# yangzichuang/TextSummarization-On-Flink

Measured on AMD Instinct MI355X. Metric: train_tokens_per_sec, higher is better.
Workload: dtype bf16; 1 GPU; model=pointer-generator+coverage hidden=256 emb=128 enc=400 dec=100 vocab=50000, global_batch=256, per_gpu_batch=256, seq_len=400->100, parallelism=dp1, backend=none, grad_allreduce=none, graph=True, persistent_lstm=True, proj_attn=True, skip_pad_steps=True, decoder_row_groups=2

## Files before the change

csrc/bindings.cpp:

```cpp
#include <torch/library.h>
#include <ATen/ATen.h>
#include <c10/hip/HIPStream.h>
#include <algorithm>
#include <optional>

#include "launchers.h"

using at::Tensor;
using OT = std::optional<Tensor>;

namespace {

hipStream_t stream() { return c10::hip::getCurrentHIPStream().stream(); }

void chk(const Tensor& t, at::ScalarType dt, const char* name) {
  TORCH_CHECK(t.is_cuda(), name, " must be a GPU tensor");
  TORCH_CHECK(t.scalar_type() == dt, name, " has dtype ", t.scalar_type(), ", expected ", dt);
  TORCH_CHECK(t.is_contiguous(), name, " must be contiguous");
}
template <typename T>
T* P(const Tensor& t) { return reinterpret_cast<T*>(t.data_ptr()); }
template <typename T>
T* PO(const OT& t) { return t.has_value() && t->defined() ? reinterpret_cast<T*>(t->data_ptr()) : nullptr; }
void numel_eq(const Tensor& t, int64_t n, const char* name) {
  TORCH_CHECK(t.numel() == n, name, " has ", t.numel(), " elements, expected ", n);
}
void chko(const OT& t, at::ScalarType dt, int64_t n, const char* name) {
  if (t.has_value() && t->defined()) { chk(*t, dt, name); numel_eq(*t, n, name); }
}
const auto F32 = at::kFloat;
const auto BF = at::kBFloat16;
const auto I32 = at::kInt;

void lstm_enc_fwd_step(const Tensor& gx, const Tensor& bias, const Tensor& Wt, const Tensor& hs, const Tensor& cs,
                       const Tensor& acts, const Tensor& out, const Tensor& lens, int64_t s, int64_t T, int64_t B,
                       int64_t H) {
  chk(gx, F32, "gx"); chk(bias, F32, "bias"); numel_eq(bias, 2 * 4 * H, "bias"); chk(Wt, BF, "Wt"); chk(hs, BF, "hs"); chk(cs, F32, "cs"); chk(acts, F32, "acts");
  chk(out, BF, "out"); chk(lens, I32, "lens");
  TORCH_CHECK(H % 32 == 0 && s >= 0 && s < T, "bad lstm args");
  numel_eq(gx, 2 * T * B * 4 * H, "gx"); numel_eq(Wt, 2 * 4 * H * H, "Wt");
  numel_eq(hs, 2 * (T + 1) * B * H, "hs"); numel_eq(cs, 2 * (T + 1) * B * H, "cs");
  numel_eq(acts, 2 * T * B * 4 * H, "acts"); numel_eq(out, B * T * 2 * H, "out"); numel_eq(lens, B, "lens");
  launch_lstm_enc_fwd_step(P<float>(gx), P<float>(bias), P<bf16>(Wt), P<bf16>(hs), P<float>(cs), P<float>(acts), P<bf16>(out),
                           P<int>(lens), s, T, B, H, stream());
}

void lstm_enc_bwd_step(const Tensor& dz, const Tensor& Wn, const Tensor& dout, const Tensor& dh_fin,
                       const Tensor& dc_carry, const Tensor& acts, const Tensor& cs, const Tensor& lens, int64_t s,
                       int64_t T, int64_t B, int64_t H) {
  chk(dz, BF, "dz"); chk(Wn, BF, "Wn"); chk(dout, F32, "dout"); chk(dh_fin, F32, "dh_fin");
  chk(dc_carry, F32, "dc_carry"); chk(acts, F32, "acts"); chk(cs, F32, "cs"); chk(lens, I32, "lens");
  TORCH_CHECK(H % 32 == 0 && s >= 0 && s < T, "bad lstm args");
  numel_eq(dz, 2 * T * B * 4 * H, "dz"); numel_eq(Wn, 2 * 4 * H * H, "Wn"); numel_eq(dout, B * T * 2 * H, "dout");
  numel_eq(dh_fin, 2 * B * H, "dh_fin"); numel_eq(dc_carry, 2 * B * H, "dc_carry");
  numel_eq(acts, 2 * T * B * 4 * H, "acts"); numel_eq(cs, 2 * (T + 1) * B * H, "cs");
  launch_lstm_enc_bwd_step(P<bf16>(dz), P<bf16>(Wn), P<float>(dout), P<float>(dh_fin), P<float>(dc_carry),
                           P<float>(acts), P<float>(cs), P<int>(lens), s, T, B, H, stream());
}

int64_t lstm_persistent_grid_op(int64_t H, int64_t B) { return lstm_persistent_grid((int)H, (int)B); }
int64_t lstm_persistent_capacity_op(int64_t H) { return lstm_persistent_capacity((int)H); }
int64_t lstm_persistent_launches_op(int64_t H, int64_t B) { return lstm_persistent_launches((int)H, (int)B); }
int64_t lstm_persistent_xbuf_op(int64_t H, int64_t B, bool bwd) {
  return (int64_t)lstm_persistent_xbuf_elems((int)H, (int)B, bwd);
}

void lstm_fwd_persistent(const Tensor& gx, const Tensor& bias, const Tensor& Wt, const Tensor& hs, const Tensor& cs,
                         const Tensor& acts, const Tensor& out, const Tensor& lens, const Tensor& xbuf,
                         const Tensor& err, int64_t T, int64_t B, int64_t H) {
  chk(gx, F32, "gx"); chk(bias, F32, "bias"); numel_eq(bias, 2 * 4 * H, "bias"); chk(Wt, BF, "Wt"); chk(hs, BF, "hs"); chk(cs, F32, "cs"); chk(acts, F32, "acts");
  chk(out, BF, "out"); chk(lens, I32, "lens"); chk(xbuf, at::kLong, "xbuf"); chk(err, I32, "err");
  TORCH_CHECK(lstm_persistent_grid((int)H, (int)B) > 0, "persistent LSTM: unsupported H/B (H in {64,128,256,512}; "
              "a launch's grid must fit the resident capacity, one workgroup per CU)");
  TORCH_CHECK(T >= 1 && T < (1 << 30), "bad T");
  numel_eq(gx, 2 * T * B * 4 * H, "gx"); numel_eq(Wt, 2 * 4 * H * H, "Wt");
  numel_eq(hs, 2 * (T + 1) * B * H, "hs"); numel_eq(cs, 2 * (T + 1) * B * H, "cs");
  numel_eq(acts, 2 * T * B * 4 * H, "acts"); numel_eq(out, B * T * 2 * H, "out"); numel_eq(lens, B, "lens");
  TORCH_CHECK(xbuf.numel() >= (int64_t)lstm_persistent_xbuf_elems((int)H, (int)B, false), "xbuf too small");
  numel_eq(err, 1, "err");
  launch_lstm_fwd_persistent(P<float>(gx), P<float>(bias), P<bf16>(Wt), P<bf16>(hs), P<float>(cs), P<float>(acts), P<bf16>(out),
                             P<int>(lens), (unsigned long long*)xbuf.data_ptr(), (unsigned*)err.data_ptr(), T, B, H,
                             stream());
}

bool lstm_persistent_fx_ok_op(int64_t H, int64_t B, int64_t E) { return lstm_persistent_fx_ok((int)H, (int)B, (int)E); }
void lstm_fwd_persistent_fx(const Tensor& xsf, const Tensor& Wx0, const Tensor& Wx1, const Tensor& bias,
                            const Tensor& Wt, const Tensor& hs, const Tensor& cs, const Tensor& acts, const Tensor& out,
                            const Tensor& lens, const Tensor& xbuf, const Tensor& err, int64_t T, int64_t B, int64_t H) {
  chk(xsf, BF, "xsf"); chk(Wx0, BF, "Wx0"); chk(Wx1, BF, "Wx1");
  chk(bias, F32, "bias"); numel_eq(bias, 2 * 4 * H, "bias"); chk(Wt, BF, "Wt"); chk(hs, BF, "hs"); chk(cs, F32, "cs");
  chk(acts, F32, "acts"); chk(out, BF, "out"); chk(lens, I32, "lens"); chk(xbuf, at::kLong, "xbuf"); chk(err, I32, "err");
  TORCH_CHECK(lstm_persistent_fx_ok((int)H, (int)B, 128), "persistent LSTM with the input projection: unsupported H/B");
  TORCH_CHECK(T >= 1 && T < (1 << 30), "bad T");
  numel_eq(xsf, 2 * T * B * 128, "xsf"); numel_eq(Wx0, 4 * H * 128, "Wx0"); numel_eq(Wx1, 4 * H * 128, "Wx1");
  numel_eq(Wt, 2 * 4 * H * H, "Wt");
  numel_eq(hs, 2 * (T + 1) * B * H, "hs"); numel_eq(cs, 2 * (T + 1) * B * H, "cs");
  numel_eq(acts, 2 * T * B * 4 * H, "acts"); numel_eq(out, B * T * 2 * H, "out"); numel_eq(lens, B, "lens");
  TORCH_CHECK(xbuf.numel() >= (int64_t)lstm_persistent_xbuf_elems((int)H, (int)B, false), "xbuf too small");
  numel_eq(err, 1, "err");
  launch_lstm_fwd_persistent(nullptr, P<float>(bias), P<bf16>(Wt), P<bf16>(hs), P<float>(cs), P<float>(acts), P<bf16>(out),
                             P<int>(lens), (unsigned long long*)xbuf.data_ptr(), (unsigned*)err.data_ptr(), T, B, H,
                             stream(), P<bf16>(xsf), P<bf16>(Wx0), P<bf16>(Wx1));
}

void lstm_bwd_persistent(const Tensor& dz, const Tensor& Wn, const Tensor& dout, const Tensor& dh_fin,
                         const Tensor& dc_carry, const Tensor& acts, const Tensor& cs, const Tensor& lens,
                         const Tensor& xbuf, const Tensor& err, const OT& dbias, int64_t T, int64_t B, int64_t H,
                         bool dout_batch_frame) {
  const bool dout16 = dout.scalar_type() == BF;
  TORCH_CHECK(!dout16 || dout_batch_frame, "lstm_bwd_persistent: a bf16 dout is read in the batch frame only");
  chk(dz, BF, "dz"); chk(Wn, BF, "Wn"); chk(dout, dout16 ? BF : F32, "dout"); chk(dh_fin, F32, "dh_fin");
  chko(dbias, F32, 2 * 4 * H, "dbias");
  chk(dc_carry, F32, "dc_carry"); chk(acts, F32, "acts"); chk(cs, F32, "cs"); chk(lens, I32, "lens");
  chk(xbuf, at::kLong, "xbuf"); chk(err, I32, "err");
  TORCH_CHECK(lstm_persistent_grid((int)H, (int)B) > 0, "persistent LSTM: unsupported H/B");
  TORCH_CHECK(T >= 1 && T < (1 << 30), "bad T");
  numel_eq(dz, 2 * T * B * 4 * H, "dz"); numel_eq(Wn, 2 * 4 * H * H, "Wn"); numel_eq(dout, B * T * 2 * H, "dout");
  numel_eq(dh_fin, 2 * B * H, "dh_fin"); numel_eq(dc_carry, 2 * B * H, "dc_carry");
  numel_eq(acts, 2 * T * B * 4 * H, "acts"); numel_eq(cs, 2 * (T + 1) * B * H, "cs"); numel_eq(lens, B, "lens");
  TORCH_CHECK(xbuf.numel() >= (int64_t)lstm_persistent_xbuf_elems((int)H, (int)B, true), "xbuf too small");
  numel_eq(err, 1, "err");
  launch_lstm_bwd_persistent(P<bf16>(dz), P<bf16>(Wn), (const float*)dout.data_ptr(), P<float>(dh_fin),
                             P<float>(dc_carry), P<float>(acts), P<float>(cs), P<int>(lens),
                             (unsigned long long*)xbuf.data_ptr(), (unsigned*)err.data_ptr(), PO<float>(dbias), T, B, H,
                             dout_batch_frame, stream(), dout16);
}

void attn_score(const Tensor& F, const Tensor& s, const Tensor& v, const OT& wc, const OT& cov, const Tensor& lens,
                const Tensor& e, int64_t B, int64_t T, int64_t A, int64_t rep) {
  chk(F, BF, "F"); chk(s, F32, "s"); chk(v, F32, "v"); chk(lens, I32, "lens"); chk(e, F32, "e");
  TORCH_CHECK(A % 64 == 0 && A <= 1024 && T % 2 == 0, "attention size must be a multiple of 64 (<= 1024), T even");
  TORCH_CHECK((rep == 1 || rep == 2 || rep == 4) && B % rep == 0, "rep must be 1, 2 or 4 and divide B");
  numel_eq(F, B / rep * T * A, "F"); numel_eq(s, B * A, "s"); numel_eq(v, A, "v"); numel_eq(e, B * T, "e");
  numel_eq(lens, B / rep, "lens"); chko(wc, F32, A, "wc"); chko(cov, F32, B * T, "cov");
  launch_attn_score(P<bf16>(F), P<float>(s), P<float>(v), PO<float>(wc), PO<float>(cov), P<int>(lens), P<float>(e), B,
                    T, A, rep, stream());
}

void attn_softmax_ctx(const Tensor& e, const Tensor& E, const Tensor& lens, const OT& cov, const Tensor& a_out,
                      const OT& cov_out, const OT& covloss, const Tensor& ctx, const OT& ctx_bf, int64_t B, int64_t T,
                      int64_t A, int64_t rep) {
  chk(e, F32, "e"); chk(E, BF, "E"); chk(lens, I32, "lens"); chk(a_out, F32, "a_out"); chk(ctx, F32, "ctx");
  TORCH_CHECK((rep == 1 || rep == 2 || rep == 4) && B % rep == 0, "rep must be 1, 2 or 4 and divide B");
  TORCH_CHECK(A % 64 == 0 && T <= (rep == 1 ? 2048 : 1024), "bad attention shape");
  numel_eq(e, B * T, "e"); numel_eq(E, B / rep * T * A, "E"); numel_eq(a_out, B * T, "a_out");
  numel_eq(ctx, B * A, "ctx"); numel_eq(lens, B / rep, "lens");
  chko(cov, F32, B * T, "cov"); chko(cov_out, F32, B * T, "cov_out"); chko(covloss, F32, B, "covloss");
  chko(ctx_bf, BF, B * A, "ctx_bf");
  launch_attn_softmax_ctx(P<float>(e), P<bf16>(E), P<int>(lens), PO<float>(cov), P<float>(a_out), PO<float>(cov_out),
                          PO<float>(covloss), P<float>(ctx), PO<bf16>(ctx_bf), B, T, A, rep, stream());
}

bool attn_row_ok(int64_t A, int64_t T) { return attn_row_supported((int)A, (int)T); }
void attn_fwd_row(const Tensor& F, const Tensor& E, const Tensor& s, const Tensor& v, const OT& wc, const OT& cov,
                  const Tensor& lens, const Tensor& a_out, const OT& cov_out, const OT& covloss, const Tensor& ctx,
                  const OT& ctx_bf, int64_t B, int64_t T, int64_t A, int64_t rep) {
  chk(F, BF, "F"); chk(E, BF, "E"); chk(s, F32, "s"); chk(v, F32, "v"); chk(lens, I32, "lens");
  chk(a_out, F32, "a_out"); chk(ctx, F32, "ctx");
  TORCH_CHECK(attn_row_supported((int)A, (int)T), "row attention needs A in {512, 1024} and T <= 2048");
  TORCH_CHECK(rep >= 1 && B % rep == 0, "attn_fwd_row: rep must divide B");
  numel_eq(F, B / rep * T * A, "F"); numel_eq(E, B / rep * T * A, "E"); numel_eq(s, B * A, "s"); numel_eq(v, A, "v");
  numel_eq(lens, B / rep, "lens"); numel_eq(a_out, B * T, "a_out"); numel_eq(ctx, B * A, "ctx");
  chko(wc, F32, A, "wc"); chko(cov, F32, B * T, "cov"); chko(cov_out, F32, B * T, "cov_out");
  chko(covloss, F32, B, "covloss"); chko(ctx_bf, BF, B * A, "ctx_bf");
  launch_attn_fwd_row(P<bf16>(F), P<bf16>(E), P<float>(s), P<float>(v), PO<float>(wc),
                      PO<float>(cov), P<int>(lens), P<float>(a_out), PO<float>(cov_out), PO<float>(covloss), P<float>(ctx),
                      PO<bf16>(ctx_bf), B, T, A, (int)rep, stream());
}
void attn_fwd_row_probe(const Tensor& F, const Tensor& E, const Tensor& s, const Tensor& v, const Tensor& wc,
                        const Tensor& cov, const Tensor& lens, const Tensor& a_out, const Tensor& ctx, int64_t B, int64_t T,
                        int64_t rep, int64_t probe) {
  chk(F, BF, "F"); chk(E, BF, "E"); chk(s, F32, "s"); chk(v, F32, "v"); chk(wc, F32, "wc"); chk(cov, F32, "cov");
  chk(lens, I32, "lens"); chk(a_out, F32, "a_out"); chk(ctx, F32, "ctx");
  TORCH_CHECK(rep >= 1 && B % rep == 0 && T <= 2048, "attn_fwd_row_probe: rep | B, T <= 2048");
  numel_eq(F, B / rep * T * 512, "F"); numel_eq(E, B / rep * T * 512, "E"); numel_eq(s, B * 512, "s");
  numel_eq(v, 512, "v"); numel_eq(wc, 512, "wc"); numel_eq(cov, B * T, "cov"); numel_eq(lens, B / rep, "lens");
  numel_eq(a_out, B * T, "a_out"); numel_eq(ctx, B * 512, "ctx");
  launch_attn_fwd_row_probe(P<bf16>(F), P<bf16>(E), P<float>(s), P<float>(v), P<float>(wc), P<float>(cov), P<int>(lens),
                            P<float>(a_out), P<float>(ctx), (int)B, (int)T, (int)rep, (int)probe, stream());
}
void attn_bwd_row(const Tensor& E, const Tensor& F, const Tensor& s, const Tensor& v, const OT& wc, const OT& cov,
                  const Tensor& a, const Tensor& dctx, const Tensor& ctx, const OT& Ga, const OT& dcov_next,
                  const OT& gcl, const Tensor& lens, const Tensor& de_out, const Tensor& ds, const OT& dcov_out,
                  int64_t B, int64_t T, int64_t A) {
  chk(E, BF, "E"); chk(F, BF, "F"); chk(s, F32, "s"); chk(v, F32, "v"); chk(a, F32, "a"); chk(dctx, F32, "dctx");
  chk(ctx, F32, "ctx"); chk(lens, I32, "lens"); chk(de_out, F32, "de_out"); chk(ds, F32, "ds");
  TORCH_CHECK(attn_row_supported((int)A, (int)T), "row attention needs A in {512, 1024} and T <= 2048");
  numel_eq(E, B * T * A, "E"); numel_eq(F, B * T * A, "F"); numel_eq(s, B * A, "s"); numel_eq(v, A, "v");
  numel_eq(a, B * T, "a"); numel_eq(dctx, B * A, "dctx"); numel_eq(ctx, B * A, "ctx"); numel_eq(lens, B, "lens");
  numel_eq(de_out, B * T, "de_out"); numel_eq(ds, B * A, "ds");
  chko(wc, F32, A, "wc"); chko(cov, F32, B * T, "cov"); chko(Ga, F32, B * T, "Ga");
  chko(dcov_next, F32, B * T, "dcov_next"); chko(gcl, F32, B, "gcl"); chko(dcov_out, F32, B * T, "dcov_out");
  launch_attn_bwd_row(P<bf16>(E), P<bf16>(F), P<float>(s), P<float>(v), PO<float>(wc), PO<float>(cov), P<float>(a),
                      P<float>(dctx), P<float>(ctx), PO<float>(Ga), PO<float>(dcov_next), PO<float>(gcl),
                      P<int>(lens), P<float>(de_out), P<float>(ds), PO<float>(dcov_out), B, T, A, stream());
}

bool attn_rowp_ok(int64_t A, int64_t T, int64_t EG) { return attn_rowp_supported((int)A, (int)T, (int)EG); }
bool dec_persistent_ok_op(int64_t H, int64_t E, int64_t A, int64_t B, int64_t T) {
  return dec_persistent_shape_ok((int)H, (int)E, (int)A, (int)B, (int)T);
}
int64_t dec_persistent_grid_op(int64_t B) { return dec_persistent_grid((int)B); }
int64_t dec_persistent_capacity_op() { return dec_persistent_capacity(); }
int64_t dec_persistent_xbuf_op(int64_t B) { return (int64_t)dec_persistent_xbuf_elems((int)B); }
void dec_fwd_persistent(const Tensor& XG, const Tensor& KcT, const Tensor& WsT, const Tensor& bs, const Tensor& Cst,
                        const Tensor& Cb, const Tensor& Hb, const Tensor& ACT, const Tensor& S, const Tensor& F,
                        const Tensor& G, const Tensor& v, const OT& wc, const OT& COV, const Tensor& lens,
                        const Tensor& ATT, const Tensor& ATTb, const OT& covloss, const Tensor& GV, const Tensor& GVb,
                        const OT& dlen, const Tensor& xbuf, const Tensor& err, int64_t B, int64_t T, int64_t D,
                        int64_t H, int64_t E, int64_t A) {
  TORCH_CHECK(dec_persistent_shape_ok((int)H, (int)E, (int)A, (int)B, (int)T) && D >= 1,
              "dec_fwd_persistent: unsupported shape");
  const int64_t grid = dec_persistent_grid((int)B);
  TORCH_CHECK(grid > 0 && grid <= dec_persistent_capacity(),
              "dec_fwd_persistent: the grid would not be co-resident on this device");
  chk(XG, F32, "XG"); numel_eq(XG, D * B * 4 * H, "XG");
  chk(KcT, BF, "KcT"); numel_eq(KcT, 4 * H * (E + H), "KcT");
  chk(WsT, BF, "WsT"); numel_eq(WsT, A * 2 * H, "WsT");
  chk(bs, F32, "bs"); numel_eq(bs, A, "bs");
  chk(Cst, F32, "Cst"); numel_eq(Cst, (D + 1) * B * H, "Cst");
  chk(Cb, BF, "Cb"); numel_eq(Cb, (D + 1) * B * H, "Cb");
  chk(Hb, BF, "Hb"); numel_eq(Hb, (D + 1) * B * H, "Hb");
  chk(ACT, F32, "ACT"); numel_eq(ACT, D * B * 4 * H, "ACT");
  chk(S, F32, "S"); numel_eq(S, D * B * A, "S");
  chk(F, BF, "F"); numel_eq(F, B * T * A, "F");
  chk(G, BF, "G"); numel_eq(G, B * T * E, "G");
  chk(v, F32, "v"); numel_eq(v, A, "v");
  chko(wc, F32, A, "wc");
  chko(COV, F32, (D + 1) * B * T, "COV");
  chk(lens, I32, "lens"); numel_eq(lens, B, "lens");
  chk(ATT, F32, "ATT"); numel_eq(ATT, D * B * T, "ATT");
  chk(ATTb, BF, "ATTb"); numel_eq(ATTb, D * B * T, "ATTb");
  chko(covloss, F32, D * B, "covloss");
  TORCH_CHECK((PO<float>(COV) != nullptr) == (PO<float>(covloss) != nullptr), "COV and covloss go together");
  chk(GV, F32, "GV"); numel_eq(GV, D * B * E, "GV");
  chk(GVb, BF, "GVb"); numel_eq(GVb, D * B * E, "GVb");
  chko(dlen, I32, B, "dlen");
  chk(xbuf, at::kLong, "xbuf"); numel_eq(xbuf, (int64_t)dec_persistent_xbuf_elems((int)B), "xbuf");
  chk(err, I32, "err");
  launch_dec_fwd_persistent(P<float>(XG), P<bf16>(KcT), P<bf16>(WsT), P<float>(bs), P<float>(Cst), P<bf16>(Cb),
                            P<bf16>(Hb), P<float>(ACT), P<float>(S), P<bf16>(F), P<bf16>(G), P<float>(v),
                            PO<float>(wc), PO<float>(COV), P<int>(lens), P<float>(ATT), P<bf16>(ATTb),
                            PO<float>(covloss), P<float>(GV), P<bf16>(GVb), PO<int>(dlen),
                            (unsigned long long*)xbuf.data_ptr(), (unsigned*)err.data_ptr(), (int)B, (int)T, (int)D,
                            stream());
}

void attn_fwd_rowp(const Tensor& F, const Tensor& G, const Tensor& s, const Tensor& v, const OT& wc, const OT& cov,
                   const Tensor& lens, const Tensor& a_out, const OT& cov_out, const OT& covloss, const Tensor& gx,
                   const Tensor& gx_bf, int64_t B, int64_t T, int64_t A, const OT& dlen, int64_t step,
                   const OT& a_bf) {
  chk(F, BF, "F"); chk(G, BF, "G"); chk(s, F32, "s"); chk(v, F32, "v"); chk(lens, I32, "lens");
  chk(a_out, F32, "a_out"); chk(gx, F32, "gx"); chk(gx_bf, BF, "gx_bf"); chko(a_bf, BF, B * T, "a_bf");
  const int64_t EG = gx.numel() / std::max<int64_t>(B, 1);
  TORCH_CHECK(attn_rowp_supported((int)A, (int)T, (int)EG), "projected row attention needs A in {512, 1024}, "
              "T <= 2048 and a 128-wide projection");
  numel_eq(F, B * T * A, "F"); numel_eq(G, B * T * EG, "G"); numel_eq(s, B * A, "s"); numel_eq(v, A, "v");
  numel_eq(lens, B, "lens"); numel_eq(a_out, B * T, "a_out"); numel_eq(gx, B * EG, "gx"); numel_eq(gx_bf, B * EG, "gx_bf");
  chko(wc, F32, A, "wc"); chko(cov, F32, B * T, "cov"); chko(cov_out, F32, B * T, "cov_out");
  chko(covloss, F32, B, "covloss"); chko(dlen, I32, B, "dlen");
  launch_attn_fwd_rowp(P<bf16>(F), P<bf16>(G), P<float>(s), P<float>(v), PO<float>(wc), PO<float>(cov), P<int>(lens),
                       P<float>(a_out), PO<float>(cov_out), PO<float>(covloss), P<float>(gx), P<bf16>(gx_bf), B, T, A,
                       PO<int>(dlen), (int)step, stream(), PO<bf16>(a_bf));
}
void attn_bwd_rowp(const Tensor& G, const Tensor& F, const Tensor& s, const Tensor& v, const OT& wc, const OT& cov,
                   const Tensor& a, const OT& dx, const Tensor& gv, const OT& Ga, const OT& dcov_next, const OT& gcl,
                   const Tensor& lens, const Tensor& de_out, const Tensor& ds, const OT& dcov_out, int64_t B, int64_t T,
                   int64_t A, const OT& dlen, int64_t step) {
  chk(G, BF, "G"); chk(F, BF, "F"); chk(s, F32, "s"); chk(v, F32, "v"); chk(a, F32, "a"); chk(gv, F32, "gv");
  chk(lens, I32, "lens"); chk(de_out, F32, "de_out"); chk(ds, F32, "ds");
  const int64_t EG = gv.numel() / std::max<int64_t>(B, 1);
  TORCH_CHECK(attn_rowp_supported((int)A, (int)T, (int)EG), "projected row attention needs A in {512, 1024}, "
              "T <= 2048 and a 128-wide projection");
  numel_eq(G, B * T * EG, "G"); numel_eq(F, B * T * A, "F"); numel_eq(s, B * A, "s"); numel_eq(v, A, "v");
  numel_eq(a, B * T, "a"); numel_eq(gv, B * EG, "gv"); numel_eq(lens, B, "lens");
  numel_eq(de_out, B * T, "de_out"); numel_eq(ds, B * A, "ds");
  chko(dx, F32, B * EG, "dx"); chko(wc, F32, A, "wc"); chko(cov, F32, B * T, "cov"); chko(Ga, F32, B * T, "Ga");
  chko(dcov_next, F32, B * T, "dcov_next"); chko(gcl, F32, B, "gcl"); chko(dcov_out, F32, B * T, "dcov_out");
  chko(dlen, I32, B, "dlen");
  launch_attn_bwd_rowp(P<bf16>(G), P<bf16>(F), P<float>(s), P<float>(v), PO<float>(wc), PO<float>(cov), P<float>(a),
                       PO<float>(dx), P<float>(gv), PO<float>(Ga), PO<float>(dcov_next), PO<float>(gcl), P<int>(lens),
                       P<float>(de_out), P<float>(ds), PO<float>(dcov_out), B, T, A, PO<int>(dlen), (int)step, stream());
}

void attn_bwd_step(const Tensor& E, const Tensor& F, const Tensor& s, const Tensor& v, const OT& wc, const OT& cov,
                   const Tensor& a, const Tensor& dctx, const Tensor& ctx, const OT& Ga, const OT& dcov_next,
                   const OT& gcl, const Tensor& lens, const Tensor& de_out, const Tensor& ds, const OT& dcov_out,
                   int64_t B, int64_t T, int64_t A) {
  chk(E, BF, "E"); chk(F, BF, "F"); chk(s, F32, "s"); chk(v, F32, "v"); chk(a, F32, "a"); chk(dctx, F32, "dctx");
  chk(ctx, F32, "ctx"); chk(lens, I32, "lens"); chk(de_out, F32, "de_out"); chk(ds, F32, "ds");
  TORCH_CHECK(A % 64 == 0 && A <= 1024 && T >= 1, "bad A/T");
  numel_eq(E, B * T * A, "E"); numel_eq(F, B * T * A, "F"); numel_eq(s, B * A, "s"); numel_eq(v, A, "v");
  numel_eq(a, B * T, "a"); numel_eq(dctx, B * A, "dctx"); numel_eq(ctx, B * A, "ctx"); numel_eq(lens, B, "lens");
  numel_eq(de_out, B * T, "de_out"); numel_eq(ds, B * A, "ds");
  chko(wc, F32, A, "wc"); chko(cov, F32, B * T, "cov"); chko(Ga, F32, B * T, "Ga");
  chko(dcov_next, F32, B * T, "dcov_next"); chko(gcl, F32, B, "gcl"); chko(dcov_out, F32, B * T, "dcov_out");
  launch_attn_bwd_step(P<bf16>(E), P<bf16>(F), P<float>(s), P<float>(v), PO<float>(wc), PO<float>(cov), P<float>(a),
                       P<float>(dctx), P<float>(ctx), PO<float>(Ga), PO<float>(dcov_next), PO<float>(gcl),
                       P<int>(lens), P<float>(de_out), P<float>(ds), PO<float>(dcov_out), B, T, A, stream());
}

void attn_bwd_feat(const Tensor& F, const Tensor& S_all, const Tensor& v, const OT& wc, const OT& cov_all,
                   const Tensor& de_all, const Tensor& lens, const Tensor& dF, const Tensor& dv, const OT& dwc,
                   int64_t D, int64_t B, int64_t T, int64_t A, const OT& dlen) {
  chk(F, BF, "F"); chk(S_all, F32, "S_all"); chk(v, F32, "v"); chk(de_all, F32, "de_all"); chk(lens, I32, "lens");
  chk(dF, BF, "dF"); chk(dv, F32, "dv");
  TORCH_CHECK(A % 64 == 0, "bad A");
  numel_eq(F, B * T * A, "F"); numel_eq(S_all, D * B * A, "S_all"); numel_eq(de_all, D * B * T, "de_all");
  const int64_t nslot = dv.numel() / A;
  TORCH_CHECK(nslot >= 1 && nslot <= (1 << 20) && (nslot & (nslot - 1)) == 0 && dv.numel() == nslot * A,
              "dv: [nslot, A] with nslot a power of two");
  numel_eq(dF, B * T * A, "dF");
  chko(wc, F32, A, "wc"); chko(cov_all, F32, D * B * T, "cov_all"); chko(dwc, F32, nslot * A, "dwc");
  chko(dlen, I32, B, "dlen");
  launch_attn_bwd_feat(P<bf16>(F), P<float>(S_all), P<float>(v), PO<float>(wc), PO<float>(cov_all), P<float>(de_all),
                       P<int>(lens), P<bf16>(dF), P<float>(dv), PO<float>(dwc), D, B, T, A, (int)nslot, stream(),
                       PO<int>(dlen));
}

int64_t attn_chunks(int64_t T) { return attn_nchunk(T); }

void emb_grad_sorted(const Tensor& gemb, const Tensor& sid, const Tensor& perm, const Tensor& src0, const Tensor& src1) {
  chk(gemb, F32, "gemb"); chk(src0, F32, "src0"); chk(src1, F32, "src1");
  TORCH_CHECK(gemb.dim() == 2 && gemb.size(1) <= 512, "gemb must be [V][E], E <= 512");
  TORCH_CHECK(sid.scalar_type() == at::kInt && perm.scalar_type() == at::kInt && sid.is_contiguous() &&
              perm.is_contiguous() && sid.numel() == perm.numel(), "sid / perm int32, contiguous, one length");
  const int64_t E = gemb.size(1), V = gemb.size(0);
  TORCH_CHECK(src0.numel() % E == 0 && src1.numel() % E == 0, "src rows");
  const int64_t n0 = src0.numel() / E, n1 = src1.numel() / E;
  TORCH_CHECK(sid.numel() == n0 + n1, "sid must cover src0 and src1 rows");
  launch_emb_grad_sorted(P<float>(gemb), P<int>(sid), P<int>(perm), P<float>(src0), (int)n0, P<float>(src1),
                         (int)n1, (int)E, (int)V, stream());
}

int64_t emb_grad_det_chunks_op(int64_t n) { return emb_grad_det_chunks((int)n); }
void emb_grad_det(const Tensor& gemb, const Tensor& sid, const Tensor& perm, const Tensor& src0, const Tensor& src1,
                  const Tensor& pf, const Tensor& pl) {
  chk(gemb, F32, "gemb"); chk(src0, F32, "src0"); chk(src1, F32, "src1"); chk(pf, F32, "pf"); chk(pl, F32, "pl");
  TORCH_CHECK(gemb.dim() == 2 && gemb.size(1) <= 512, "gemb must be [V][E], E <= 512");
  TORCH_CHECK(sid.scalar_type() == at::kInt && perm.scalar_type() == at::kInt && sid.is_contiguous() &&
              perm.is_contiguous() && sid.numel() == perm.numel(), "sid / perm int32, contiguous, one length");
  const int64_t E = gemb.size(1), V = gemb.size(0);
  TORCH_CHECK(src0.numel() % E == 0 && src1.numel() % E == 0, "src rows");
  const int64_t n0 = src0.numel() / E, n1 = src1.numel() / E;
  TORCH_CHECK(sid.numel() == n0 + n1, "sid must cover src0 and src1 rows");
  const int64_t nc = emb_grad_det_chunks((int)(n0 + n1));
  numel_eq(pf, nc * E, "pf"); numel_eq(pl, nc * E, "pl");
  launch_emb_grad_det(P<float>(gemb), P<int>(sid), P<int>(perm), P<float>(src0), (int)n0, P<float>(src1), (int)n1,
                      (int)E, (int)V, P<float>(pf), P<float>(pl), stream());
}

void step_frame_hop(const Tensor& in, const Tensor& rev, const Tensor& out, int64_t B, int64_t T, int64_t H) {
  chk(in, F32, "in"); chk(out, F32, "out");
  TORCH_CHECK(H % 4 == 0 && B > 0 && T > 0, "step_frame_hop: H % 4 == 0");
  TORCH_CHECK(rev.scalar_type() == at::kLong && rev.is_contiguous() && rev.numel() == B * T, "rev [B,T] int64");
  numel_eq(in, 2 * T * B * 2 * H, "in"); numel_eq(out, 2 * T * B * H, "out");
  launch_step_frame_hop(P<float>(in), rev.data_ptr<int64_t>(), P<float>(out), (int)B, (int)T, (int)H, stream());
}

void to_step_frame(const Tensor& src, const OT& ids, const Tensor& rev, const Tensor& out, int64_t B, int64_t T,
                   int64_t W, int64_t doff) {
  TORCH_CHECK(src.is_cuda() && src.is_contiguous() && out.is_contiguous() && src.scalar_type() == out.scalar_type(),
              "src/out: contiguous GPU tensors of one dtype");
  TORCH_CHECK(src.scalar_type() == BF || src.scalar_type() == F32, "bf16 or fp32");
  TORCH_CHECK(rev.scalar_type() == at::kLong && rev.is_contiguous() && rev.numel() == B * T, "rev [B,T] int64");
  const int es = (int)src.element_size();
  TORCH_CHECK((W * es) % 16 == 0 && (doff * es) % 16 == 0, "rows must be 16-byte multiples");
  const int64_t S = src.size(-1);
  TORCH_CHECK(doff + W <= S && (S * es) % 16 == 0, "bad row width");
  if (ids.has_value()) {
    TORCH_CHECK(ids->scalar_type() == at::kLong && ids->is_contiguous() && ids->numel() == B * T, "ids [B,T] int64");
  } else {
    TORCH_CHECK(src.numel() == B * T * S, "src must be [B,T,S] without ids");
  }
  numel_eq(out, 2 * T * B * W, "out");
  launch_to_step_frame(src.data_ptr(), es, PO<int64_t>(ids), P<int64_t>(rev), out.data_ptr(), (int)B, (int)T, (int)W,
                       (int)S, (int)doff, src.numel() / S, stream());
}
void from_step_frame(const Tensor& in, const Tensor& rev, const Tensor& out, int64_t B, int64_t T, int64_t W) {
  chk(in, F32, "in"); chk(out, F32, "out");
  TORCH_CHECK(rev.scalar_type() == at::kLong && rev.is_contiguous() && rev.numel() == B * T, "rev [B,T] int64");
  TORCH_CHECK(W % 4 == 0, "W % 4");
  numel_eq(in, 2 * T * B * W, "in"); numel_eq(out, B * T * W, "out");
  launch_from_step_frame(P<float>(in), P<int64_t>(rev), P<float>(out), (int)B, (int)T, (int)W, stream());
}
void transpose_bta(const Tensor& in, const Tensor& out, int64_t B, int64_t T, int64_t A) {
  chk(in, BF, "in"); chk(out, BF, "out");
  TORCH_CHECK(A % 64 == 0, "A % 64");
  numel_eq(in, B * T * A, "in"); numel_eq(out, B * T * A, "out");
  launch_transpose_bta(P<bf16>(in), P<bf16>(out), (int)B, (int)T, (int)A, stream());
}
void tr01(const Tensor& in, const OT& out, const OT& outb, int64_t np_, int64_t nq, int64_t nr, bool acc) {
  chk(in, F32, "in");
  TORCH_CHECK(nr % 4 == 0 && np_ >= 1 && nq >= 1, "tr01: R % 4 == 0");
  TORCH_CHECK(!acc || (out.has_value() && !outb.has_value()), "tr01: acc adds into out (no bf16 twin)");
  numel_eq(in, np_ * nq * nr, "in");
  chko(out, F32, np_ * nq * nr, "out"); chko(outb, BF, np_ * nq * nr, "outb");
  TORCH_CHECK((uintptr_t)in.data_ptr() % 16 == 0, "tr01: in must be 16-byte aligned");
  TORCH_CHECK(!PO<float>(out) || (uintptr_t)PO<float>(out) % 16 == 0, "tr01: out must be 16-byte aligned");
  TORCH_CHECK(!PO<bf16>(outb) || (uintptr_t)PO<bf16>(outb) % 8 == 0, "tr01: outb must be 8-byte aligned");
  launch_tr01(P<float>(in), PO<float>(out), PO<bf16>(outb), (int)np_, (int)nq, (int)nr, acc, stream());
}
void cast_colsum(const Tensor& x, const Tensor& xb, const Tensor& colsum, int64_t N, int64_t C) {
  chk(x, F32, "x"); chk(xb, BF, "xb"); chk(colsum, F32, "colsum");
  TORCH_CHECK(C % 4 == 0 && C / 4 <= 256 && 256 % (C / 4) == 0, "cast_colsum: C % 4 == 0 and C / 4 divides 256");
  numel_eq(x, N * C, "x"); numel_eq(xb, N * C, "xb"); numel_eq(colsum, C, "colsum");
  auto part = at::empty({(int64_t)cast_colsum_blocks((int)N, (int)C), C}, x.options());
  launch_cast_colsum(P<float>(x), P<bf16>(xb), P<float>(part), P<float>(colsum), (int)N, (int)C, stream());
}
void colsum(const Tensor& x, const Tensor& out, int64_t N, int64_t C, bool acc) {
  TORCH_CHECK(x.is_cuda() && x.is_contiguous() && (x.scalar_type() == F32 || x.scalar_type() == BF),
              "colsum: x must be a contiguous CUDA fp32 / bf16 tensor");
  chk(out, F32, "out");
  numel_eq(x, N * C, "x"); numel_eq(out, C, "out");
  auto part = at::empty({(int64_t)colsum_det_chunks((int)N, (int)C), C}, out.options());
  launch_colsum_det(x.data_ptr(), x.scalar_type() == BF, P<float>(part), P<float>(out), (int)N, (int)C, acc, stream());
}

void rs_fwd(const Tensor& cs, const Tensor& hs, int64_t T, const Tensor& RCt, const Tensor& RHt, const Tensor& bc,
            const Tensor& bh, const Tensor& pre_c, const Tensor& pre_h, const Tensor& c0, const Tensor& c0b,
            const Tensor& h0b, const OT& cat_c, const OT& cat_h, int64_t B, int64_t H) {
  chk(cs, F32, "cs"); chk(hs, BF, "hs"); chk(RCt, BF, "RCt"); chk(RHt, BF, "RHt"); chk(bc, F32, "bc"); chk(bh, F32, "bh");
  chk(pre_c, F32, "pre_c"); chk(pre_h, F32, "pre_h"); chk(c0, F32, "c0"); chk(c0b, BF, "c0b"); chk(h0b, BF, "h0b");
  TORCH_CHECK(H % 32 == 0 && H <= 512, "reduce_states: H % 32 == 0, H <= 512");
  numel_eq(cs, 2 * (T + 1) * B * H, "cs"); numel_eq(hs, 2 * (T + 1) * B * H, "hs");
  numel_eq(RCt, 2 * H * H, "RCt"); numel_eq(RHt, 2 * H * H, "RHt"); numel_eq(bc, H, "bc"); numel_eq(bh, H, "bh");
  numel_eq(pre_c, B * H, "pre_c"); numel_eq(pre_h, B * H, "pre_h"); numel_eq(c0, B * H, "c0");
  numel_eq(c0b, B * H, "c0b"); numel_eq(h0b, B * H, "h0b");
  chko(cat_c, BF, 2 * B * H, "cat_c"); chko(cat_h, BF, 2 * B * H, "cat_h");
  const size_t off = (size_t)T * B * H, ds = (size_t)(T + 1) * B * H;
  launch_rs_fwd(P<float>(cs) + off, P<bf16>(hs) + off, ds, P<bf16>(RCt), P<bf16>(RHt), P<float>(bc), P<float>(bh),
                P<float>(pre_c), P<float>(pre_h), P<float>(c0), P<bf16>(c0b), P<bf16>(h0b), PO<bf16>(cat_c),
                PO<bf16>(cat_h), (int)B, (int)H, stream());
}

void rs_bwd(const Tensor& gc, const Tensor& gh, const Tensor& pre_c, const Tensor& pre_h, const Tensor& RC,
            const Tensor& RH, const Tensor& dpc, const Tensor& dph, const OT& gbc, const OT& gbh,
            const Tensor& dold_c, const Tensor& dold_h, int64_t B, int64_t H) {
  chk(gc, F32, "gc"); chk(gh, F32, "gh"); chk(pre_c, F32, "pre_c"); chk(pre_h, F32, "pre_h"); chk(RC, BF, "RC");
  chk(RH, BF, "RH"); chk(dpc, BF, "dpc"); chk(dph, BF, "dph"); chko(gbc, F32, H, "gbc"); chko(gbh, F32, H, "gbh");
  chk(dold_c, F32, "dold_c"); chk(dold_h, F32, "dold_h");
  TORCH_CHECK(H % 32 == 0 && H <= 512, "reduce_states: H % 32 == 0, H <= 512");
  for (const Tensor* t : {&gc, &gh, &pre_c, &pre_h, &dpc, &dph}) numel_eq(*t, B * H, "[B][H] operand");
  numel_eq(RC, 2 * H * H, "RC"); numel_eq(RH, 2 * H * H, "RH");
  numel_eq(dold_c, 2 * B * H, "dold_c"); numel_eq(dold_h, 2 * B * H, "dold_h");
  launch_rs_bwd(P<float>(gc), P<float>(gh), P<float>(pre_c), P<float>(pre_h), P<bf16>(RC), P<bf16>(RH), P<bf16>(dpc),
                P<bf16>(dph), PO<float>(gbc), PO<float>(gbh), P<float>(dold_c), P<float>(dold_h), (size_t)B * H, (int)B,
                (int)H, stream());
}

void emb_grad(const Tensor& gemb, const Tensor& ids0, const Tensor& src0, const Tensor& ids1, const Tensor& src1) {
  chk(gemb, F32, "gemb"); chk(src0, F32, "src0"); chk(src1, F32, "src1");
  TORCH_CHECK(ids0.scalar_type() == at::kLong && ids1.scalar_type() == at::kLong && ids0.is_contiguous() &&
              ids1.is_contiguous(), "ids must be contiguous int64");
  TORCH_CHECK(gemb.dim() == 2, "gemb must be [V][E]");
  const int64_t E = gemb.size(1), V = gemb.size(0);
  numel_eq(src0, ids0.numel() * E, "src0"); numel_eq(src1, ids1.numel() * E, "src1");
  launch_emb_grad(P<float>(gemb), P<int64_t>(ids0), P<float>(src0), (int)ids0.numel(), P<int64_t>(ids1), P<float>(src1),
                  (int)ids1.numel(), (int)E, (int)V, stream());
}


void dec_cell_fwd(const Tensor& XG, const OT& ctxp, const Tensor& hprev, const Tensor& cprev, const Tensor& WcT,
                  const Tensor& c_out, const Tensor& cb_out, const Tensor& hb_out, const Tensor& act, int64_t B,
                  int64_t H, int64_t A, const OT& dlen, int64_t step) {
  chk(XG, F32, "XG"); chk(hprev, BF, "hprev"); chk(cprev, F32, "cprev"); chk(WcT, BF, "WcT"); chk(c_out, F32, "c_out");
  chk(cb_out, BF, "cb_out"); chk(hb_out, BF, "hb_out"); chk(act, F32, "act");
  TORCH_CHECK(H % 32 == 0 && A % 32 == 0, "dims must be multiples of 32");
  numel_eq(XG, B * 4 * H, "XG"); chko(ctxp, BF, B * A, "ctxp"); numel_eq(hprev, B * H, "hprev");
  numel_eq(cprev, B * H, "cprev"); numel_eq(WcT, 4 * H * (A + H), "WcT"); numel_eq(c_out, B * H, "c_out");
  numel_eq(cb_out, B * H, "cb_out"); numel_eq(hb_out, B * H, "hb_out"); numel_eq(act, B * 4 * H, "act");
  chko(dlen, I32, B, "dlen");
  launch_dec_cell_fwd(P<float>(XG), PO<bf16>(ctxp), P<bf16>(hprev), P<float>(cprev), P<bf16>(WcT), P<float>(c_out),
                      P<bf16>(cb_out), P<bf16>(hb_out), P<float>(act), B, H, A, PO<int>(dlen), (int)step, stream());
}

void dec_sproj(const Tensor& cb, const Tensor& hb, const Tensor& WsT, const Tensor& bs, const Tensor& s_out, int64_t B,
               int64_t H, int64_t A, const OT& dlen, int64_t step) {
  chk(cb, BF, "cb"); chk(hb, BF, "hb"); chk(WsT, BF, "WsT"); chk(bs, F32, "bs"); chk(s_out, F32, "s_out");
  TORCH_CHECK(H % 32 == 0 && A % 16 == 0, "bad dims");
  numel_eq(cb, B * H, "cb"); numel_eq(hb, B * H, "hb"); numel_eq(WsT, A * 2 * H, "WsT"); numel_eq(bs, A, "bs");
  numel_eq(s_out, B * A, "s_out"); chko(dlen, I32, B, "dlen");
  launch_dec_sproj(P<bf16>(cb), P<bf16>(hb), P<bf16>(WsT), P<float>(bs), P<float>(s_out), B, H, A, PO<int>(dlen),
                   (int)step, stream());
}

void dec_bwd_cell(const Tensor& ds, const Tensor& Ws, const OT& dC_dir, const OT& dH_dir, const Tensor& dh_rec,
                  const Tensor& dc_carry, const Tensor& act, const Tensor& c_now, const Tensor& c_prev,
                  const Tensor& dz, int64_t B, int64_t H, int64_t A, const OT& dlen, int64_t step) {
  chk(ds, F32, "ds"); chk(Ws, BF, "Ws"); chk(dh_rec, F32, "dh_rec"); chk(dc_carry, F32, "dc_carry");
  chk(act, F32, "act"); chk(c_now, F32, "c_now"); chk(c_prev, F32, "c_prev"); chk(dz, BF, "dz");
  TORCH_CHECK(H % 16 == 0 && A % 32 == 0, "bad dims");
  numel_eq(ds, B * A, "ds"); numel_eq(Ws, 2 * H * A, "Ws"); chko(dC_dir, F32, B * H, "dC_dir");
  chko(dH_dir, F32, B * H, "dH_dir"); numel_eq(dh_rec, B * H, "dh_rec"); numel_eq(dc_carry, B * H, "dc_carry");
  numel_eq(act, B * 4 * H, "act"); numel_eq(c_now, B * H, "c_now"); numel_eq(c_prev, B * H, "c_prev");
  numel_eq(dz, B * 4 * H, "dz"); chko(dlen, I32, B, "dlen");
  launch_dec_bwd_cell(P<float>(ds), P<bf16>(Ws), PO<float>(dC_dir), PO<float>(dH_dir), P<float>(dh_rec),
                      P<float>(dc_carry), P<float>(act), P<float>(c_now), P<float>(c_prev), P<bf16>(dz), B, H, A,
                      PO<int>(dlen), (int)step, stream());
}

void dec_bwd_dz(const Tensor& dz, const Tensor& Wbig, const OT& dX_dir, const OT& dCTX_dir_prev, const Tensor& dx_out,
                const OT& dctx_prev_out, const Tensor& dh_rec, int64_t B, int64_t E, int64_t H, int64_t A,
                const OT& dlen, int64_t step) {
  chk(dz, BF, "dz"); chk(Wbig, BF, "Wbig"); chk(dx_out, F32, "dx_out"); chk(dh_rec, F32, "dh_rec");
  TORCH_CHECK(E % 16 == 0 && H % 32 == 0 && A % 16 == 0, "bad dims");
  numel_eq(dz, B * 4 * H, "dz"); numel_eq(Wbig, (E + H + A) * 4 * H, "Wbig");
  chko(dX_dir, F32, B * E, "dX_dir"); chko(dCTX_dir_prev, F32, B * A, "dCTX_dir_prev");
  numel_eq(dx_out, B * E, "dx_out"); chko(dctx_prev_out, F32, B * A, "dctx_prev_out");
  numel_eq(dh_rec, B * H, "dh_rec"); chko(dlen, I32, B, "dlen");
  launch_dec_bwd_dz(P<bf16>(dz), P<bf16>(Wbig), PO<float>(dX_dir), PO<float>(dCTX_dir_prev), P<float>(dx_out),
                    PO<float>(dctx_prev_out), P<float>(dh_rec), B, E, H, A, PO<int>(dlen), (int)step, stream());
}

void ptr_loss(const Tensor& logits, const OT& bias, const Tensor& target, const Tensor& rowg, const OT& pgen,
              const OT& attn, const Tensor& ext, const Tensor& lens, const Tensor& loss_row, const OT& dlogits,
              const OT& dpre, const OT& dA, int64_t N, int64_t B, int64_t T, int64_t V) {
  const bool lbf = logits.scalar_type() == at::kBFloat16;
  chk(logits, lbf ? BF : F32, "logits"); chk(target, I32, "target"); chk(rowg, F32, "rowg"); chk(ext, I32, "ext");
  chk(lens, I32, "lens"); chk(loss_row, F32, "loss_row");
  TORCH_CHECK(lbf != bias.has_value(), "bf16 logits carry their bias (pass None); fp32 logits need the bias");
  chko(bias, F32, V, "bias");
  numel_eq(logits, N * V, "logits"); numel_eq(target, N, "target"); numel_eq(rowg, N, "rowg");
  numel_eq(ext, B * T, "ext"); numel_eq(lens, B, "lens"); numel_eq(loss_row, N, "loss_row");
  TORCH_CHECK(N % B == 0, "N must be D*B");
  chko(pgen, F32, N, "pgen"); chko(attn, F32, N * T, "attn"); chko(dlogits, BF, N * V, "dlogits");
  chko(dpre, F32, N, "dpre"); chko(dA, F32, N * T, "dA");
  TORCH_CHECK(!PO<float>(pgen) || (PO<float>(attn) && (!PO<bf16>(dlogits) || (PO<float>(dpre) && PO<float>(dA)))),
              "pointer mode needs attn, and dpre/dA when computing grads");
  if (lbf) {
    TORCH_CHECK(V <= ptr_loss_bf16_max_vocab(), "bf16 ptr_loss: V <= 65536");
    launch_ptr_loss_bf16(P<bf16>(logits), P<int>(target), P<float>(rowg), PO<float>(pgen), PO<float>(attn),
                         P<int>(ext), P<int>(lens), P<float>(loss_row), PO<bf16>(dlogits), PO<float>(dpre),
                         PO<float>(dA), N, B, T, V, stream());
    return;
  }
  launch_ptr_loss(P<float>(logits), P<float>(*bias), P<int>(target), P<float>(rowg), PO<float>(pgen), PO<float>(attn),
                  P<int>(ext), P<int>(lens), P<float>(loss_row), PO<bf16>(dlogits), PO<float>(dpre), PO<float>(dA), N,
                  B, T, V, stream());
}

int64_t wgrad_tt_ws(int64_t M, int64_t N, int64_t K) {
  if (wgrad_tt_ok((int)M, (int)N, (int)K))
    return wgrad_tt_direct((int)M, (int)N, (int)K, false, false) ? 1
                                                                 : (int64_t)wgrad_tt_splits((int)M, (int)N, (int)K) * M * N;
  if (wgrad_tt_ok((int)N, (int)M, (int)K)) return (int64_t)wgrad_tt_splits((int)N, (int)M, (int)K) * M * N;
  return 0;
}
bool wgrad_tt(const Tensor& a, const Tensor& b, const Tensor& out, const Tensor& ws, bool acc) {
  TORCH_CHECK(a.dim() == 2 && b.dim() == 2 && out.dim() == 2, "wgrad_tt: 2-D views");
  TORCH_CHECK(a.is_cuda() && b.is_cuda() && out.is_cuda() && ws.is_cuda(), "wgrad_tt: GPU tensors");
  TORCH_CHECK(a.scalar_type() == BF && b.scalar_type() == BF && out.scalar_type() == F32 && ws.scalar_type() == F32,
              "wgrad_tt: bf16, bf16 -> fp32");
  TORCH_CHECK(a.stride(1) == 1 && b.stride(1) == 1 && out.stride(1) == 1 && ws.is_contiguous(), "wgrad_tt: unit column stride");
  const int64_t K = a.size(0), M = a.size(1), N = b.size(1), nv = out.size(1);
  TORCH_CHECK(b.size(0) == K && out.size(0) == M && nv <= N, "wgrad_tt: shapes");
  if (!(a.stride(0) % 8 == 0 && b.stride(0) % 8 == 0 && (uintptr_t)a.data_ptr() % 16 == 0 &&
        (uintptr_t)b.data_ptr() % 16 == 0))
    return false;
  const bool plain = wgrad_tt_ok((int)M, (int)N, (int)K), swapped = !plain && wgrad_tt_ok((int)N, (int)M, (int)K);
  if (!plain && !(swapped && nv == N)) return false;
  if (nv != N && (nv % 4 != 0)) return false;
  const bool direct = plain && wgrad_tt_direct((int)M, (int)N, (int)K, false, acc);
  const int64_t need = direct ? 0 : (int64_t)wgrad_tt_splits((int)(plain ? M : N), (int)(plain ? N : M), (int)K) * M * N;
  if (ws.numel() < need) {
    TORCH_CHECK(acc, "wgrad_tt: workspace too small");
    return false;
  }
  if (plain)
    launch_wgrad_tt(P<bf16>(a), (int)a.stride(0), P<bf16>(b), (int)b.stride(0), P<float>(ws), P<float>(out),
                    (int)out.stride(0), (int)M, (int)N, (int)K, false, acc, (int)nv, stream());
  else
    launch_wgrad_tt(P<bf16>(b), (int)b.stride(0), P<bf16>(a), (int)a.stride(0), P<float>(ws), P<float>(out),
                    (int)out.stride(0), (int)N, (int)M, (int)K, true, acc, (int)M, stream());
  return true;
}
bool ctx_bmm_ok_op(int64_t B, int64_t T, int64_t D, int64_t A) { return ctx_bmm_ok((int)B, (int)T, (int)D, (int)A); }
static void ctx_chk(const Tensor& t, at::ScalarType dt, int64_t n, const char* name) {
  chk(t, dt, name);
  numel_eq(t, n, name);
  TORCH_CHECK((uintptr_t)t.data_ptr() % 16 == 0, name, ": 16-byte aligned base");
}
void ctx_fwd(const Tensor& att, const Tensor& enc, const Tensor& ctx, const Tensor& ctxb, int64_t B, int64_t T, int64_t D,
             int64_t A) {
  TORCH_CHECK(ctx_bmm_ok((int)B, (int)T, (int)D, (int)A), "ctx_fwd: D <= 128, T % 8 == 0, A % 128 == 0");
  ctx_chk(att, BF, D * B * T, "att"); ctx_chk(enc, BF, B * T * A, "enc");
  ctx_chk(ctx, F32, D * B * A, "ctx"); ctx_chk(ctxb, BF, D * B * A, "ctxb");
  launch_ctx_fwd(P<bf16>(att), P<bf16>(enc), P<float>(ctx), P<bf16>(ctxb), (int)B, (int)T, (int)D, (int)A, stream());
}
void ctx_da(const Tensor& dctx, const Tensor& enc, const Tensor& da, int64_t B, int64_t T, int64_t D, int64_t A, bool acc) {
  TORCH_CHECK(ctx_bmm_ok((int)B, (int)T, (int)D, (int)A), "ctx_da: D <= 128, T % 8 == 0, A % 128 == 0");
  ctx_chk(dctx, BF, D * B * A, "dctx"); ctx_chk(enc, BF, B * T * A, "enc"); ctx_chk(da, F32, D * B * T, "da");
  launch_ctx_da(P<bf16>(dctx), P<bf16>(enc), P<float>(da), (int)B, (int)T, (int)D, (int)A, acc, stream());
}
void ctx_de(const Tensor& att, const Tensor& dctx, const Tensor& de, int64_t B, int64_t T, int64_t D, int64_t A) {
  TORCH_CHECK(ctx_bmm_ok((int)B, (int)T, (int)D, (int)A), "ctx_de: D <= 128, T % 8 == 0, A % 128 == 0");
  const bool b16 = de.scalar_type() == BF;
  ctx_chk(att, BF, D * B * T, "att"); ctx_chk(dctx, BF, D * B * A, "dctx"); ctx_chk(de, b16 ? BF : F32, B * T * A, "de");
  launch_ctx_de(P<bf16>(att), P<bf16>(dctx), b16 ? nullptr : P<float>(de), b16 ? P<bf16>(de) : nullptr, (int)B, (int)T,
                (int)D, (int)A, stream());
}
void wgrad_tn(const Tensor& a, const Tensor& b, const Tensor& out) {
  TORCH_CHECK(a.dim() == 2 && b.dim() == 2 && out.dim() == 2, "wgrad_tn: 2-D views");
  TORCH_CHECK(a.is_cuda() && b.is_cuda() && out.is_cuda(), "wgrad_tn: GPU tensors");
  TORCH_CHECK(a.scalar_type() == BF && b.scalar_type() == BF && out.scalar_type() == F32, "wgrad_tn: bf16, bf16 -> fp32");
  TORCH_CHECK(a.stride(1) == 1 && b.stride(1) == 1 && out.stride(1) == 1, "wgrad_tn: unit column stride");
  const int64_t K = a.size(0), M = a.size(1), N = b.size(1);
  TORCH_CHECK(b.size(0) == K && out.size(0) == M && out.size(1) == N, "wgrad_tn: shapes");
  TORCH_CHECK(M % 128 == 0 && N % 8 == 0 && K >= 1, "wgrad_tn: M a multiple of 128, N of 8");
  TORCH_CHECK(a.stride(0) % 8 == 0 && b.stride(0) % 8 == 0 && (uintptr_t)a.data_ptr() % 16 == 0 &&
              (uintptr_t)b.data_ptr() % 16 == 0, "wgrad_tn: 16-byte aligned rows");
  launch_wgrad_tn(P<bf16>(a), (int)a.stride(0), P<bf16>(b), (int)b.stride(0), P<float>(out), (int)out.stride(0),
                  (int)M, (int)N, (int)K, stream());
}

int64_t pack_max_jobs_op() { return pack_max_jobs(); }
int64_t pack_job_cols_op() { return pack_job_cols(); }
void pack_cast(const Tensor& jobs, int64_t total) {
  TORCH_CHECK(jobs.is_cuda() && jobs.scalar_type() == at::kLong && jobs.is_contiguous() && jobs.dim() == 2 &&
              jobs.size(1) == pack_job_cols(), "pack_cast: jobs [nj][", pack_job_cols(), "] int64 on the GPU");
  TORCH_CHECK(jobs.size(0) >= 1 && jobs.size(0) <= pack_max_jobs(), "pack_cast: 1..", pack_max_jobs(), " jobs");
  launch_pack_cast(P<long>(jobs), (int)jobs.size(0), (long)total, stream());
}

int64_t debug_enabled() { return tsamd_debug_enabled(); }
Tensor debug_status() {
  unsigned v[4];
  tsamd_debug_read(v);
  Tensor t = at::empty({4}, at::TensorOptions().dtype(at::kLong));
  int64_t* d = t.data_ptr<int64_t>();
  for (int i = 0; i < 4; ++i) d[i] = (int64_t)v[i];
  return t;
}
void debug_clear() { tsamd_debug_clear(); }

bool gemm_bt_ok(int64_t M, int64_t N, int64_t K) { return gemm_bt_supported((int)M, (int)N, (int)K, N % 256 == 0 ? 256 : 128); }
int64_t gemm_bt_splitk_ws(int64_t M, int64_t N, int64_t K) {
  if (!gemm_bt_ok(M, N, K)) return 0;
  const int S = gemm_bt_splits((int)M, (int)N, (int)K);
  return S > 1 ? (int64_t)S * M * N : 0;
}
bool gemm_bt_splitk(const Tensor& A, const Tensor& Bt, const Tensor& out, const Tensor& ws, bool acc) {
  TORCH_CHECK(A.is_cuda() && A.dim() == 2 && A.scalar_type() == BF && A.stride(1) == 1, "gemm_bt_splitk: A [rows, K] bf16");
  TORCH_CHECK(Bt.is_cuda() && Bt.dim() == 2 && Bt.scalar_type() == BF && Bt.stride(1) == 1, "gemm_bt_splitk: Bt [N, K] bf16");
  TORCH_CHECK(out.is_cuda() && out.dim() == 2 && out.stride(1) == 1 && out.scalar_type() == F32, "gemm_bt_splitk: out fp32");
  TORCH_CHECK(ws.is_cuda() && ws.is_contiguous() && ws.scalar_type() == F32, "gemm_bt_splitk: fp32 workspace");
  const int64_t M = out.size(0), N = out.size(1), K = Bt.size(1);
  TORCH_CHECK(Bt.size(0) == N && A.size(1) == K && A.size(0) >= M, "gemm_bt_splitk: shape mismatch A ", A.sizes(), " Bt ",
              Bt.sizes(), " out ", out.sizes());
  const int64_t need = gemm_bt_splitk_ws(M, N, K);
  if (need == 0 || ws.numel() < need) return false;
  if (!(A.stride(0) % 8 == 0 && Bt.stride(0) % 8 == 0 && reinterpret_cast<uintptr_t>(A.data_ptr()) % 16 == 0 &&
        reinterpret_cast<uintptr_t>(Bt.data_ptr()) % 16 == 0 && reinterpret_cast<uintptr_t>(out.data_ptr()) % 16 == 0 &&
        out.stride(0) % 4 == 0))
    return false;
  launch_gemm_bt_splitk(P<bf16>(A), A.stride(0), P<bf16>(Bt), Bt.stride(0), P<float>(ws), P<float>(out), out.stride(0),
                        (int)M, (int)N, (int)K, acc, stream());
  return true;
}
void gemm_bt(const Tensor& A, const Tensor& Bt, const Tensor& out, double beta, const OT& bias, const OT& ids,
             const OT& rev, int64_t B, int64_t T, int64_t dir, const OT& xsf) {
  TORCH_CHECK(A.is_cuda() && A.dim() == 2 && A.scalar_type() == BF && A.stride(1) == 1, "gemm_bt: A [rows, K] bf16");
  TORCH_CHECK(Bt.is_cuda() && Bt.dim() == 2 && Bt.scalar_type() == BF && Bt.stride(1) == 1, "gemm_bt: Bt [N, K] bf16");
  TORCH_CHECK(out.is_cuda() && out.dim() == 2 && out.stride(1) == 1 && (out.scalar_type() == F32 || out.scalar_type() == BF),
              "gemm_bt: out [M, N] fp32 / bf16");
  const int64_t M = out.size(0), N = out.size(1), K = Bt.size(1);
  TORCH_CHECK(Bt.size(0) == N && A.size(1) >= K, "gemm_bt: shape mismatch A ", A.sizes(), " Bt ", Bt.sizes(), " out ", out.sizes());
  TORCH_CHECK(gemm_bt_ok(M, N, K), "gemm_bt: N % 128 == 0 and K % 64 == 0 (got N ", N, " K ", K, ")");
  TORCH_CHECK(A.stride(0) % 8 == 0 && Bt.stride(0) % 8 == 0 && out.stride(0) % 8 == 0 &&
              reinterpret_cast<uintptr_t>(A.data_ptr()) % 16 == 0 && reinterpret_cast<uintptr_t>(Bt.data_ptr()) % 16 == 0 &&
              reinterpret_cast<uintptr_t>(out.data_ptr()) % 16 == 0, "gemm_bt: 16-byte aligned rows");
  const bool obf = out.scalar_type() == BF;
  TORCH_CHECK(beta == 0.0 || (beta == 1.0 && !obf), "gemm_bt: beta 0, or 1 with an fp32 out");
  chko(bias, F32, N, "bias");
  const bool frame = PO<int64_t>(rev) != nullptr;
  if (frame) {
    chk(*rev, at::kLong, "rev"); numel_eq(*rev, B * T, "rev");
    TORCH_CHECK(M == B * T && (dir == 0 || dir == 1), "gemm_bt: step frame needs M = T * B and dir 0 / 1");
    if (PO<int64_t>(ids)) { chk(*ids, at::kLong, "ids"); numel_eq(*ids, B * T, "ids"); }
    else TORCH_CHECK(A.size(0) == B * T, "gemm_bt: batch-frame A needs B * T rows");
    chko(xsf, BF, M * K, "xsf");
  } else {
    TORCH_CHECK(A.size(0) >= M && !PO<int64_t>(ids) && !PO<bf16>(xsf), "gemm_bt: plain A needs M rows (no xsf)");
  }
  launch_gemm_bt(P<bf16>(A), A.stride(0), P<bf16>(Bt), Bt.stride(0), out.data_ptr(), out.stride(0), obf, beta != 0.0,
                 PO<float>(bias), (int)M, (int)N, (int)K, frame ? 1 : 0, PO<int64_t>(ids), PO<int64_t>(rev), PO<bf16>(xsf), A.size(0),
                 (int)B, (int)T, (int)dir, stream());
}

void gemm_bt_merge(const Tensor& dz, const Tensor& Bt, const Tensor& out, const Tensor& rev, int64_t B, int64_t T,
                   int64_t mode) {
  TORCH_CHECK(dz.is_cuda() && dz.scalar_type() == BF && dz.is_contiguous() && dz.numel() % (2 * B * T) == 0,
              "gemm_bt_merge: dz [2][T][B][Kh] bf16, contiguous");
  const int64_t Kh = dz.numel() / (2 * B * T);
  TORCH_CHECK(Bt.is_cuda() && Bt.dim() == 2 && Bt.scalar_type() == BF && Bt.stride(1) == 1 && Bt.size(1) == 2 * Kh,
              "gemm_bt_merge: Bt [N, 2 Kh] bf16");
  chk(out, F32, "out");
  TORCH_CHECK(out.dim() == 2 && out.size(0) == B * T && out.size(1) == Bt.size(0) && out.stride(1) == 1,
              "gemm_bt_merge: out [T * B, N] fp32");
  chk(rev, at::kLong, "rev");
  numel_eq(rev, B * T, "rev");
  TORCH_CHECK(mode >= 0 && mode <= 7, "gemm_bt_merge: mode bits 0-2");
  const int64_t M = B * T, N = Bt.size(0), K = 2 * Kh;
  TORCH_CHECK(Kh % 64 == 0 && gemm_bt_ok(M, N, K), "gemm_bt_merge: Kh % 64 == 0 and N % 128 == 0");
  TORCH_CHECK(Bt.stride(0) % 8 == 0 && out.stride(0) % 4 == 0 && reinterpret_cast<uintptr_t>(dz.data_ptr()) % 16 == 0 &&
              reinterpret_cast<uintptr_t>(Bt.data_ptr()) % 16 == 0 && reinterpret_cast<uintptr_t>(out.data_ptr()) % 16 == 0,
              "gemm_bt_merge: 16-byte aligned rows");
  launch_gemm_bt(P<bf16>(dz), Kh, P<bf16>(Bt), Bt.stride(0), out.data_ptr(), out.stride(0), false, false, nullptr,
                 (int)M, (int)N, (int)K, 2, nullptr, P<int64_t>(rev), nullptr, 0, (int)B, (int)T, (int)mode, stream());
}

int64_t cu_hold_max_lds_op() { return cu_hold_max_lds(); }
void cu_hold(const Tensor& times, int64_t grid, double ms, int64_t lds_bytes) {
  chk(times, at::kLong, "times");
  numel_eq(times, 2 * grid, "times");
  TORCH_CHECK(grid >= 1 && grid <= 4096 && ms > 0 && ms <= 2000, "cu_hold: 1..4096 workgroups for at most 2 s");
  TORCH_CHECK(lds_bytes >= 0 && lds_bytes <= cu_hold_max_lds(), "cu_hold: lds_bytes above the CU's LDS");
  launch_cu_hold((int)grid, (unsigned long long)(ms * 1e5), P<long long>(times), (int)lds_bytes, stream());
}
void tanh_eval(const Tensor& x, const Tensor& t, const Tensor& s2, int64_t mode) {
  chk(x, F32, "x"); chk(t, F32, "t"); chk(s2, F32, "s2");
  numel_eq(t, x.numel(), "t"); numel_eq(s2, x.numel(), "s2");
  TORCH_CHECK(mode == 0 || mode == 1, "tanh_eval: mode 0 (exp + rcp) or 1 (rational)");
  launch_tanh_eval(P<float>(x), P<float>(t), P<float>(s2), (int)x.numel(), (int)mode, stream());
}
void tanh_tput(const Tensor& in, const Tensor& out, int64_t iters, int64_t mode) {
  chk(in, F32, "in"); chk(out, F32, "out");
  TORCH_CHECK(in.numel() >= 1024 && out.numel() % 256 == 0 && out.numel() > 0, "tanh_tput: in >= 1024, out % 256");
  TORCH_CHECK((mode == 0 || mode == 1) && iters >= 1, "tanh_tput: mode 0 / 1");
  launch_tanh_tput(P<float>(in), P<float>(out), (int)out.numel(), (int)iters, (int)mode, stream());
}

int64_t vocab_train_tiles_op(int64_t V, int64_t H) { return vocab_train_tiles((int)V, (int)H); }

void vocab_train_fwd(const Tensor& X, const Tensor& WT, const Tensor& bias, const Tensor& target, const Tensor& part,
                     const Tensor& zg, const Tensor& lse, const Tensor& pv, int64_t N, int64_t V, int64_t H,
                     int64_t ldx, const OT& vblk, const OT& vblk_n) {
  chk(X, BF, "X"); chk(WT, BF, "WT"); chk(bias, F32, "bias"); chk(target, I32, "target"); chk(part, F32, "part");
  chk(zg, F32, "zg"); chk(lse, F32, "lse"); chk(pv, F32, "pv");
  TORCH_CHECK(H == 128 || H == 256 || H == 512, "fused training vocab head: hidden size 128, 256 or 512");
  TORCH_CHECK(N >= 1 && V >= 1 && ldx >= H && ldx % 8 == 0, "bad N/V/ldx");
  numel_eq(X, N * ldx, "X"); numel_eq(WT, V * H, "WT"); numel_eq(bias, V, "bias"); numel_eq(target, N, "target");
  numel_eq(part, (int64_t)vocab_train_tiles((int)V, (int)H) * N * 2, "part"); numel_eq(zg, N, "zg"); numel_eq(lse, N, "lse");
  numel_eq(pv, N, "pv");
  const int64_t RB = (N + 31) / 32;
  TORCH_CHECK(vblk.has_value() == vblk_n.has_value(), "vblk and vblk_n go together");
  chko(vblk, I32, RB, "vblk"); chko(vblk_n, I32, 1, "vblk_n");
  launch_vocab_train_fwd(P<bf16>(X), (int)ldx, P<bf16>(WT), P<float>(bias), P<int>(target), P<float>(part), P<float>(zg),
                         P<float>(lse), P<float>(pv), N, V, H, PO<int>(vblk), PO<int>(vblk_n), stream());
}

void vocab_train_bwd(const Tensor& X, const Tensor& WT, const Tensor& bias, const Tensor& target, const Tensor& lse,
                     const Tensor& alpha, const Tensor& dl, const OT& dbias, int64_t N, int64_t V, int64_t H,
                     int64_t ldx, const OT& vblk, const OT& vblk_n, const OT& vlive, const OT& vstate) {
  chk(X, BF, "X"); chk(WT, BF, "WT"); chk(bias, F32, "bias"); chk(target, I32, "target"); chk(lse, F32, "lse");
  chk(alpha, F32, "alpha"); chk(dl, BF, "dl");
  TORCH_CHECK(H == 128 || H == 256 || H == 512, "fused training vocab head: hidden size 128, 256 or 512");
  TORCH_CHECK(N >= 1 && V >= 1 && ldx >= H && ldx % 8 == 0, "bad N/V/ldx");
  numel_eq(X, N * ldx, "X"); numel_eq(WT, V * H, "WT"); numel_eq(bias, V, "bias"); numel_eq(target, N, "target");
  numel_eq(lse, N, "lse"); numel_eq(alpha, N, "alpha"); chko(dbias, F32, V, "dbias");
  TORCH_CHECK(dl.numel() % N == 0, "dl: numel must be N * ldd");
  const int64_t ldd = dl.numel() / N;
  TORCH_CHECK(ldd >= V && (ldd == V || ldd % 8 == 0), "dl: row length ", ldd, " must be V or a multiple of 8");
  const int64_t RB = (N + 31) / 32;
  const bool has = vblk.has_value();
  TORCH_CHECK(vblk_n.has_value() == has && vlive.has_value() == vstate.has_value() && (has || !vlive.has_value()),
              "vblk and vblk_n go together, vlive and vstate go together (and need vblk)");
  chko(vblk, I32, RB, "vblk"); chko(vblk_n, I32, 1, "vblk_n"); chko(vlive, I32, RB, "vlive");
  chko(vstate, I32, RB, "vstate");
  launch_vocab_train_bwd(P<bf16>(X), (int)ldx, P<bf16>(WT), P<float>(bias), P<int>(target), P<float>(lse), P<float>(alpha),
                         P<bf16>(dl), (int)ldd, PO<float>(dbias), N, V, H, PO<int>(vblk), PO<int>(vblk_n), PO<int>(vlive),
                         PO<int>(vstate), stream());
}

void ptr_rowfin(const Tensor& pv, const Tensor& target, const Tensor& rowg, const OT& pgen, const OT& attn,
                const Tensor& ext, const Tensor& lens, const Tensor& loss_row, const OT& alpha, const OT& dpre,
                const OT& dA, int64_t N, int64_t B, int64_t T) {
  chk(pv, F32, "pv"); chk(target, I32, "target"); chk(rowg, F32, "rowg"); chk(ext, I32, "ext"); chk(lens, I32, "lens");
  chk(loss_row, F32, "loss_row");
  TORCH_CHECK(B >= 1 && N % B == 0, "N must be D*B");
  numel_eq(pv, N, "pv"); numel_eq(target, N, "target"); numel_eq(rowg, N, "rowg"); numel_eq(ext, B * T, "ext");
  numel_eq(lens, B, "lens"); numel_eq(loss_row, N, "loss_row");
  chko(pgen, F32, N, "pgen"); chko(attn, F32, N * T, "attn"); chko(alpha, F32, N, "alpha"); chko(dpre, F32, N, "dpre");
  chko(dA, F32, N * T, "dA");
  TORCH_CHECK(!PO<float>(pgen) || PO<float>(attn), "pointer mode needs attn");
  launch_ptr_rowfin(P<float>(pv), P<int>(target), P<float>(rowg), PO<float>(pgen), PO<float>(attn), P<int>(ext),
                    P<int>(lens), P<float>(loss_row), PO<float>(alpha), PO<float>(dpre), PO<float>(dA), N, B, T,
                    stream());
}

void clip_adagrad(const Tensor& w, const Tensor& acc, const Tensor& g, const Tensor& part, double lr, double max_norm,
                  double gscale, const Tensor& norm_out, const Tensor& flag, const OT& skip) {
  chk(w, F32, "w"); chk(acc, F32, "acc"); chk(g, F32, "g"); chk(part, F32, "part"); chk(norm_out, F32, "norm_out");
  chk(flag, I32, "flag"); chko(skip, I32, 1, "skip");
  TORCH_CHECK(w.numel() == acc.numel() && w.numel() == g.numel(), "flat buffers differ in size");
  numel_eq(part, opt_nparts(), "part");
  TORCH_CHECK(reinterpret_cast<uintptr_t>(w.data_ptr()) % 16 == 0 && reinterpret_cast<uintptr_t>(g.data_ptr()) % 16 == 0 &&
                  reinterpret_cast<uintptr_t>(acc.data_ptr()) % 16 == 0,
              "flat buffers must be 16-byte aligned");
  launch_clip_adagrad(P<float>(w), P<float>(acc), P<float>(g), w.numel(), P<float>(part), (float)lr, (float)max_norm,
                      (float)gscale, P<float>(norm_out), P<int>(flag), PO<int>(skip), stream());
}
int64_t opt_parts() { return opt_nparts(); }

void final_topk(const Tensor& logits, const Tensor& bias, const OT& pgen, const OT& attn, const Tensor& ext,
                const Tensor& lens, const Tensor& out_ids, const Tensor& out_lp, const Tensor& part_ms,
                const Tensor& part_v, const Tensor& part_i, int64_t R, int64_t V, int64_t T, int64_t K, int64_t beam) {
  chk(logits, F32, "logits"); chk(bias, F32, "bias"); chk(ext, I32, "ext"); chk(lens, I32, "lens");
  chk(out_ids, I32, "out_ids"); chk(out_lp, F32, "out_lp"); chk(part_ms, F32, "part_ms"); chk(part_v, F32, "part_v");
  chk(part_i, I32, "part_i");
  TORCH_CHECK(K >= 1 && K <= 16 && beam >= 1 && R % beam == 0 && T <= 2048, "bad topk args");
  numel_eq(logits, R * V, "logits"); numel_eq(bias, V, "bias"); numel_eq(ext, (R / beam) * T, "ext");
  numel_eq(lens, R / beam, "lens"); numel_eq(out_ids, R * K, "out_ids"); numel_eq(out_lp, R * K, "out_lp");
  TORCH_CHECK(topk_split(V) <= 64, "vocab too large for final_topk");
  numel_eq(part_ms, R * topk_split(V) * 2, "part_ms"); numel_eq(part_v, R * topk_split(V) * K, "part_v");
  numel_eq(part_i, R * topk_split(V) * K, "part_i");
  chko(pgen, F32, R, "pgen"); chko(attn, F32, R * T, "attn");
  TORCH_CHECK(!PO<float>(pgen) || PO<float>(attn), "pointer mode needs attn");
  launch_final_topk(P<float>(logits), P<float>(bias), PO<float>(pgen), PO<float>(attn), P<int>(ext), P<int>(lens),
                    P<int>(out_ids), P<float>(out_lp), P<float>(part_ms), P<float>(part_v), P<int>(part_i), R, V, T, K,
                    beam, stream());
}
int64_t topk_parts(int64_t V) { return topk_split(V); }

void vocab_topk(const Tensor& X, const Tensor& WT, const Tensor& bias, const OT& pgen, const OT& attn,
                const Tensor& ext, const Tensor& lens, const Tensor& out_ids, const Tensor& out_lp,
                const Tensor& logits, const Tensor& part_ms, int64_t R, int64_t V, int64_t H, int64_t T, int64_t K,
                int64_t beam) {
  chk(X, BF, "X"); chk(WT, BF, "WT"); chk(bias, F32, "bias"); chk(ext, I32, "ext"); chk(lens, I32, "lens");
  chk(out_ids, I32, "out_ids"); chk(out_lp, F32, "out_lp"); chk(logits, F32, "logits"); chk(part_ms, F32, "part_ms");
  const int64_t nt = vocab_topk_tiles((int)V, (int)H);
  TORCH_CHECK(K >= 1 && K <= 8 && beam >= 1 && R % beam == 0 && T <= 2048, "bad vocab_topk args (K <= 8)");
  TORCH_CHECK(H % 32 == 0 && (H <= 256 || H == 512) && nt <= 4096, "vocab_topk: H % 32 == 0, H <= 256 or 512, V <= 512k");
  numel_eq(X, R * H, "X"); numel_eq(WT, V * H, "WT"); numel_eq(bias, V, "bias");
  numel_eq(ext, (R / beam) * T, "ext"); numel_eq(lens, R / beam, "lens");
  numel_eq(out_ids, R * K, "out_ids"); numel_eq(out_lp, R * K, "out_lp");
  numel_eq(logits, R * V, "logits"); numel_eq(part_ms, R * nt * 2, "part_ms");
  chko(pgen, F32, R, "pgen"); chko(attn, F32, R * T, "attn");
  TORCH_CHECK(!PO<float>(pgen) || PO<float>(attn), "pointer mode needs attn");
  launch_vocab_topk(P<bf16>(X), P<bf16>(WT), P<float>(bias), PO<float>(pgen), PO<float>(attn), P<int>(ext),
                    P<int>(lens), P<int>(out_ids), P<float>(out_lp), P<float>(logits), P<float>(part_ms), R, V, H, T,
                    K, beam, PgIn{}, stream());
}
void vocab_topk_pg(const Tensor& X, const Tensor& WT, const Tensor& bias, const Tensor& ctx, const Tensor& c,
                   const Tensor& h, const Tensor& x, const Tensor& pg_w, const Tensor& pg_b, const Tensor& pg_out,
                   const Tensor& attn, const Tensor& ext, const Tensor& lens, const Tensor& out_ids,
                   const Tensor& out_lp, const Tensor& logits, const Tensor& part_ms, int64_t R, int64_t V, int64_t H,
                   int64_t T, int64_t K, int64_t beam, int64_t A, int64_t E) {
  chk(X, BF, "X"); chk(WT, BF, "WT"); chk(bias, F32, "bias"); chk(ext, I32, "ext"); chk(lens, I32, "lens");
  chk(out_ids, I32, "out_ids"); chk(out_lp, F32, "out_lp"); chk(logits, F32, "logits"); chk(part_ms, F32, "part_ms");
  chk(ctx, F32, "ctx"); chk(c, F32, "c"); chk(h, BF, "h"); chk(x, F32, "x"); chk(pg_w, F32, "pg_w");
  chk(pg_b, F32, "pg_b"); chk(pg_out, F32, "pg_out"); chk(attn, F32, "attn");
  const int64_t nt = vocab_topk_tiles((int)V, (int)H);
  TORCH_CHECK(K >= 1 && K <= 8 && beam >= 1 && R % beam == 0 && T <= 2048, "bad vocab_topk args (K <= 8)");
  TORCH_CHECK(H % 32 == 0 && (H <= 256 || H == 512) && nt <= 4096, "vocab_topk: H % 32 == 0, H <= 256 or 512, V <= 512k");
  numel_eq(X, R * H, "X"); numel_eq(WT, V * H, "WT"); numel_eq(bias, V, "bias");
  numel_eq(ext, (R / beam) * T, "ext"); numel_eq(lens, R / beam, "lens");
  numel_eq(out_ids, R * K, "out_ids"); numel_eq(out_lp, R * K, "out_lp");
  numel_eq(logits, R * V, "logits"); numel_eq(part_ms, R * nt * 2, "part_ms"); numel_eq(attn, R * T, "attn");
  numel_eq(ctx, R * A, "ctx"); numel_eq(c, R * H, "c"); numel_eq(h, R * H, "h"); numel_eq(x, R * E, "x");
  numel_eq(pg_w, A + 2 * H + E, "pg_w"); numel_eq(pg_b, 1, "pg_b"); numel_eq(pg_out, R, "pg_out");
  const PgIn pgi{P<float>(ctx), P<float>(c), P<bf16>(h), P<float>(x), P<float>(pg_w), P<float>(pg_b),
                 P<float>(pg_out), (int)A, (int)H, (int)E};
  launch_vocab_topk(P<bf16>(X), P<bf16>(WT), P<float>(bias), nullptr, P<float>(attn), P<int>(ext), P<int>(lens),
                    P<int>(out_ids), P<float>(out_lp), P<float>(logits), P<float>(part_ms), R, V, H, T, K, beam, pgi,
                    stream());
}
int64_t vocab_topk_parts(int64_t V, int64_t H) { return vocab_topk_tiles((int)V, (int)H); }
void lstm_bwd_stamps(const OT& buf) {
  set_lstm_bwd_stamps(buf.has_value() && buf->defined() ? (unsigned long long*)buf->data_ptr() : nullptr);
}
void vocab_select_stamps(const OT& buf) {
  set_vocab_select_stamps(buf.has_value() && buf->defined() ? (unsigned long long*)buf->data_ptr() : nullptr);
}
void vocab_span_probe(const Tensor& X, const Tensor& WT, const Tensor& bias, const Tensor& logits, const Tensor& part_ms,
                      int64_t R, int64_t V, int64_t probe) {
  chk(X, BF, "X"); chk(WT, BF, "WT"); chk(bias, F32, "bias"); chk(logits, F32, "logits"); chk(part_ms, F32, "part_ms");
  numel_eq(X, R * 256, "X"); numel_eq(WT, V * 256, "WT"); numel_eq(bias, V, "bias");
  TORCH_CHECK(logits.numel() >= std::max(R * V, R * 32 * 8 * (int64_t)vocab_topk_tiles((int)V, 256)), "logits too small");
  numel_eq(part_ms, R * vocab_topk_tiles((int)V, 256) * 2, "part_ms");
  launch_vocab_span_probe(P<bf16>(X), P<bf16>(WT), P<float>(bias), P<float>(logits), P<float>(part_ms), (int)R, (int)V,
                          (int)probe, stream());
}

NgSeq ng_seq(const OT& seq0, const OT& seq1, int64_t ngram, int64_t R, int64_t beam, int64_t max_dec) {
  if (ngram <= 1) return NgSeq{{nullptr, nullptr}, 0, 0};
  TORCH_CHECK(seq0.has_value() && seq0->defined() && seq1.has_value() && seq1->defined(),
              "n-gram blocking needs the seq0 / seq1 token-sequence buffers");
  chk(*seq0, I32, "seq0"); chk(*seq1, I32, "seq1");
  const int64_t pitch = R > 0 ? seq0->numel() / R : 0;
  TORCH_CHECK(pitch >= max_dec + 1 && pitch % 4 == 0 && beam * pitch <= NG_BAN_MAX && ngram <= (1 << 20),
              "n-gram blocking: seq is [R][P] with P >= max_dec + 1, P % 4 == 0 and beam * P <= ", NG_BAN_MAX);
  numel_eq(*seq0, R * pitch, "seq0"); numel_eq(*seq1, R * pitch, "seq1");
  TORCH_CHECK(seq0->data_ptr() != seq1->data_ptr(), "seq0 and seq1 must be two buffers");
  return NgSeq{{P<int>(*seq0), P<int>(*seq1)}, (int)pitch, (int)ngram};
}

void vocab_topk_beam_ng(const Tensor& X, const Tensor& WT, const Tensor& bias, const OT& ctx, const OT& c, const OT& h,
                     const OT& x, const OT& pg_w, const OT& pg_b, const OT& pg_out, const OT& attn, const Tensor& ext,
                     const Tensor& lens, const Tensor& out_ids, const Tensor& out_lp, const Tensor& logits,
                     const Tensor& part_ms, const Tensor& lp_sum, const Tensor& latest, const Tensor& gidx,
                     const Tensor& tok_hist, const Tensor& par_hist, const Tensor& done, const Tensor& res_count,
                     const Tensor& res_score, const Tensor& res_len, const Tensor& res_step, const Tensor& res_par,
                     const Tensor& step, const Tensor& art_ctr, const Tensor& gran, const Tensor& err,
                     const OT& att_hist, const OT& pg_hist, int64_t R,
                     int64_t V, int64_t H, int64_t T, int64_t K, int64_t beam, int64_t A, int64_t E, int64_t stop_id,
                     int64_t min_dec, int64_t max_dec, const OT& seq0, const OT& seq1, int64_t ngram) {
  chk(X, BF, "X"); chk(WT, BF, "WT"); chk(bias, F32, "bias"); chk(ext, I32, "ext"); chk(lens, I32, "lens");
  chk(out_ids, I32, "out_ids"); chk(out_lp, F32, "out_lp"); chk(logits, F32, "logits"); chk(part_ms, F32, "part_ms");
  const int64_t nt = vocab_topk_tiles((int)V, (int)H), Na = R / beam;
  TORCH_CHECK(K >= 1 && K <= 8 && beam >= 1 && R % beam == 0 && T <= 2048 && beam * K <= 64, "bad vocab_topk_beam args");
  TORCH_CHECK(H % 32 == 0 && (H <= 256 || H == 512) && nt <= 4096, "vocab_topk: H % 32 == 0, H <= 256 or 512, V <= 512k");
  numel_eq(X, R * H, "X"); numel_eq(WT, V * H, "WT"); numel_eq(bias, V, "bias");
  numel_eq(ext, Na * T, "ext"); numel_eq(lens, Na, "lens");
  numel_eq(out_ids, R * K, "out_ids"); numel_eq(out_lp, R * K, "out_lp");
  numel_eq(logits, R * V, "logits"); numel_eq(part_ms, R * nt * 2, "part_ms"); chko(attn, F32, R * T, "attn");
  const bool ptr = pg_w.has_value() && pg_w->defined();
  PgIn pgi{};
  if (ptr) {
    chko(ctx, F32, R * A, "ctx"); chko(c, F32, R * H, "c"); chko(h, BF, R * H, "h"); chko(x, F32, R * E, "x");
    chko(pg_w, F32, A + 2 * H + E, "pg_w"); chko(pg_b, F32, 1, "pg_b"); chko(pg_out, F32, R, "pg_out");
    TORCH_CHECK(PO<float>(ctx) && PO<float>(c) && PO<bf16>(h) && PO<float>(x) && PO<float>(pg_b) && PO<float>(attn),
                "pointer mode needs ctx, c, h, x, pg_b and attn");
    pgi = PgIn{PO<float>(ctx), PO<float>(c), PO<bf16>(h), PO<float>(x), PO<float>(pg_w), PO<float>(pg_b),
               PO<float>(pg_out), (int)A, (int)H, (int)E};
  }
  chk(lp_sum, F32, "lp_sum"); chk(latest, I32, "latest"); chk(gidx, I32, "gidx"); chk(tok_hist, I32, "tok_hist");
  chk(par_hist, I32, "par_hist"); chk(done, I32, "done"); chk(res_count, I32, "res_count");
  chk(res_score, F32, "res_score"); chk(res_len, I32, "res_len"); chk(res_step, I32, "res_step");
  chk(res_par, I32, "res_par"); chk(step, I32, "step"); chk(art_ctr, I32, "art_ctr");
  numel_eq(lp_sum, R, "lp_sum"); numel_eq(latest, R, "latest"); numel_eq(gidx, R, "gidx");
  numel_eq(tok_hist, max_dec * R, "tok_hist"); numel_eq(par_hist, max_dec * R, "par_hist"); numel_eq(done, Na, "done");
  numel_eq(res_count, Na, "res_count"); numel_eq(res_score, R, "res_score"); numel_eq(res_len, R, "res_len");
  numel_eq(res_step, R, "res_step"); numel_eq(res_par, R, "res_par"); numel_eq(step, 1, "step");
  numel_eq(art_ctr, Na, "art_ctr"); chk(gran, at::kLong, "gran"); numel_eq(gran, R * K, "gran");
  chk(err, I32, "err"); numel_eq(err, 1, "err");
  TORCH_CHECK(V + T < (1 << 17), "vocab_topk_beam: extended ids must fit 17 bits");
  chko(att_hist, F32, max_dec * R * T, "att_hist"); chko(pg_hist, F32, max_dec * R, "pg_hist");
  TORCH_CHECK(!PO<float>(att_hist) || PO<float>(attn), "att_hist needs attn");
  TORCH_CHECK(!PO<float>(pg_hist) || (ptr && PO<float>(att_hist)), "pg_hist needs the pointer inputs and att_hist");
  const BeamTail bt{P<float>(lp_sum), P<int>(latest), P<int>(gidx), P<int>(tok_hist), P<int>(par_hist), P<int>(done),
                    P<int>(res_count), P<float>(res_score), P<int>(res_len), P<int>(res_step), P<int>(res_par),
                    P<int>(step), (unsigned*)P<int>(art_ctr), (unsigned long long*)gran.data_ptr(), P<int>(err),
                    PO<float>(attn), PO<float>(att_hist), PO<float>(pg_out),
                    PO<float>(pg_hist), (int)T, (int)Na, (int)beam, (int)K, (int)stop_id, (int)min_dec, (int)max_dec};
  const NgSeq ng = ng_seq(seq0, seq1, ngram, R, beam, max_dec);
  launch_vocab_topk(P<bf16>(X), P<bf16>(WT), P<float>(bias), nullptr, ptr ? PO<float>(attn) : nullptr, P<int>(ext),
                    P<int>(lens), P<int>(out_ids), P<float>(out_lp), P<float>(logits), P<float>(part_ms), R, V, H, T, K,
                    beam, pgi, stream(), &bt, &ng);
}

void vocab_topk_beam(const Tensor& X, const Tensor& WT, const Tensor& bias, const OT& ctx, const OT& c, const OT& h,
                     const OT& x, const OT& pg_w, const OT& pg_b, const OT& pg_out, const OT& attn, const Tensor& ext,
                     const Tensor& lens, const Tensor& out_ids, const Tensor& out_lp, const Tensor& logits,
                     const Tensor& part_ms, const Tensor& lp_sum, const Tensor& latest, const Tensor& gidx,
                     const Tensor& tok_hist, const Tensor& par_hist, const Tensor& done, const Tensor& res_count,
                     const Tensor& res_score, const Tensor& res_len, const Tensor& res_step, const Tensor& res_par,
                     const Tensor& step, const Tensor& art_ctr, const Tensor& gran, const Tensor& err,
                     const OT& att_hist, const OT& pg_hist, int64_t R,
                     int64_t V, int64_t H, int64_t T, int64_t K, int64_t beam, int64_t A, int64_t E, int64_t stop_id,
                     int64_t min_dec, int64_t max_dec) {
  vocab_topk_beam_ng(X, WT, bias, ctx, c, h, x, pg_w, pg_b, pg_out, attn, ext, lens, out_ids, out_lp, logits, part_ms,
                     lp_sum, latest, gidx, tok_hist, par_hist, done, res_count, res_score, res_len, res_step, res_par,
                     step, art_ctr, gran, err, att_hist, pg_hist, R, V, H, T, K, beam, A, E, stop_id, min_dec, max_dec,
                     c10::nullopt, c10::nullopt, 0);
}

void dec_cell_fwd_beam(const Tensor& gidx, const Tensor& latest, const Tensor& XGtab, const Tensor& ctx_src,
                       const Tensor& h_src, const Tensor& c_src, const Tensor& WcT, const Tensor& c_out,
                       const Tensor& cb_out, const Tensor& hb_out, const Tensor& step, int64_t R, int64_t H, int64_t A,
                       int64_t V, int64_t unk) {
  chk(gidx, I32, "gidx"); chk(latest, I32, "latest"); chk(XGtab, F32, "XGtab"); chk(ctx_src, BF, "ctx_src");
  chk(h_src, BF, "h_src"); chk(c_src, F32, "c_src"); chk(WcT, BF, "WcT"); chk(c_out, F32, "c_out");
  chk(cb_out, BF, "cb_out"); chk(hb_out, BF, "hb_out"); chk(step, I32, "step");
  TORCH_CHECK(H % 16 == 0 && A % 32 == 0 && H % 32 == 0 && unk >= 0 && unk < V, "bad dims");
  numel_eq(gidx, R, "gidx"); numel_eq(latest, R, "latest"); numel_eq(XGtab, V * 4 * H, "XGtab");
  numel_eq(ctx_src, R * A, "ctx_src"); numel_eq(h_src, R * H, "h_src"); numel_eq(c_src, R * H, "c_src");
  numel_eq(WcT, 4 * H * (A + H), "WcT"); numel_eq(c_out, R * H, "c_out"); numel_eq(cb_out, R * H, "cb_out");
  numel_eq(hb_out, R * H, "hb_out"); numel_eq(step, 1, "step");
  launch_dec_cell_fwd_beam(P<int>(gidx), P<int>(latest), P<float>(XGtab), P<bf16>(ctx_src), P<bf16>(h_src),
                           P<float>(c_src), P<bf16>(WcT), P<float>(c_out), P<bf16>(cb_out), P<bf16>(hb_out),
                           P<int>(step), (int)R, (int)H, (int)A, (int)V, (int)unk, stream());
}

void beam_sproj_xmerge(const Tensor& cb, const Tensor& hb, const Tensor& WsT, const Tensor& bs, const Tensor& s_out,
                       const Tensor& ctx_src, const Tensor& WicT, const Tensor& Xtab, const Tensor& gidx,
                       const Tensor& latest, const Tensor& x_out, int64_t R, int64_t H, int64_t A, int64_t E,
                       int64_t V, int64_t unk) {
  chk(cb, BF, "cb"); chk(hb, BF, "hb"); chk(WsT, BF, "WsT"); chk(bs, F32, "bs"); chk(s_out, F32, "s_out");
  chk(ctx_src, BF, "ctx_src"); chk(WicT, BF, "WicT"); chk(Xtab, F32, "Xtab"); chk(gidx, I32, "gidx");
  chk(latest, I32, "latest"); chk(x_out, F32, "x_out");
  TORCH_CHECK(H % 32 == 0 && A % 32 == 0 && A % 16 == 0 && E % 16 == 0 && unk >= 0 && unk < V, "bad dims");
  numel_eq(cb, R * H, "cb"); numel_eq(hb, R * H, "hb"); numel_eq(WsT, A * 2 * H, "WsT"); numel_eq(bs, A, "bs");
  numel_eq(s_out, R * A, "s_out"); numel_eq(ctx_src, R * A, "ctx_src"); numel_eq(WicT, E * A, "WicT");
  numel_eq(Xtab, V * E, "Xtab"); numel_eq(gidx, R, "gidx"); numel_eq(latest, R, "latest"); numel_eq(x_out, R * E, "x_out");
  launch_beam_sproj_xmerge(P<bf16>(cb), P<bf16>(hb), P<bf16>(WsT), P<float>(bs), P<float>(s_out), P<bf16>(ctx_src),
                           P<bf16>(WicT), P<float>(Xtab), P<int>(gidx), P<int>(latest), P<float>(x_out), (int)R,
                           (int)H, (int)A, (int)E, (int)V, (int)unk, stream());
}

void attn_fwd_row_beam(const Tensor& F, const Tensor& E, const Tensor& s, const Tensor& v, const OT& wc,
                       const OT& cov_src, const OT& a_src, const OT& cov_keep, const Tensor& gidx, const Tensor& lens,
                       const Tensor& a_out, const Tensor& ctx, const OT& ctx_bf, int64_t B, int64_t T, int64_t A,
                       int64_t rep) {
  chk(F, BF, "F"); chk(E, BF, "E"); chk(s, F32, "s"); chk(v, F32, "v"); chk(lens, I32, "lens"); chk(gidx, I32, "gidx");
  chk(a_out, F32, "a_out"); chk(ctx, F32, "ctx");
  TORCH_CHECK(attn_row_supported((int)A, (int)T), "row attention needs A in {512, 1024} and T <= 2048");
  TORCH_CHECK(rep >= 1 && B % rep == 0, "attn_fwd_row_beam: rep must divide B");
  numel_eq(F, B / rep * T * A, "F"); numel_eq(E, B / rep * T * A, "E"); numel_eq(s, B * A, "s"); numel_eq(v, A, "v");
  numel_eq(lens, B / rep, "lens"); numel_eq(a_out, B * T, "a_out"); numel_eq(ctx, B * A, "ctx"); numel_eq(gidx, B, "gidx");
  chko(wc, F32, A, "wc"); chko(cov_src, F32, B * T, "cov_src"); chko(a_src, F32, B * T, "a_src");
  chko(cov_keep, F32, B * T, "cov_keep"); chko(ctx_bf, BF, B * A, "ctx_bf");
  const bool cov = PO<float>(cov_src) != nullptr;
  TORCH_CHECK(cov == (PO<float>(a_src) != nullptr) && cov == (PO<float>(cov_keep) != nullptr),
              "coverage gather: cov_src, a_src and cov_keep together");
  launch_attn_fwd_row(P<bf16>(F), P<bf16>(E), P<float>(s), P<float>(v), PO<float>(wc), PO<float>(cov_src), P<int>(lens),
                      P<float>(a_out), nullptr, nullptr, P<float>(ctx), PO<bf16>(ctx_bf), B, T, A, (int)rep, stream(),
                      cov ? P<int>(gidx) : nullptr, PO<float>(a_src), PO<float>(cov_keep));
}


void beam_step_ng(const Tensor& top_ids, const Tensor& top_lp, const Tensor& lp_sum, const Tensor& latest,
               const Tensor& gidx, const Tensor& tok_hist, const Tensor& par_hist, const Tensor& done,
               const Tensor& res_count, const Tensor& res_score, const Tensor& res_len, const Tensor& res_step,
               const Tensor& res_par, const Tensor& step, const OT& ctr, const OT& att, const OT& att_hist,
               const OT& pg, const OT& pg_hist, int64_t T, int64_t Na, int64_t beam, int64_t K, int64_t stop_id,
               int64_t min_dec, int64_t max_dec, const OT& seq0, const OT& seq1, int64_t ngram) {
  chk(top_ids, I32, "top_ids"); chk(top_lp, F32, "top_lp"); chk(lp_sum, F32, "lp_sum"); chk(latest, I32, "latest");
  chk(gidx, I32, "gidx"); chk(tok_hist, I32, "tok_hist"); chk(par_hist, I32, "par_hist"); chk(done, I32, "done");
  chk(res_count, I32, "res_count"); chk(res_score, F32, "res_score"); chk(res_len, I32, "res_len");
  chk(res_step, I32, "res_step"); chk(res_par, I32, "res_par"); chk(step, I32, "step"); chko(ctr, I32, 1, "ctr");
  const int64_t R = Na * beam;
  TORCH_CHECK(beam >= 1 && beam <= 16 && K >= 1 && K <= 16 && beam * K <= 64, "bad beam args");
  numel_eq(top_ids, R * K, "top_ids"); numel_eq(top_lp, R * K, "top_lp"); numel_eq(lp_sum, R, "lp_sum");
  numel_eq(latest, R, "latest"); numel_eq(gidx, R, "gidx"); numel_eq(tok_hist, max_dec * R, "tok_hist");
  numel_eq(par_hist, max_dec * R, "par_hist"); numel_eq(done, Na, "done"); numel_eq(res_count, Na, "res_count");
  numel_eq(res_score, R, "res_score"); numel_eq(res_len, R, "res_len"); numel_eq(res_step, R, "res_step");
  numel_eq(res_par, R, "res_par"); numel_eq(step, 1, "step");
  TORCH_CHECK(att.has_value() == att_hist.has_value() && pg.has_value() == pg_hist.has_value() &&
              (!pg.has_value() || att.has_value()), "att/att_hist and pg/pg_hist come in pairs (pg needs att)");
  chko(att, F32, R * T, "att"); chko(att_hist, F32, max_dec * R * T, "att_hist");
  chko(pg, F32, R, "pg"); chko(pg_hist, F32, max_dec * R, "pg_hist");
  const NgSeq ng = ng_seq(seq0, seq1, ngram, R, beam, max_dec);
  launch_beam_step(P<int>(top_ids), P<float>(top_lp), P<float>(lp_sum), P<int>(latest), P<int>(gidx), P<int>(tok_hist),
                   P<int>(par_hist), P<int>(done), P<int>(res_count), P<float>(res_score), P<int>(res_len),
                   P<int>(res_step), P<int>(res_par), P<int>(step), (unsigned*)PO<int>(ctr), PO<float>(att),
                   PO<float>(att_hist), PO<float>(pg), PO<float>(pg_hist), (int)T, Na, beam, K, stop_id, min_dec,
                   max_dec, stream(), &ng);
}

void beam_step(const Tensor& top_ids, const Tensor& top_lp, const Tensor& lp_sum, const Tensor& latest,
               const Tensor& gidx, const Tensor& tok_hist, const Tensor& par_hist, const Tensor& done,
               const Tensor& res_count, const Tensor& res_score, const Tensor& res_len, const Tensor& res_step,
               const Tensor& res_par, const Tensor& step, const OT& ctr, const OT& att, const OT& att_hist,
               const OT& pg, const OT& pg_hist, int64_t T, int64_t Na, int64_t beam, int64_t K, int64_t stop_id,
               int64_t min_dec, int64_t max_dec) {
  beam_step_ng(top_ids, top_lp, lp_sum, latest, gidx, tok_hist, par_hist, done, res_count, res_score, res_len, res_step,
               res_par, step, ctr, att, att_hist, pg, pg_hist, T, Na, beam, K, stop_id, min_dec, max_dec, c10::nullopt,
               c10::nullopt, 0);
}

void beam_gather(const Tensor& gidx, const Tensor& latest, const Tensor& c_src, const Tensor& h_src,
                 const Tensor& ctx_src, const Tensor& a_src, const OT& cov_src, const Tensor& XGtab, const Tensor& Xtab,
                 const Tensor& c_out, const Tensor& h_out, const Tensor& ctx_out, const Tensor& ctxb_out,
                 const OT& cov_out, const Tensor& XG_out, const Tensor& x_out, int64_t R, int64_t H, int64_t A,
                 int64_t T, int64_t E, int64_t V, int64_t unk, const OT& step) {
  chko(step, I32, 1, "step");
  chk(gidx, I32, "gidx"); chk(latest, I32, "latest"); chk(c_src, F32, "c_src"); chk(h_src, BF, "h_src");
  chk(ctx_src, F32, "ctx_src"); chk(a_src, F32, "a_src"); chk(XGtab, F32, "XGtab"); chk(Xtab, F32, "Xtab");
  chk(c_out, F32, "c_out"); chk(h_out, BF, "h_out"); chk(ctx_out, F32, "ctx_out"); chk(ctxb_out, BF, "ctxb_out");
  chk(XG_out, F32, "XG_out"); chk(x_out, F32, "x_out");
  numel_eq(gidx, R, "gidx"); numel_eq(latest, R, "latest"); numel_eq(c_src, R * H, "c_src"); numel_eq(h_src, R * H, "h_src");
  numel_eq(ctx_src, R * A, "ctx_src"); numel_eq(a_src, R * T, "a_src"); numel_eq(XGtab, V * 4 * H, "XGtab");
  numel_eq(Xtab, V * E, "Xtab"); numel_eq(c_out, R * H, "c_out"); numel_eq(h_out, R * H, "h_out");
  numel_eq(ctx_out, R * A, "ctx_out"); numel_eq(ctxb_out, R * A, "ctxb_out"); numel_eq(XG_out, R * 4 * H, "XG_out");
  numel_eq(x_out, R * E, "x_out"); chko(cov_src, F32, R * T, "cov_src"); chko(cov_out, F32, R * T, "cov_out");
  TORCH_CHECK(unk >= 0 && unk < V, "bad unk id");
  TORCH_CHECK(!PO<float>(cov_out) || PO<float>(cov_src), "coverage gather needs cov_src");
  launch_beam_gather(P<int>(gidx), P<int>(latest), P<float>(c_src), P<bf16>(h_src), P<float>(ctx_src), P<float>(a_src),
                     PO<float>(cov_src), P<float>(XGtab), P<float>(Xtab), P<float>(c_out), P<bf16>(h_out),
                     P<float>(ctx_out), P<bf16>(ctxb_out), PO<float>(cov_out), P<float>(XG_out), P<float>(x_out), R, H,
                     A, T, E, V, unk, PO<int>(step), stream());
}

void linear2(const Tensor& a1, int64_t K1, const OT& a2, int64_t K2, const Tensor& Wt, const OT& bias, const OT& add,
             const OT& out, const OT& outb, int64_t B, int64_t N) {
  chk(a1, BF, "a1"); chk(Wt, BF, "Wt");
  TORCH_CHECK(K1 % 32 == 0 && K2 % 32 == 0 && N % 16 == 0 && K1 > 0, "linear2: K multiples of 32, N of 16");
  TORCH_CHECK((K2 == 0) == !(a2.has_value() && a2->defined()), "linear2: a2 given iff K2 > 0");
  numel_eq(a1, B * K1, "a1"); chko(a2, BF, B * K2, "a2"); numel_eq(Wt, N * (K1 + K2), "Wt");
  chko(bias, F32, N, "bias"); chko(add, F32, B * N, "add"); chko(out, F32, B * N, "out"); chko(outb, BF, B * N, "outb");
  TORCH_CHECK(PO<float>(out) || PO<bf16>(outb), "linear2 needs an output");
  launch_linear2(P<bf16>(a1), K1, PO<bf16>(a2), K2, P<bf16>(Wt), PO<float>(bias), PO<float>(add), PO<float>(out),
                 PO<bf16>(outb), B, N, stream());
}

static void linear2_check(const Tensor& a1, int64_t K1, const OT& a2, int64_t K2, const Tensor& Wt, const OT& bias,
                          const OT& add, const OT& out, const OT& outb, int64_t B, int64_t N) {
  chk(a1, BF, "a1"); chk(Wt, BF, "Wt");
  TORCH_CHECK(K1 % 32 == 0 && K2 % 32 == 0 && N % 16 == 0 && K1 > 0, "linear2: K multiples of 32, N of 16");
  TORCH_CHECK((K2 == 0) == !(a2.has_value() && a2->defined()), "linear2: a2 given iff K2 > 0");
  numel_eq(a1, B * K1, "a1"); chko(a2, BF, B * K2, "a2"); numel_eq(Wt, N * (K1 + K2), "Wt");
  chko(bias, F32, N, "bias"); chko(add, F32, B * N, "add"); chko(out, F32, B * N, "out"); chko(outb, BF, B * N, "outb");
  TORCH_CHECK(PO<float>(out) || PO<bf16>(outb), "linear2 needs an output");
}
void linear2_pair(const Tensor& a1, int64_t K1, const OT& a2, int64_t K2, const Tensor& Wt, const OT& bias,
                  const OT& add, const OT& out, const OT& outb, int64_t N, const Tensor& c1, int64_t L1, const OT& c2,
                  int64_t L2, const Tensor& Vt, const OT& vbias, const OT& vadd, const OT& vout, const OT& voutb,
                  int64_t M, int64_t B) {
  linear2_check(a1, K1, a2, K2, Wt, bias, add, out, outb, B, N);
  linear2_check(c1, L1, c2, L2, Vt, vbias, vadd, vout, voutb, B, M);
  launch_linear2_pair(P<bf16>(a1), K1, PO<bf16>(a2), K2, P<bf16>(Wt), PO<float>(bias), PO<float>(add), PO<float>(out),
                      PO<bf16>(outb), N, P<bf16>(c1), L1, PO<bf16>(c2), L2, P<bf16>(Vt), PO<float>(vbias),
                      PO<float>(vadd), PO<float>(vout), PO<bf16>(voutb), M, B, stream());
}

void pgen(const Tensor& ctx, const Tensor& c, const Tensor& h, const Tensor& x, const Tensor& w, const Tensor& b,
          const Tensor& pg, int64_t R, int64_t A, int64_t H, int64_t E) {
  chk(ctx, F32, "ctx"); chk(c, F32, "c"); chk(h, BF, "h"); chk(x, F32, "x"); chk(w, F32, "w"); chk(b, F32, "b");
  chk(pg, F32, "pg");
  numel_eq(ctx, R * A, "ctx"); numel_eq(c, R * H, "c"); numel_eq(h, R * H, "h"); numel_eq(x, R * E, "x");
  numel_eq(w, A + 2 * H + E, "w"); numel_eq(b, 1, "b"); numel_eq(pg, R, "pg");
  launch_pgen(P<float>(ctx), P<float>(c), P<bf16>(h), P<float>(x), P<float>(w), P<float>(b), P<float>(pg), R, A, H, E,
              stream());
}

void pgen_bwd(const Tensor& ctx, const Tensor& c, const Tensor& h, const Tensor& x, const Tensor& dpre,
              const Tensor& gw, int64_t N, int64_t A, int64_t H, int64_t E, bool det) {
  chk(ctx, F32, "ctx"); chk(c, F32, "c"); chk(h, BF, "h"); chk(x, F32, "x"); chk(dpre, F32, "dpre");
  chk(gw, F32, "gw");
  numel_eq(ctx, N * A, "ctx"); numel_eq(c, N * H, "c"); numel_eq(h, N * H, "h"); numel_eq(x, N * E, "x");
  numel_eq(dpre, N, "dpre"); numel_eq(gw, A + 2 * H + E, "gw");
  (void)det;
  const int64_t Kt = A + 2 * H + E, S = pgen_bwd_splits((int)N, (int)A, (int)H, (int)E);
  auto part = at::empty({S, Kt}, gw.options());
  auto cpart = at::empty({(int64_t)colsum_det_chunks((int)S, (int)Kt), Kt}, gw.options());
  launch_pgen_bwd(P<float>(ctx), P<float>(c), P<bf16>(h), P<float>(x), P<float>(dpre), P<float>(gw), P<float>(part),
                  P<float>(cpart), N, A, H, E, stream());
}

void pgen_dirs(const Tensor& dpre, const Tensor& w, const Tensor& dctx, const Tensor& dc, const Tensor& dh,
               const Tensor& dx, const OT& gb, int64_t N, int64_t A, int64_t H, int64_t E) {
  chk(dpre, F32, "dpre"); chk(w, F32, "w"); chk(dctx, F32, "dctx"); chk(dc, F32, "dc"); chk(dh, F32, "dh");
  chk(dx, F32, "dx"); chko(gb, F32, 1, "gb");
  numel_eq(dpre, N, "dpre"); numel_eq(w, A + 2 * H + E, "w"); numel_eq(dctx, N * A, "dctx"); numel_eq(dc, N * H, "dc");
  numel_eq(dh, N * H, "dh"); numel_eq(dx, N * E, "dx");
  launch_pgen_dirs(P<float>(dpre), P<float>(w), P<float>(dctx), P<float>(dc), P<float>(dh), P<float>(dx), PO<float>(gb),
                   (int)N, (int)A, (int)H, (int)E, stream());
}

}

TORCH_LIBRARY(tsamd, m) {
  m.def("lstm_enc_fwd_step", &lstm_enc_fwd_step);
  m.def("lstm_enc_bwd_step", &lstm_enc_bwd_step);
  m.def("lstm_persistent_grid", &lstm_persistent_grid_op);
  m.def("lstm_persistent_capacity", &lstm_persistent_capacity_op);
  m.def("lstm_persistent_launches", &lstm_persistent_launches_op);
  m.def("rs_fwd", &rs_fwd);
  m.def("vocab_topk_pg", &vocab_topk_pg);
  m.def("rs_bwd", &rs_bwd);
  m.def("lstm_persistent_xbuf", &lstm_persistent_xbuf_op);
  m.def("lstm_fwd_persistent", &lstm_fwd_persistent);
  m.def("lstm_fwd_persistent_fx", &lstm_fwd_persistent_fx);
  m.def("lstm_persistent_fx_ok", &lstm_persistent_fx_ok_op);
  m.def("lstm_bwd_persistent", &lstm_bwd_persistent);
  m.def("attn_score", &attn_score);
  m.def("attn_softmax_ctx", &attn_softmax_ctx);
  m.def("attn_bwd_step", &attn_bwd_step);
  m.def("attn_row_ok", &attn_row_ok);
  m.def("attn_fwd_row", &attn_fwd_row);
  m.def("attn_bwd_row", &attn_bwd_row);
  m.def("attn_rowp_ok", &attn_rowp_ok);
  m.def("attn_fwd_rowp", &attn_fwd_rowp);
  m.def("dec_persistent_ok", &dec_persistent_ok_op);
  m.def("dec_persistent_grid", &dec_persistent_grid_op);
  m.def("dec_persistent_capacity", &dec_persistent_capacity_op);
  m.def("dec_persistent_xbuf", &dec_persistent_xbuf_op);
  m.def("dec_fwd_persistent", &dec_fwd_persistent);
  m.def("attn_bwd_rowp", &attn_bwd_rowp);
  m.def("attn_bwd_feat", &attn_bwd_feat);
  m.def("attn_chunks", &attn_chunks);
  m.def("dec_cell_fwd", &dec_cell_fwd);
  m.def("dec_sproj", &dec_sproj);
  m.def("dec_bwd_cell", &dec_bwd_cell);
  m.def("dec_bwd_dz", &dec_bwd_dz);
  m.def("ptr_loss", &ptr_loss);
  m.def("wgrad_tn", &wgrad_tn);
  m.def("wgrad_tt", &wgrad_tt);
  m.def("ctx_bmm_ok", &ctx_bmm_ok_op);
  m.def("ctx_fwd", &ctx_fwd);
  m.def("ctx_da", &ctx_da);
  m.def("ctx_de", &ctx_de);
  m.def("wgrad_tt_ws", &wgrad_tt_ws);
  m.def("pgen_dirs", &pgen_dirs);
  m.def("pack_cast", &pack_cast);
  m.def("pack_max_jobs", &pack_max_jobs_op);
  m.def("pack_job_cols", &pack_job_cols_op);
  m.def("debug_enabled", &debug_enabled);
  m.def("debug_status", &debug_status);
  m.def("debug_clear", &debug_clear);
  m.def("gemm_bt_ok", &gemm_bt_ok);
  m.def("gemm_bt", &gemm_bt);
  m.def("gemm_bt_splitk_ws", &gemm_bt_splitk_ws);
  m.def("gemm_bt_splitk", &gemm_bt_splitk);
  m.def("gemm_bt_merge", &gemm_bt_merge);
  m.def("cu_hold_max_lds", &cu_hold_max_lds_op);
  m.def("cu_hold", &cu_hold);
  m.def("tanh_eval", &tanh_eval);
  m.def("tanh_tput", &tanh_tput);
  m.def("vocab_train_tiles", &vocab_train_tiles_op);
  m.def("vocab_train_fwd", &vocab_train_fwd);
  m.def("vocab_train_bwd", &vocab_train_bwd);
  m.def("emb_grad", &emb_grad);
  m.def("emb_grad_sorted", &emb_grad_sorted);
  m.def("emb_grad_det", &emb_grad_det);
  m.def("emb_grad_det_chunks", &emb_grad_det_chunks_op);
  m.def("to_step_frame", &to_step_frame);
  m.def("from_step_frame", &from_step_frame);
  m.def("transpose_bta", &transpose_bta);
  m.def("tr01", &tr01);
  m.def("linear2_pair", &linear2_pair);
  m.def("cast_colsum", &cast_colsum);
  m.def("colsum", &colsum);
  m.def("step_frame_hop", &step_frame_hop);
  m.def("ptr_rowfin", &ptr_rowfin);
  m.def("clip_adagrad", &clip_adagrad);
  m.def("opt_parts", &opt_parts);
  m.def("final_topk", &final_topk);
  m.def("topk_parts", &topk_parts);
  m.def("beam_step", &beam_step);
  m.def("beam_step_ng", &beam_step_ng);
  m.def("beam_gather", &beam_gather);
  m.def("linear2", &linear2);
  m.def("pgen", &pgen);
  m.def("vocab_topk", &vocab_topk);
  m.def("vocab_topk_parts", &vocab_topk_parts);
  m.def("vocab_span_probe", &vocab_span_probe);
  m.def("attn_fwd_row_probe", &attn_fwd_row_probe);
  m.def("vocab_select_stamps", &vocab_select_stamps);
  m.def("lstm_bwd_stamps", &lstm_bwd_stamps);
  m.def("vocab_topk_beam", &vocab_topk_beam);
  m.def("vocab_topk_beam_ng", &vocab_topk_beam_ng);
  m.def("dec_cell_fwd_beam", &dec_cell_fwd_beam);
  m.def("beam_sproj_xmerge", &beam_sproj_xmerge);
  m.def("attn_fwd_row_beam", &attn_fwd_row_beam);
  m.def("pgen_bwd", &pgen_bwd);
}
```

csrc/kernels/attn_rowp_fwd.h:

```cpp
#pragma once
#include "attn_common.h"

namespace attn_rowp {

typedef uint32_t u32x4 __attribute__((ext_vector_type(4)));
constexpr int kRowMaxT = 2048;
constexpr int kEG = 128;

template <int NK>
struct Rows {
  u32x4 x[NK][4];
};

template <int NK>
__device__ __forceinline__ void load_rows(Rows<NK>& r, const bf16* base, int p0, int len, int lane) {
  constexpr int A = 512 * NK;
#pragma unroll
  for (int q = 0; q < 4; ++q) {
    const int p = min(p0 + q, len - 1);
#pragma unroll
    for (int kb = 0; kb < NK; ++kb)
      r.x[kb][q] = __builtin_bit_cast(u32x4, ld8(base + (size_t)p * A + kb * 512 + lane * 8));
  }
}

template <int NK, int NW, typename OnG>
__device__ __forceinline__ void attn_fwd_rowp_body(
    const bf16* __restrict__ F, const bf16* __restrict__ G, const float* srow, const float* __restrict__ v,
    const float* __restrict__ wc, const float* cov, const int* __restrict__ lens, float* __restrict__ a_out,
    float* cov_out, float* __restrict__ covloss, float* __restrict__ gx, bf16* __restrict__ gx_bf, int T,
    const int* __restrict__ dlen, int step, bf16* __restrict__ a_bf, int b, float* es, float (*part)[4][kEG],
    float* wm, float* wl, float* red, OnG on_g) {
  const Dot2Sel dsel = dot2_sel();
  constexpr int A = 512 * NK, NT = NW * 64;
  const int tid = threadIdx.x, wid = tid >> 6, lane = tid & 63;
  const int len = (int)DCHECK_IDX(lens[b], 1, T + 1, CHK_ATTN_LEN);
  const size_t rb = (size_t)b * T;
  if (dlen && step >= dlen[b]) {
    for (int i = tid; i < T; i += NT) {
      a_out[rb + i] = 0.f;
      if (a_bf) a_bf[rb + i] = f2bf(0.f);
      if (cov_out) cov_out[rb + i] = cov ? cov[rb + i] : 0.f;
    }
    for (int k = tid; k < kEG; k += NT) {
      gx[(size_t)b * kEG + k] = 0.f;
      gx_bf[(size_t)b * kEG + k] = f2bf(0.f);
      on_g(k, 0.f);
    }
    if (covloss && tid == 0) covloss[b] = 0.f;
    return;
  }
  const bf16* Fb = F + (size_t)b * T * A;
  const bf16* Gb = G + (size_t)b * T * kEG + (lane & 15) * 8;
  const int ngrp = (len + 3) >> 2;
  const int qm = lane >> 4;
  const int b5 = (lane >> 5) & 1, b4 = (lane >> 4) & 1;
  Rows<NK> fA, fB;
  u32x4 gA, gB;
  float cA = 0.f, cB = 0.f;
  auto load = [&](int grp, Rows<NK>& f, u32x4& gq, float& c) {
    load_rows<NK>(f, Fb, 4 * grp, len, lane);
    const int p = min(4 * grp + qm, len - 1);
    gq = __builtin_bit_cast(u32x4, ld8(Gb + (size_t)p * kEG));
    c = cov ? cov[rb + p] : 0.f;
  };
  if (wid < ngrp) load(wid, fA, gA, cA);
  f32x2 s2[NK][4], w2[NK][4], v2[NK][4], acc[4];
  float vsum = 0.f;
#pragma unroll
  for (int kb = 0; kb < NK; ++kb) {
    const int k0 = kb * 512 + lane * 8;
#pragma unroll
    for (int jp = 0; jp < 4; ++jp) {
      const float2 sv = *reinterpret_cast<const float2*>(srow + k0 + 2 * jp);
      const float2 vv = *reinterpret_cast<const float2*>(v + k0 + 2 * jp);
      const float2 wv = wc ? *reinterpret_cast<const float2*>(wc + k0 + 2 * jp) : make_float2(0.f, 0.f);
      s2[kb][jp] = f32x2{sv.x, sv.y} * K2LOG2E;
      w2[kb][jp] = f32x2{wv.x, wv.y} * K2LOG2E;
      v2[kb][jp] = f32x2{vv.x, vv.y};
      vsum += vv.x + vv.y;
    }
  }
#pragma unroll
  for (int jp = 0; jp < 4; ++jp) acc[jp] = f32x2{0.f, 0.f};
  float m_w = -INFINITY, l_l = 0.f;
  auto compute = [&](int grp, const Rows<NK>& f, const u32x4& gq, float c_l) {
    float pd[4];
#pragma unroll
    for (int q = 0; q < 4; ++q) {
      const float c = rdlane(c_l, 16 * q);
      f32x2 d2 = f32x2{0.f, 0.f};
#pragma unroll
      for (int kb = 0; kb < NK; ++kb)
#pragma unroll
        for (int jp = 0; jp < 4; ++jp) {
          const f32x2 y = fadd_bf2(f.x[kb][q][jp], fma2(w2[kb][jp], splat2(c), s2[kb][jp]), dsel);
          d2 = fma2(v2[kb][jp], rsig2(y), d2);
        }
      pd[q] = vsum - 2.0f * (d2.x + d2.y);
    }
    float eq = bfly4(pd, b5, b4);
    const int p = 4 * grp + qm;
    if (p >= len) eq = -INFINITY;
    if ((lane & 15) == 0 && p < len) es[p] = eq;
    const float e0 = rdlane(eq, 0), e1 = rdlane(eq, 16), e2 = rdlane(eq, 32), e3 = rdlane(eq, 48);
    const float mn = fmaxf(m_w, fmaxf(fmaxf(e0, e1), fmaxf(e2, e3)));
    const float sc = m_w == -INFINITY ? 0.f : fexp(m_w - mn);
    const float pq = fexp(eq - mn);
    l_l = fmaf(l_l, sc, pq);
#pragma unroll
    for (int jp = 0; jp < 4; ++jp) acc[jp] = fma2(bf2pair(gq[jp]), splat2(pq), acc[jp] * sc);
    m_w = mn;
  };
  for (int g = wid; g < ngrp;) {
    const int g1 = g + NW;
    if (g1 < ngrp) load(g1, fB, gB, cB);
    compute(g, fA, gA, cA);
    if (g1 >= ngrp) break;
    const int g2 = g1 + NW;
    if (g2 < ngrp) load(g2, fA, gA, cA);
    compute(g1, fB, gB, cB);
    g = g2;
  }
  const float lw = (rdlane(l_l, 0) + rdlane(l_l, 16)) + (rdlane(l_l, 32) + rdlane(l_l, 48));
  if (lane == 0) {
    wm[wid] = m_w;
    wl[wid] = lw;
  }
#pragma unroll
  for (int jp = 0; jp < 4; ++jp)
    *reinterpret_cast<float2*>(&part[wid][qm][(lane & 15) * 8 + 2 * jp]) = make_float2(acc[jp].x, acc[jp].y);
  __syncthreads();
  float m = -INFINITY;
#pragma unroll
  for (int w = 0; w < NW; ++w) m = fmaxf(m, wm[w]);
  float L = 0.f, wsc[NW];
#pragma unroll
  for (int w = 0; w < NW; ++w) {
    wsc[w] = wm[w] == -INFINITY ? 0.f : fexp(wm[w] - m);
    L += wl[w] * wsc[w];
  }
  const float invL = 1.0f / L;
  for (int k = tid; k < kEG; k += NT) {
    float c = 0.f;
#pragma unroll
    for (int w = 0; w < NW; ++w) c += ((part[w][0][k] + part[w][1][k]) + (part[w][2][k] + part[w][3][k])) * wsc[w];
    c *= invL;
    gx[(size_t)b * kEG + k] = c;
    gx_bf[(size_t)b * kEG + k] = f2bf(c);
    on_g(k, c);
  }
  float cl = 0.f;
  for (int i = tid; i < T; i += NT) {
    const float a = i < len ? fexp(es[i] - m) * invL : 0.f;
    a_out[rb + i] = a;
    if (a_bf) a_bf[rb + i] = f2bf(a);
    if (cov_out) {
      const float c = cov ? cov[rb + i] : 0.f;
      cov_out[rb + i] = c + a;
      cl += fminf(a, c);
    }
  }
  if (covloss) {
    cl = block_sum<NT>(cl, red);
    if (tid == 0) covloss[b] = cl;
  }
}

}
```

csrc/kernels/decoder_persistent.hip:

```cpp
#include "attn_rowp_fwd.h"
#include "handoff.h"
#include "launchers.h"
#include <mutex>

using namespace attn_rowp;
using namespace handoff;

namespace {

constexpr int kH = 256, kE = 128, kA = 512, kNC = 16, kNW = 16, kNT = kNW * 64;
constexpr int kKc = kE + kH;
constexpr int kWcS = kKc + 8, kWsS = 2 * kH + 8;
constexpr int kChS = 2 * kH + 8, kGtS = kE + 8;
constexpr int kGg = 16 * (kE / 2), kGch = 16 * kH, kGs = 16 * kA;
constexpr int kTeamGranules = 2 * (kGg + kGch + kGs);
constexpr int oWc = 0;
constexpr int oWs = oWc + 64 * kWcS * 2;
constexpr int oCh = oWs + 32 * kWsS * 2;
constexpr int oGt = oCh + 16 * kChS * 2;
constexpr int oEs = oGt + 16 * kGtS * 2;
constexpr int oPart = oEs + kRowMaxT * 4;
constexpr int oSrow = oPart + kNW * 4 * kEG * 4;
constexpr int oMisc = oSrow + kA * 4;
constexpr int kLds = oMisc + 3 * kNW * 4;
static_assert(oWs % 16 == 0 && oCh % 16 == 0 && oGt % 16 == 0 && oEs % 16 == 0 && oPart % 16 == 0 && oSrow % 16 == 0 &&
              oMisc % 16 == 0, "LDS carve alignment");
static_assert(kLds <= 160 * 1024, "LDS of one CU");
static_assert(4 * 4 * 256 * 4 <= kNW * 4 * kEG * 4, "K-split partials fit the attention partial buffer");

}

struct DecPersistentArgs {
  const float* XG;
  const bf16* KcT;
  const bf16* WsT;
  const float* bs;
  float* Cst;
  bf16* Cb;
  bf16* Hb;
  float* ACT;
  float* S;
  const bf16* F;
  const bf16* G;
  const float* v;
  const float* wc;
  float* COV;
  const int* lens;
  float* ATT;
  bf16* ATTb;
  float* covloss;
  float* GV;
  bf16* GVb;
  const int* dlen;
  gu64* xbuf;
  gu32* err;
  int B, T, D;
};

__global__ __launch_bounds__(kNT) void dec_fwd_persistent_kernel(DecPersistentArgs p) {
  extern __shared__ __attribute__((aligned(16))) char smem[];
  bf16* Wc = reinterpret_cast<bf16*>(smem + oWc);
  bf16* Ws = reinterpret_cast<bf16*>(smem + oWs);
  bf16* ch = reinterpret_cast<bf16*>(smem + oCh);
  bf16* gt = reinterpret_cast<bf16*>(smem + oGt);
  float* es = reinterpret_cast<float*>(smem + oEs);
  float(*part)[4][kEG] = reinterpret_cast<float(*)[4][kEG]>(smem + oPart);
  float* red = reinterpret_cast<float*>(smem + oPart);
  float* srow = reinterpret_cast<float*>(smem + oSrow);
  float* wm = reinterpret_cast<float*>(smem + oMisc);
  float* wl = wm + kNW;
  float* redw = wl + kNW;

  const int B = p.B, T = p.T, D = p.D;
  int team, j;
  if (!team_of(kNC, B / 16, team, j)) return;
  const int tid = threadIdx.x, wid = tid >> 6, lane = tid & 63;
  const int r0 = team * 16, b = r0 + j;
  const int l15 = lane & 15, kof = 8 * (lane >> 4);
  gu64* gbuf = p.xbuf + (size_t)team * kTeamGranules;
  gu64* chbuf = gbuf + 2 * kGg;
  gu64* sbuf = chbuf + 2 * kGch;

  int tile_last = D, row_last = D;
  if (p.dlen) {
    tile_last = 0;
    for (int i = 0; i < 16; ++i) tile_last = max(tile_last, p.dlen[r0 + i]);
    tile_last = min(tile_last, D);
    row_last = p.dlen[b];
  }

  for (int i = tid; i < 64 * (kKc / 8); i += kNT) {
    const int row = i / (kKc / 8), c8 = i % (kKc / 8);
    const int grow = (row >> 4) * kH + 16 * j + (row & 15);
    *reinterpret_cast<bf16x8*>(Wc + row * kWcS + c8 * 8) = ld8(p.KcT + (size_t)grow * kKc + c8 * 8);
  }
  for (int i = tid; i < 32 * (2 * kH / 8); i += kNT) {
    const int row = i / (2 * kH / 8), c8 = i % (2 * kH / 8);
    *reinterpret_cast<bf16x8*>(Ws + row * kWsS + c8 * 8) = ld8(p.WsT + (size_t)(32 * j + row) * (2 * kH) + c8 * 8);
  }
  if (tid < 16 * (kH / 8)) {
    const int row = tid / (kH / 8), c8 = tid % (kH / 8);
    *reinterpret_cast<bf16x8*>(ch + row * kChS + kH + c8 * 8) = ld8(p.Hb + (size_t)(r0 + row) * kH + c8 * 8);
  }
  const int crow = (lane >> 4) * 4 + (wid & 3), cu = 16 * j + l15;
  const size_t cri = (size_t)(r0 + crow) * kH + cu;
  float cstate = wid < 4 ? p.Cst[cri] : 0.f;
  const size_t BH = (size_t)B * kH, BT = (size_t)B * T;
  bool dead = false;

  for (int t = 0; t < tile_last; ++t) {
    const unsigned tag = (unsigned)t + 1u;
    const int par = t & 1;
    const bf16 *Fp = p.F, *Gp = p.G;
    const float *vp = p.v, *wcp = p.wc;
    asm volatile("" : "+s"(Fp), "+s"(Gp), "+s"(vp), "+s"(wcp));
    float xg[4] = {0.f, 0.f, 0.f, 0.f};
    if (wid < 4) {
      const float* xr = p.XG + ((size_t)t * B + r0 + crow) * (4 * kH);
#pragma unroll
      for (int g = 0; g < 4; ++g) xg[g] = xr[g * kH + cu];
    }
    if (t > 0) {
      unsigned gv[1] = {0u};
      sweep<1>(gbuf + (par ^ 1) * kGg, wid * 64, tag - 1u, gv, dead, p.err, 3u, lane);
      *reinterpret_cast<unsigned*>(gt + wid * kGtS + 2 * lane) = gv[0];
    }
    __syncthreads();
    {
      const int gate = wid & 3, ks = wid >> 2;
      const int ib = t > 0 ? 0 : kE / 32, nst = kKc / 32 - ib;
      const int i0 = ib + ks * nst / 4, i1 = ib + (ks + 1) * nst / 4;
      const bf16* wrow = Wc + (gate * 16 + l15) * kWcS + kof;
      const bf16* grow = gt + l15 * kGtS + kof;
      const bf16* hrow = ch + l15 * kChS + kH - kE + kof;
      f32x4 acc = f32x4{0, 0, 0, 0};
      for (int i = i0; i < i1; ++i) {
        const int k = 32 * i;
        const bf16x8 a = k < kE ? ld8(grow + k) : ld8(hrow + k);
        acc = mfma16(a, ld8(wrow + k), acc);
      }
#pragma unroll
      for (int r = 0; r < 4; ++r) red[((ks * 4 + gate) * 4 + r) * 64 + lane] = acc[r];
    }
    __syncthreads();
    if (wid < 4) {
      float z[4];
#pragma unroll
      for (int g = 0; g < 4; ++g) {
        float s = 0.f;
#pragma unroll
        for (int src = 0; src < 4; ++src) s += red[((src * 4 + g) * 4 + wid) * 64 + lane];
        z[g] = s;
      }
      const float ig = fsigmoid(z[0] + xg[0]), jg = ftanh(z[1] + xg[1]);
      const float fg = fsigmoid(z[2] + xg[2] + 1.0f), og = fsigmoid(z[3] + xg[3]);
      const float c = fg * cstate + ig * jg;
      const float h = og * ftanh(c);
      cstate = c;
      store_granule(chbuf + par * kGch + crow * kH + cu, tag, pack_bf2(c, h));
      const size_t o = (size_t)(t + 1) * BH + cri;
      p.Cst[o] = c;
      p.Cb[o] = f2bf(c);
      p.Hb[o] = f2bf(h);
      float* a4 = p.ACT + ((size_t)t * B + r0 + crow) * (4 * kH);
      a4[cu] = ig; a4[kH + cu] = jg; a4[2 * kH + cu] = fg; a4[3 * kH + cu] = og;
    }
    {
      unsigned cv[4] = {0u, 0u, 0u, 0u};
      sweep<4>(chbuf + par * kGch, wid * kH, tag, cv, dead, p.err, 3u, lane);
      unsigned short* crw = reinterpret_cast<unsigned short*>(ch + wid * kChS);
#pragma unroll
      for (int q = 0; q < 4; ++q) {
        crw[q * 64 + lane] = (unsigned short)(cv[q] & 0xffffu);
        crw[kH + q * 64 + lane] = (unsigned short)(cv[q] >> 16);
      }
    }
    __syncthreads();
    if (wid < 8) {
      const int nt = wid & 1, ks = wid >> 1;
      const bf16* arow = ch + l15 * kChS + kof;
      const bf16* wrow = Ws + (nt * 16 + l15) * kWsS + kof;
      f32x4 acc = f32x4{0, 0, 0, 0};
#pragma unroll
      for (int i = 4 * ks; i < 4 * ks + 4; ++i) acc = mfma16(ld8(arow + 32 * i), ld8(wrow + 32 * i), acc);
#pragma unroll
      for (int r = 0; r < 4; ++r) red[((ks * 2 + nt) * 4 + r) * 64 + lane] = acc[r];
    }
    __syncthreads();
    if (wid < 8) {
      const int w = wid & 3, nt = wid >> 2;
      float o = 0.f;
#pragma unroll
      for (int src = 0; src < 4; ++src) o += red[((src * 2 + nt) * 4 + w) * 64 + lane];
      const int row = (lane >> 4) * 4 + w, n = 32 * j + nt * 16 + l15;
      const float sv = o + p.bs[n] + 0.f;
      store_granule(sbuf + par * kGs + row * kA + n, tag, __float_as_uint(sv));
      p.S[((size_t)t * B + r0 + row) * kA + n] = sv;
    }
    if (t < row_last && wid < 8) {
      unsigned sv[1] = {0u};
      sweep<1>(sbuf + par * kGs + j * kA, wid * 64, tag, sv, dead, p.err, 3u, lane);
      srow[wid * 64 + lane] = __uint_as_float(sv[0]);
    }
    __syncthreads();
    gu64* gdst = gbuf + par * kGg + j * (kE / 2);
    attn_fwd_rowp_body<1, kNW>(
        Fp, Gp, srow, vp, wcp, (p.COV && t > 0) ? p.COV + (size_t)t * BT : nullptr, p.lens,
        p.ATT + (size_t)t * BT, p.COV ? p.COV + (size_t)(t + 1) * BT : nullptr,
        p.covloss ? p.covloss + (size_t)t * B : nullptr, p.GV + (size_t)t * B * kE, p.GVb + (size_t)t * B * kE, T,
        p.dlen, t, p.ATTb + (size_t)t * BT, b, es, part, wm, wl, redw, [&](int k, float g) {
          const float gn = __shfl_xor(g, 1, 64);
          if (!(k & 1)) store_granule(gdst + (k >> 1), tag, pack_bf2(g, gn));
        });
  }
  for (int t = tile_last; t < D; ++t) {
    if (wid < 4) {
      const size_t o = (size_t)(t + 1) * BH + cri;
      p.Cst[o] = 0.f;
      p.Cb[o] = f2bf(0.f);
      p.Hb[o] = f2bf(0.f);
      float* a4 = p.ACT + ((size_t)t * B + r0 + crow) * (4 * kH);
      a4[cu] = 0.f; a4[kH + cu] = 0.f; a4[2 * kH + cu] = 0.f; a4[3 * kH + cu] = 0.f;
    }
    __syncthreads();
    attn_fwd_rowp_body<1, kNW>(
        p.F, p.G, srow, p.v, p.wc, (p.COV && t > 0) ? p.COV + (size_t)t * BT : nullptr, p.lens,
        p.ATT + (size_t)t * BT, p.COV ? p.COV + (size_t)(t + 1) * BT : nullptr,
        p.covloss ? p.covloss + (size_t)t * B : nullptr, p.GV + (size_t)t * B * kE, p.GVb + (size_t)t * B * kE, T,
        p.dlen, t, p.ATTb + (size_t)t * BT, b, es, part, wm, wl, redw, [](int, float) {});
  }
}

bool dec_persistent_shape_ok(int H, int E, int A, int B, int T) {
  return H == kH && E == kE && A == kA && B >= 16 && B % 16 == 0 && T >= 1 && T <= kRowMaxT;
}

int dec_persistent_grid(int B) { return B >= 16 && B % 16 == 0 ? 8 * kNC * ((B / 16 + 7) / 8) : 0; }

size_t dec_persistent_xbuf_elems(int B) { return (size_t)(B / 16) * kTeamGranules; }

int dec_persistent_capacity() {
  static std::mutex mu;
  static int cache[64] = {};
  int dev = 0;
  if (hipGetDevice(&dev) != hipSuccess || dev < 0 || dev >= 64) return 0;
  std::lock_guard<std::mutex> lock(mu);
  if (cache[dev]) return cache[dev] - 1;
  int cus = 0, occ = 0;
  if (hipDeviceGetAttribute(&cus, hipDeviceAttributeMultiprocessorCount, dev) != hipSuccess) cus = 0;
  bool ok = hipFuncSetAttribute(reinterpret_cast<const void*>(dec_fwd_persistent_kernel),
                                hipFuncAttributeMaxDynamicSharedMemorySize, kLds) == hipSuccess;
  ok = ok && hipOccupancyMaxActiveBlocksPerMultiprocessor(&occ, dec_fwd_persistent_kernel, kNT, kLds) == hipSuccess;
  const int cap = (ok && occ >= 1) ? cus : 0;
  cache[dev] = cap + 1;
  return cap;
}

void launch_dec_fwd_persistent(const float* XG, const bf16* KcT, const bf16* WsT, const float* bs, float* Cst, bf16* Cb,
                               bf16* Hb, float* ACT, float* S, const bf16* F, const bf16* G, const float* v,
                               const float* wc, float* COV, const int* lens, float* ATT, bf16* ATTb, float* covloss,
                               float* GV, bf16* GVb, const int* dlen, unsigned long long* xbuf, unsigned* err, int B,
                               int T, int D, hipStream_t st) {
  const int grid = dec_persistent_grid(B);
  if (grid <= 0 || grid > dec_persistent_capacity()) return;
  DecPersistentArgs p{XG, KcT, WsT, bs, Cst, Cb, Hb, ACT, S, F, G, v, wc, COV, lens, ATT, ATTb, covloss, GV, GVb, dlen,
                      (gu64*)xbuf, (gu32*)err, B, T, D};
  hipLaunchKernelGGL(dec_fwd_persistent_kernel, dim3(grid), dim3(kNT), kLds, st, p);
}
```

csrc/kernels/handoff.h:

```cpp
#pragma once
#include "common.h"

#define RLX_AGENT __ATOMIC_RELAXED, __HIP_MEMORY_SCOPE_AGENT

namespace handoff {

typedef __attribute__((address_space(1))) unsigned long long gu64;
typedef __attribute__((address_space(1))) unsigned int gu32;
constexpr unsigned kSpinLimit = 1u << 21;

__device__ __forceinline__ unsigned pack_bf2(float lo, float hi) {
  const unsigned a = __builtin_bit_cast(unsigned short, f2bf(lo));
  const unsigned b = __builtin_bit_cast(unsigned short, f2bf(hi));
  return a | (b << 16);
}

__device__ __forceinline__ void store_granule(gu64* g, unsigned tag, unsigned v) {
  __hip_atomic_store(g, ((unsigned long long)tag << 32) | v, RLX_AGENT);
}

template <int NPL>
__device__ __forceinline__ void sweep(const gu64* g, int first, unsigned tag, unsigned (&v)[NPL], bool& dead,
                                      gu32* err, unsigned code, int lane) {
  static_assert(NPL <= 32, "ready mask is 32 bits");
  constexpr unsigned all = NPL == 32 ? 0xffffffffu : ((1u << NPL) - 1);
  unsigned ready = 0;
  unsigned long long x[NPL];
  for (unsigned spins = 0;;) {
#pragma unroll
    for (int j = 0; j < NPL; ++j)
      if (!((ready >> j) & 1)) x[j] = __hip_atomic_load(g + first + j * 64 + lane, RLX_AGENT);
#pragma unroll
    for (int j = 0; j < NPL; ++j)
      if (!((ready >> j) & 1) && (unsigned)(x[j] >> 32) == tag) {
        v[j] = (unsigned)x[j];
        ready |= 1u << j;
      }
    if (__all(ready == all) || dead) return;
    if (++spins > kSpinLimit / 4) {
      if (lane == 0) __hip_atomic_store(err, code, RLX_AGENT);
      dead = true;
      return;
    }
    __builtin_amdgcn_s_sleep(24);
  }
}

__device__ __forceinline__ bool team_of(int NC, int nteams, int& team, int& c) {
  const int xcd = blockIdx.x & 7, q = blockIdx.x >> 3;
  team = (q / NC) * 8 + xcd;
  c = q % NC;
  return team < nteams;
}

}
```

csrc/kernels/launchers.h:

```cpp
#pragma once
#include <hip/hip_runtime.h>
typedef __bf16 bf16;

void launch_lstm_enc_fwd_step(const float* gx, const float* bias, const bf16* Wt, bf16* hs, float* cs, float* acts, bf16* out,
                              const int* lens, int s, int T, int B, int H, hipStream_t st);
void launch_lstm_enc_bwd_step(bf16* dz, const bf16* Wn, const float* dout, const float* dh_fin, float* dc_carry,
                              const float* acts, const float* cs, const int* lens, int s, int T, int B, int H,
                              hipStream_t st);

void launch_attn_score(const bf16* F, const float* s, const float* v, const float* wc, const float* cov,
                       const int* lens, float* e, int B, int T, int A, int rep, hipStream_t st);
void launch_attn_softmax_ctx(const float* e, const bf16* E, const int* lens, const float* cov, float* a_out,
                             float* cov_out, float* covloss, float* ctx, bf16* ctx_bf, int B, int T, int A, int rep,
                             hipStream_t st);
int attn_nchunk(int T);
void launch_attn_bwd_step(const bf16* E, const bf16* F, const float* s, const float* v, const float* wc,
                          const float* cov, const float* a, const float* dctx, const float* ctx, const float* Ga,
                          const float* dcov_next, const float* gcl, const int* lens, float* de_out, float* ds,
                          float* dcov_out, int B, int T, int A, hipStream_t st);
void launch_attn_bwd_feat(const bf16* F, const float* S_all, const float* v, const float* wc, const float* cov_all,
                          const float* de_all, const int* lens, bf16* dF, float* dv, float* dwc, int D, int B, int T,
                          int A, int nslot, hipStream_t st, const int* dlen = nullptr);

bool attn_row_supported(int A, int T);
void launch_attn_fwd_row_probe(const bf16* F, const bf16* E, const float* s, const float* v, const float* wc,
                               const float* cov, const int* lens, float* a_out, float* ctx, int B, int T, int rep,
                               int probe, hipStream_t st);
void launch_attn_fwd_row(const bf16* F, const bf16* E, const float* s, const float* v, const float* wc,
                         const float* cov, const int* lens, float* a_out, float* cov_out, float* covloss, float* ctx,
                         bf16* ctx_bf, int B, int T, int A, int rep, hipStream_t st, const int* cg = nullptr,
                         const float* asrc = nullptr, float* cov_keep = nullptr);
void launch_attn_bwd_row(const bf16* E, const bf16* F, const float* s, const float* v, const float* wc,
                         const float* cov, const float* a, const float* dctx, const float* ctx, const float* Ga,
                         const float* dcov_next, const float* gcl, const int* lens, float* de_out, float* ds,
                         float* dcov_out, int B, int T, int A, hipStream_t st);

bool attn_rowp_supported(int A, int T, int EG);
void launch_attn_fwd_rowp(const bf16* F, const bf16* G, const float* s, const float* v, const float* wc,
                          const float* cov, const int* lens, float* a_out, float* cov_out, float* covloss, float* gx,
                          bf16* gx_bf, int B, int T, int A, const int* dlen, int step, hipStream_t st,
                          bf16* a_bf = nullptr);
void launch_attn_bwd_rowp(const bf16* G, const bf16* F, const float* s, const float* v, const float* wc,
                          const float* cov, const float* a, const float* dx, const float* gv, const float* Ga,
                          const float* dcov_next, const float* gcl, const int* lens, float* de_out, float* ds,
                          float* dcov_out, int B, int T, int A, const int* dlen, int step, hipStream_t st);

void launch_dec_cell_fwd(const float* XG, const bf16* ctxp, const bf16* hprev, const float* cprev, const bf16* WcT,
                         float* c_out, bf16* cb_out, bf16* hb_out, float* act, int B, int H, int A, const int* dlen,
                         int step, hipStream_t st);
void launch_dec_cell_fwd_beam(const int* gidx, const int* latest, const float* XGtab, const bf16* ctxp,
                              const bf16* hprev, const float* cprev, const bf16* WcT, float* c_out, bf16* cb_out,
                              bf16* hb_out, int* step, int B, int H, int A, int V, int unk, hipStream_t st);
void launch_beam_sproj_xmerge(const bf16* cb, const bf16* hb, const bf16* WsT, const float* bs, float* s_out,
                              const bf16* ctx_src, const bf16* WicT, const float* Xtab, const int* gidx,
                              const int* latest, float* x_out, int B, int H, int A, int E, int V, int unk,
                              hipStream_t st);
void launch_dec_sproj(const bf16* cb, const bf16* hb, const bf16* WsT, const float* bs, float* s_out, int B, int H,
                      int A, const int* dlen, int step, hipStream_t st);
bool dec_persistent_shape_ok(int H, int E, int A, int B, int T);
int dec_persistent_grid(int B);
int dec_persistent_capacity();
size_t dec_persistent_xbuf_elems(int B);
void launch_dec_fwd_persistent(const float* XG, const bf16* KcT, const bf16* WsT, const float* bs, float* Cst, bf16* Cb,
                               bf16* Hb, float* ACT, float* S, const bf16* F, const bf16* G, const float* v,
                               const float* wc, float* COV, const int* lens, float* ATT, bf16* ATTb, float* covloss,
                               float* GV, bf16* GVb, const int* dlen, unsigned long long* xbuf, unsigned* err, int B,
                               int T, int D, hipStream_t st);
void launch_dec_bwd_cell(const float* ds, const bf16* Ws, const float* dC_dir, const float* dH_dir,
                         const float* dh_rec, float* dc_carry, const float* act, const float* c_now,
                         const float* c_prev, bf16* dz, int B, int H, int A, const int* dlen, int step,
                         hipStream_t st);
void launch_dec_bwd_dz(const bf16* dz, const bf16* Wbig, const float* dX_dir, const float* dCTX_dir_prev,
                       float* dx_out, float* dctx_prev_out, float* dh_rec, int B, int E, int H, int A,
                       const int* dlen, int step, hipStream_t st);

void launch_ptr_loss_bf16(const bf16* logits, const int* target, const float* rowg, const float* pgen,
                          const float* attn, const int* ext, const int* lens, float* loss_row, bf16* dlogits,
                          float* dpre, float* dA, int N, int B, int T, int V, hipStream_t st);
int ptr_loss_bf16_max_vocab();
void launch_ptr_loss(const float* logits, const float* bias, const int* target, const float* rowg, const float* pgen, const float* attn,
                     const int* ext, const int* lens, float* loss_row, bf16* dlogits, float* dpre, float* dA, int N,
                     int B, int T, int V, hipStream_t st);

void launch_clip_adagrad(float* w, float* acc, const float* g, long n, float* part, float lr, float max_norm,
                         float gscale, float* norm_out, int* flag, const int* skip, hipStream_t st);
int opt_nparts();

void launch_final_topk(const float* logits, const float* bias, const float* pgen, const float* attn, const int* ext,
                       const int* lens, int* out_ids, float* out_lp, float* part_ms, float* part_v, int* part_i, int R,
                       int V, int T, int K, int beam, hipStream_t st);
#define NG_BAN_MAX 4096
struct NgSeq {
  int* seq[2];
  int P;
  int n;
};
int topk_split(int V);
void launch_beam_step(const int* top_ids, const float* top_lp, float* lp_sum, int* latest, int* gidx, int* tok_hist,
                      int* par_hist, int* done, int* res_count, float* res_score, int* res_len, int* res_step,
                      int* res_par, int* step, unsigned* ctr, const float* att, float* att_hist, const float* pg,
                      float* pg_hist, int T, int Na, int beam, int K, int stop_id, int min_dec, int max_dec,
                      hipStream_t st, const NgSeq* ng = nullptr);
void launch_beam_gather(const int* gidx, const int* latest, const float* c_src, const bf16* h_src,
                        const float* ctx_src, const float* a_src, const float* cov_src, const float* XGtab,
                        const float* Xtab, float* c_out, bf16* h_out, float* ctx_out, bf16* ctxb_out, float* cov_out,
                        float* XG_out, float* x_out, int R, int H, int A, int T, int E, int V, int unk,
                        int* step, hipStream_t st);
void launch_linear2(const bf16* a1, int K1, const bf16* a2, int K2, const bf16* Wt, const float* bias,
                    const float* add, float* out, bf16* outb, int B, int N, hipStream_t st);
void launch_linear2_pair(const bf16* a1, int K1, const bf16* a2, int K2, const bf16* Wt, const float* bias,
                         const float* add, float* out, bf16* outb, int N, const bf16* c1, int L1, const bf16* c2,
                         int L2, const bf16* Vt, const float* vbias, const float* vadd, float* vout, bf16* voutb,
                         int M, int B, hipStream_t st);
void launch_pgen(const float* ctx, const float* c, const bf16* h, const float* x, const float* w, const float* b,
                 float* pg, int R, int A, int H, int E, hipStream_t st);
int pgen_bwd_splits(int N, int A, int H, int E);
void launch_pgen_bwd(const float* ctx, const float* c, const bf16* h, const float* x, const float* dpre, float* gw,
                     float* part, float* cpart, int N, int A, int H, int E, hipStream_t st);
int lstm_persistent_grid(int H, int B);
int lstm_persistent_capacity(int H);
int lstm_persistent_launches(int H, int B);
size_t lstm_persistent_xbuf_elems(int H, int B, bool bwd);
void launch_lstm_fwd_persistent(const float* gx, const float* bias, const bf16* Wt, bf16* hs, float* cs, float* acts,
                                bf16* out, const int* lens, unsigned long long* xbuf, unsigned* err, int T, int B,
                                int H, hipStream_t st, const bf16* xsf = nullptr, const bf16* Wx0 = nullptr,
                                const bf16* Wx1 = nullptr);
bool lstm_persistent_fx_ok(int H, int B, int E);
void launch_lstm_bwd_persistent(bf16* dz, const bf16* Wn, const float* dout, const float* dh_fin, float* dc_carry,
                                const float* acts, const float* cs, const int* lens, unsigned long long* xbuf,
                                unsigned* err, float* dbias, int T, int B, int H, bool dout_bf, hipStream_t st,
                                bool dout_bf16 = false);
int vocab_topk_tiles(int V, int H);
void set_vocab_select_stamps(unsigned long long* buf);
void launch_vocab_span_probe(const bf16* X, const bf16* WT, const float* bias, float* logits, float* part_ms, int R, int V,
                             int probe, hipStream_t st);


struct BeamTail {
  float* lp_sum; int* latest; int* gidx; int* tok_hist; int* par_hist; int* done; int* res_count;
  float* res_score; int* res_len; int* res_step; int* res_par; int* step;
  unsigned* art_ctr;
  unsigned long long* gran;
  int* err;
  const float* att; float* att_hist; const float* pg; float* pg_hist;
  int T, Na, beam, K, stop_id, min_dec, max_dec;
};
struct PgIn {
  const float* ctx; const float* c; const bf16* h; const float* x; const float* w; const float* b; float* out;
  int A, H, E;
};
void launch_vocab_topk(const bf16* X, const bf16* WT, const float* bias, const float* pgen, const float* attn,
                       const int* ext, const int* lens, int* out_ids, float* out_lp, float* logits, float* part_ms,
                       int R, int V, int H, int T, int K, int beam, PgIn pgi, hipStream_t st,
                       const BeamTail* bt = nullptr, const NgSeq* ng = nullptr);
int vocab_train_tiles(int V, int H);
void launch_vocab_train_fwd(const bf16* X, int ldx, const bf16* WT, const float* bias, const int* target, float* part,
                            float* zg, float* lse, float* pv, int N, int V, int H, const int* vblk, const int* vblk_n,
                            hipStream_t st);
void launch_vocab_train_bwd(const bf16* X, int ldx, const bf16* WT, const float* bias, const int* target,
                            const float* lse, const float* alpha, bf16* dl, int ldd, float* dbias, int N, int V, int H,
                            const int* vblk, const int* vblk_n, const int* vlive, int* vstate, hipStream_t st);
void launch_ptr_rowfin(const float* pv, const int* target, const float* rowg, const float* pgen, const float* attn,
                       const int* ext, const int* lens, float* loss_row, float* alpha, float* dpre, float* dA, int N,
                       int B, int T, hipStream_t st);

void launch_rs_fwd(const float* c_fw, const bf16* h_fw, size_t dstride, const bf16* RCt, const bf16* RHt,
                   const float* bc, const float* bh, float* pre_c, float* pre_h, float* c0, bf16* c0b, bf16* h0b,
                   bf16* cat_c, bf16* cat_h, int B, int H, hipStream_t st);
void launch_rs_bwd(const float* gc, const float* gh, const float* pre_c, const float* pre_h, const bf16* RC,
                   const bf16* RH, bf16* dpc, bf16* dph, float* gbc, float* gbh, float* dold_c, float* dold_h,
                   size_t dstride, int B, int H, hipStream_t st);

void launch_emb_grad(float* gemb, const int64_t* ids0, const float* src0, int n0, const int64_t* ids1,
                     const float* src1, int n1, int E, int V, hipStream_t st);

void launch_to_step_frame(const void* src, int es, const int64_t* ids, const int64_t* rev, void* out, int B, int T,
                          int W, int S, int doff, long nsrc, hipStream_t st);
void launch_from_step_frame(const float* in, const int64_t* rev, float* out, int B, int T, int W, hipStream_t st);
void launch_step_frame_hop(const float* in, const int64_t* rev, float* out, int B, int T, int H, hipStream_t st);
void launch_transpose_bta(const bf16* in, bf16* out, int B, int T, int A, hipStream_t st);
void launch_tr01(const float* in, float* out, bf16* outb, int P, int Q, int R, bool acc, hipStream_t st);
int cast_colsum_blocks(int N, int C);
void launch_cast_colsum(const float* x, bf16* xb, float* part, float* colsum, int N, int C, hipStream_t st);
int colsum_det_chunks(int N, int C);
void launch_colsum_det(const void* x, bool bf, float* part, float* out, int N, int C, bool acc, hipStream_t st);
void launch_emb_grad_sorted(float* gemb, const int* sid, const int* perm, const float* src0, int n0,
                            const float* src1, int n1, int E, int V, hipStream_t st);
int emb_grad_det_chunks(int n);
void launch_emb_grad_det(float* gemb, const int* sid, const int* perm, const float* src0, int n0, const float* src1,
                         int n1, int E, int V, float* pf, float* pl, hipStream_t st);

int tsamd_debug_enabled();
void tsamd_debug_read(unsigned* out4);
void tsamd_debug_clear();

int wgrad_tn_splits(int M, int N, int K);
int wgrad_tt_splits(int M, int N, int K);
bool wgrad_tt_ok(int M, int N, int K);
void launch_wgrad_tt(const bf16* a, int lda, const bf16* b, int ldb, float* slab, float* out, int ldo, int M, int N,
                     int K, bool trans, bool acc, int nv, hipStream_t st);
bool wgrad_tt_direct(int M, int N, int K, bool trans, bool acc);
void launch_wgrad_tn(const bf16* a, int lda, const bf16* b, int ldb, float* out, int ldo, int M, int N, int K,
                     hipStream_t st);

int pack_max_jobs();
int pack_job_cols();
void launch_pack_cast(const long* jobs, int nj, long total, hipStream_t st);

void launch_pgen_dirs(const float* dpre, const float* w, float* dctx, float* dc, float* dh, float* dx, float* gb,
                      int N, int A, int H, int E, hipStream_t st);

int cu_hold_max_lds();
void launch_cu_hold(int grid, unsigned long long ticks, long long* times, int lds_bytes, hipStream_t st);
void launch_tanh_eval(const float* x, float* t, float* s2, int n, int mode, hipStream_t st);
void launch_tanh_tput(const float* in, float* out, int threads, int iters, int mode, hipStream_t st);

bool gemm_bt_supported(int M, int N, int K, int BN);
int gemm_bt_splits(int M, int N, int K);
void launch_gemm_bt_splitk(const bf16* A, long lda, const bf16* Bt, long ldb, float* slab, float* out, long ldo, int M,
                           int N, int K, bool acc, hipStream_t st);
void launch_slab_sum(const float* slab, float* out, int ldo, int M, int N, int S, bool acc, hipStream_t st);
void launch_gemm_bt(const bf16* A, long lda, const bf16* Bt, long ldb, void* C, long ldc, bool out_bf16, bool beta,
                    const float* bias, int M, int N, int K, int amode, const int64_t* ids, const int64_t* rev,
                    bf16* xsf, long nsrc, int B, int T, int dir, hipStream_t st);

bool ctx_bmm_ok(int B, int T, int D, int A);
void launch_ctx_fwd(const bf16* att, const bf16* enc, float* ctx, bf16* ctxb, int B, int T, int D, int A, hipStream_t st);
void launch_ctx_da(const bf16* dctx, const bf16* enc, float* da, int B, int T, int D, int A, bool acc, hipStream_t st);
void launch_ctx_de(const bf16* att, const bf16* dctx, float* de, bf16* deb, int B, int T, int D, int A, hipStream_t st);

void set_lstm_bwd_stamps(unsigned long long* buf);
```

textsummarization_on_flink_amd/_build.py:

```python
from __future__ import annotations

import concurrent.futures as cf
import os
import subprocess
import sys
import sysconfig

PKG_DIR = os.path.dirname(os.path.abspath(__file__))
REPO = os.path.dirname(PKG_DIR)
CSRC = os.path.join(REPO, "csrc")
BUILD = os.path.join(REPO, "build", "obj")
ARCH = os.environ.get("PYTORCH_ROCM_ARCH", "gfx950")
HIPCC = os.environ.get("HIPCC", "/opt/rocm/bin/hipcc")
CXX = os.environ.get("CXX", "g++")


def _torch_flags():
    import torch
    import torch.utils.cpp_extension as ce

    inc = ce.include_paths(device_type="cuda")
    libs = ce.library_paths(device_type="cuda")
    abi = int(torch._C._GLIBCXX_USE_CXX11_ABI)
    cflags = [f"-I{p}" for p in inc] + [
        f"-I{sysconfig.get_paths()['include']}",
        f"-D_GLIBCXX_USE_CXX11_ABI={abi}",
        "-DTORCH_EXTENSION_NAME=_C",
    ]
    ldflags = [f"-L{p}" for p in libs] + [f"-Wl,-rpath,{p}" for p in libs] + [
        "-lc10", "-ltorch", "-ltorch_cpu", "-lc10_hip", "-ltorch_hip", "-lamdhip64",
    ]
    return cflags, ldflags


def _newer(src_list, dst):
    if not os.path.exists(dst):
        return True
    t = os.path.getmtime(dst)
    return any(os.path.getmtime(s) > t for s in src_list)


def _run(cmd, verbose):
    if verbose:
        print(" ".join(cmd), flush=True)
    r = subprocess.run(cmd, capture_output=True, text=True)
    if r.returncode != 0:
        raise RuntimeError(f"build failed: {' '.join(cmd)}\n{r.stdout}\n{r.stderr}")
    if verbose and r.stderr.strip():
        print(r.stderr, flush=True)


def _headers(d):
    out = []
    for root, _, files in os.walk(d):
        out += [os.path.join(root, f) for f in files if f.endswith((".h", ".hpp", ".cuh"))]
    return out


def build_kernels(verbose=False, jobs=8, debug=False):
    bdir = BUILD + ("_debug" if debug else "")
    os.makedirs(bdir, exist_ok=True)
    kdir = os.path.join(CSRC, "kernels")
    hips = sorted(os.path.join(kdir, f) for f in os.listdir(kdir) if f.endswith(".hip"))
    hdrs = _headers(kdir)
    common = ["-O3", "-std=c++17", "-fPIC", f"--offload-arch={ARCH}", "-ffp-contract=fast",
              "-Wno-unused-result", "-munsafe-fp-atomics", f"-I{kdir}"]
    if debug:
        common += ["-DTSAMD_DEBUG", "-fgpu-rdc"]
    objs, jobsl = [], []
    for src in hips:
        obj = os.path.join(bdir, os.path.basename(src) + ".o")
        objs.append(obj)
        if _newer([src] + hdrs, obj):
            jobsl.append([HIPCC, *common, "-c", src, "-o", obj])
    tflags, tld = _torch_flags()
    for host in ("bindings.cpp", "blt_gemm.cpp"):
        bsrc = os.path.join(CSRC, host)
        bobj = os.path.join(bdir, host.replace(".cpp", ".o"))
        objs.append(bobj)
        if _newer([bsrc] + hdrs, bobj):
            jobsl.append([HIPCC, "-O2", "-std=c++17", "-fPIC", f"-I{kdir}", *tflags, "-c", bsrc, "-o", bobj])
    with cf.ThreadPoolExecutor(max_workers=jobs) as ex:
        list(ex.map(lambda c: _run(c, verbose), jobsl))
    so = os.path.join(PKG_DIR, "_C_debug.so" if debug else "_C.so")
    if jobsl or not os.path.exists(so):
        link = [HIPCC, "-shared", "-fPIC", f"--offload-arch={ARCH}"] + (["-fgpu-rdc"] if debug else [])
        _run([*link, *objs, "-o", so, *tld, "-lhipblaslt"], verbose)
    return so


def build_runtime(verbose=False):
    os.makedirs(BUILD, exist_ok=True)
    rdir = os.path.join(CSRC, "runtime")
    srcs = sorted(os.path.join(rdir, f) for f in os.listdir(rdir) if f.endswith(".cpp"))
    so = os.path.join(PKG_DIR, "_rt.so")
    if not srcs:
        return None
    if _newer(srcs + _headers(rdir), so):
        _run([CXX, "-O2", "-std=c++17", "-fPIC", "-shared", "-pthread", f"-I{rdir}", *srcs,
              "-o", so, "-lrt"], verbose)
    return so


def build(verbose=False, debug=True):
    rt = build_runtime(verbose)
    c = build_kernels(verbose)
    if debug:
        build_kernels(verbose, debug=True)
    return rt, c


if __name__ == "__main__":
    print(build(verbose="-v" in sys.argv, debug="--no-debug" not in sys.argv))
```

Baseline: 7.510 million tokens/s.

## Restructure persistent decoder step into phases with LDS-resident attention vectors and coverage

The persistent decoder kernel is split into scoped phases that re-read kernel arguments from the kernarg segment and re-derive thread ids, which keeps long-lived registers down across the time loop. The attention vector v, the scaled coverage weight and the running coverage row now stay resident in LDS instead of being re-read from global memory each step. The rowp attention body is made generic over a source/hooks policy so the decoder can defer its LSTM state stores into the attention phase and reuse the dead-row path. Optional wall-clock stamping is added behind a compile flag. The change costs extra LDS and adds complexity in how coverage state flows between steps.

```diff
diff --git a/csrc/bindings.cpp b/csrc/bindings.cpp
--- a/csrc/bindings.cpp
+++ b/csrc/bindings.cpp
@@ -203,6 +203,15 @@
 int64_t dec_persistent_grid_op(int64_t B) { return dec_persistent_grid((int)B); }
 int64_t dec_persistent_capacity_op() { return dec_persistent_capacity(); }
 int64_t dec_persistent_xbuf_op(int64_t B) { return (int64_t)dec_persistent_xbuf_elems((int)B); }
+int64_t dec_persistent_stamps_op(const OT& buf, int64_t B, int64_t D) {
+  if (buf.has_value()) {
+    chk(*buf, I32, "stamps");
+    TORCH_CHECK(buf->numel() >= dec_persistent_grid((int)B) * D * 8, "stamps too small");
+  }
+  const int n = dec_persistent_stamps_into(buf.has_value() ? (unsigned*)buf->data_ptr() : nullptr);
+  TORCH_CHECK(n > 0, "dec_persistent_stamps: this library was built without -DTSAMD_DEC_STAMPS");
+  return n;
+}
 void dec_fwd_persistent(const Tensor& XG, const Tensor& KcT, const Tensor& WsT, const Tensor& bs, const Tensor& Cst,
                         const Tensor& Cb, const Tensor& Hb, const Tensor& ACT, const Tensor& S, const Tensor& F,
                         const Tensor& G, const Tensor& v, const OT& wc, const OT& COV, const Tensor& lens,
@@ -1177,6 +1186,7 @@
   m.def("dec_persistent_grid", &dec_persistent_grid_op);
   m.def("dec_persistent_capacity", &dec_persistent_capacity_op);
   m.def("dec_persistent_xbuf", &dec_persistent_xbuf_op);
+  m.def("dec_persistent_stamps", &dec_persistent_stamps_op);
   m.def("dec_fwd_persistent", &dec_fwd_persistent);
   m.def("attn_bwd_rowp", &attn_bwd_rowp);
   m.def("attn_bwd_feat", &attn_bwd_feat);
diff --git a/csrc/kernels/attn_rowp_fwd.h b/csrc/kernels/attn_rowp_fwd.h
--- a/csrc/kernels/attn_rowp_fwd.h
+++ b/csrc/kernels/attn_rowp_fwd.h
@@ -24,30 +24,63 @@
   }
 }
 
-template <int NK, int NW, typename OnG>
-__device__ __forceinline__ void attn_fwd_rowp_body(
-    const bf16* __restrict__ F, const bf16* __restrict__ G, const float* srow, const float* __restrict__ v,
-    const float* __restrict__ wc, const float* cov, const int* __restrict__ lens, float* __restrict__ a_out,
-    float* cov_out, float* __restrict__ covloss, float* __restrict__ gx, bf16* __restrict__ gx_bf, int T,
-    const int* __restrict__ dlen, int step, bf16* __restrict__ a_bf, int b, float* es, float (*part)[4][kEG],
-    float* wm, float* wl, float* red, OnG on_g) {
+struct GlobalSrc {
+  const float* __restrict__ v;
+  const float* __restrict__ wc;
+  const float* cov;
+  __device__ __forceinline__ float2 v2(int k) const { return *reinterpret_cast<const float2*>(v + k); }
+  __device__ __forceinline__ f32x2 w2(int k) const {
+    const float2 wv = wc ? *reinterpret_cast<const float2*>(wc + k) : make_float2(0.f, 0.f);
+    return f32x2{wv.x, wv.y} * K2LOG2E;
+  }
+  __device__ __forceinline__ float cov_at(size_t rb, int p) const { return cov ? cov[rb + p] : 0.f; }
+  __device__ __forceinline__ void cov_set(int, float) const {}
+};
+
+template <typename OnG>
+struct OnGHooks {
+  OnG on_g;
+  __device__ __forceinline__ int tid() const { return threadIdx.x; }
+  __device__ __forceinline__ void early() const {}
+  __device__ __forceinline__ void mark(int) const {}
+};
+
+template <int NW, typename Src, typename Hooks>
+__device__ __forceinline__ void attn_fwd_rowp_dead(const Src src, float* __restrict__ a_out, float* cov_out,
+                                                   float* __restrict__ covloss, float* __restrict__ gx,
+                                                   bf16* __restrict__ gx_bf, int T, bf16* __restrict__ a_bf, int b,
+                                                   Hooks hk) {
+  constexpr int NT = NW * 64;
+  const int tid = hk.tid();
+  const size_t rb = (size_t)b * T;
+  for (int k = tid; k < kEG; k += NT) {
+    gx[(size_t)b * kEG + k] = 0.f;
+    gx_bf[(size_t)b * kEG + k] = f2bf(0.f);
+    hk.on_g(k, 0.f);
+  }
+  hk.mark(1);
+  for (int i = tid; i < T; i += NT) {
+    a_out[rb + i] = 0.f;
+    if (a_bf) a_bf[rb + i] = f2bf(0.f);
+    if (cov_out) cov_out[rb + i] = src.cov_at(rb, i);
+  }
+  if (covloss && tid == 0) covloss[b] = 0.f;
+}
+
+template <int NK, int NW, typename Src, typename Hooks>
+__device__ __forceinline__ void attn_fwd_rowp_core(
+    const bf16* __restrict__ F, const bf16* __restrict__ G, const float* srow, const Src src,
+    const int* __restrict__ lens, float* __restrict__ a_out, float* cov_out, float* __restrict__ covloss,
+    float* __restrict__ gx, bf16* __restrict__ gx_bf, int T, const int* __restrict__ dlen, int step,
+    bf16* __restrict__ a_bf, int b, float* es, float (*part)[4][kEG], float* wm, float* wl, float* red, Hooks hk) {
   const Dot2Sel dsel = dot2_sel();
   constexpr int A = 512 * NK, NT = NW * 64;
-  const int tid = threadIdx.x, wid = tid >> 6, lane = tid & 63;
+  const int tid = hk.tid(), wid = tid >> 6, lane = tid & 63;
   const int len = (int)DCHECK_IDX(lens[b], 1, T + 1, CHK_ATTN_LEN);
   const size_t rb = (size_t)b * T;
   if (dlen && step >= dlen[b]) {
-    for (int i = tid; i < T; i += NT) {
-      a_out[rb + i] = 0.f;
-      if (a_bf) a_bf[rb + i] = f2bf(0.f);
-      if (cov_out) cov_out[rb + i] = cov ? cov[rb + i] : 0.f;
-    }
-    for (int k = tid; k < kEG; k += NT) {
-      gx[(size_t)b * kEG + k] = 0.f;
-      gx_bf[(size_t)b * kEG + k] = f2bf(0.f);
-      on_g(k, 0.f);
-    }
-    if (covloss && tid == 0) covloss[b] = 0.f;
+    hk.early();
+    attn_fwd_rowp_dead<NW>(src, a_out, cov_out, covloss, gx, gx_bf, T, a_bf, b, hk);
     return;
   }
   const bf16* Fb = F + (size_t)b * T * A;
@@ -62,9 +95,10 @@
     load_rows<NK>(f, Fb, 4 * grp, len, lane);
     const int p = min(4 * grp + qm, len - 1);
     gq = __builtin_bit_cast(u32x4, ld8(Gb + (size_t)p * kEG));
-    c = cov ? cov[rb + p] : 0.f;
+    c = src.cov_at(rb, p);
   };
   if (wid < ngrp) load(wid, fA, gA, cA);
+  hk.early();
   f32x2 s2[NK][4], w2[NK][4], v2[NK][4], acc[4];
   float vsum = 0.f;
 #pragma unroll
@@ -73,10 +107,9 @@
 #pragma unroll
     for (int jp = 0; jp < 4; ++jp) {
       const float2 sv = *reinterpret_cast<const float2*>(srow + k0 + 2 * jp);
-      const float2 vv = *reinterpret_cast<const float2*>(v + k0 + 2 * jp);
-      const float2 wv = wc ? *reinterpret_cast<const float2*>(wc + k0 + 2 * jp) : make_float2(0.f, 0.f);
+      const float2 vv = src.v2(k0 + 2 * jp);
       s2[kb][jp] = f32x2{sv.x, sv.y} * K2LOG2E;
-      w2[kb][jp] = f32x2{wv.x, wv.y} * K2LOG2E;
+      w2[kb][jp] = src.w2(k0 + 2 * jp);
       v2[kb][jp] = f32x2{vv.x, vv.y};
       vsum += vv.x + vv.y;
     }
@@ -122,6 +155,7 @@
     compute(g1, fB, gB, cB);
     g = g2;
   }
+  hk.mark(0);
   const float lw = (rdlane(l_l, 0) + rdlane(l_l, 16)) + (rdlane(l_l, 32) + rdlane(l_l, 48));
   if (lane == 0) {
     wm[wid] = m_w;
@@ -138,26 +172,29 @@
 #pragma unroll
   for (int w = 0; w < NW; ++w) {
     wsc[w] = wm[w] == -INFINITY ? 0.f : fexp(wm[w] - m);
-    L += wl[w] * wsc[w];
+    L = __builtin_fmaf(wl[w], wsc[w], L);
   }
   const float invL = 1.0f / L;
   for (int k = tid; k < kEG; k += NT) {
     float c = 0.f;
 #pragma unroll
-    for (int w = 0; w < NW; ++w) c += ((part[w][0][k] + part[w][1][k]) + (part[w][2][k] + part[w][3][k])) * wsc[w];
+    for (int w = 0; w < NW; ++w)
+      c = __builtin_fmaf((part[w][0][k] + part[w][1][k]) + (part[w][2][k] + part[w][3][k]), wsc[w], c);
     c *= invL;
     gx[(size_t)b * kEG + k] = c;
     gx_bf[(size_t)b * kEG + k] = f2bf(c);
-    on_g(k, c);
-  }
+    hk.on_g(k, c);
+  }
+  hk.mark(1);
   float cl = 0.f;
   for (int i = tid; i < T; i += NT) {
     const float a = i < len ? fexp(es[i] - m) * invL : 0.f;
     a_out[rb + i] = a;
     if (a_bf) a_bf[rb + i] = f2bf(a);
     if (cov_out) {
-      const float c = cov ? cov[rb + i] : 0.f;
+      const float c = src.cov_at(rb, i);
       cov_out[rb + i] = c + a;
+      src.cov_set(i, c + a);
       cl += fminf(a, c);
     }
   }
@@ -167,4 +204,15 @@
   }
 }
 
-}
+template <int NK, int NW, typename OnG>
+__device__ __forceinline__ void attn_fwd_rowp_body(
+    const bf16* __restrict__ F, const bf16* __restrict__ G, const float* srow, const float* __restrict__ v,
+    const float* __restrict__ wc, const float* cov, const int* __restrict__ lens, float* __restrict__ a_out,
+    float* cov_out, float* __restrict__ covloss, float* __restrict__ gx, bf16* __restrict__ gx_bf, int T,
+    const int* __restrict__ dlen, int step, bf16* __restrict__ a_bf, int b, float* es, float (*part)[4][kEG],
+    float* wm, float* wl, float* red, OnG on_g) {
+  attn_fwd_rowp_core<NK, NW>(F, G, srow, GlobalSrc{v, wc, cov}, lens, a_out, cov_out,
+                             covloss, gx, gx_bf, T, dlen, step, a_bf, b, es, part, wm, wl, red, OnGHooks<OnG>{on_g});
+}
+
+}
diff --git a/csrc/kernels/decoder_persistent.hip b/csrc/kernels/decoder_persistent.hip
--- a/csrc/kernels/decoder_persistent.hip
+++ b/csrc/kernels/decoder_persistent.hip
@@ -14,6 +14,8 @@
 constexpr int kChS = 2 * kH + 8, kGtS = kE + 8;
 constexpr int kGg = 16 * (kE / 2), kGch = 16 * kH, kGs = 16 * kA;
 constexpr int kTeamGranules = 2 * (kGg + kGch + kGs);
+constexpr int kSleep = 24;
+constexpr int kStamps = 8;
 constexpr int oWc = 0;
 constexpr int oWs = oWc + 64 * kWcS * 2;
 constexpr int oCh = oWs + 32 * kWsS * 2;
@@ -22,9 +24,12 @@
 constexpr int oPart = oEs + kRowMaxT * 4;
 constexpr int oSrow = oPart + kNW * 4 * kEG * 4;
 constexpr int oMisc = oSrow + kA * 4;
-constexpr int kLds = oMisc + 3 * kNW * 4;
+constexpr int oV = oMisc + 3 * kNW * 4;
+constexpr int oWk = oV + kA * 4;
+constexpr int oCov = oWk + kA * 4;
+constexpr int kLds = oCov + kRowMaxT * 4;
 static_assert(oWs % 16 == 0 && oCh % 16 == 0 && oGt % 16 == 0 && oEs % 16 == 0 && oPart % 16 == 0 && oSrow % 16 == 0 &&
-              oMisc % 16 == 0, "LDS carve alignment");
+              oMisc % 16 == 0 && oV % 16 == 0 && oWk % 16 == 0 && oCov % 16 == 0, "LDS carve alignment");
 static_assert(kLds <= 160 * 1024, "LDS of one CU");
 static_assert(4 * 4 * 256 * 4 <= kNW * 4 * kEG * 4, "K-split partials fit the attention partial buffer");
 
@@ -54,8 +59,59 @@
   const int* dlen;
   gu64* xbuf;
   gu32* err;
+  unsigned* stamps;
   int B, T, D;
 };
+
+namespace {
+
+typedef const DecPersistentArgs __attribute__((address_space(4))) KArgs;
+__device__ __forceinline__ KArgs* phase_args() {
+  KArgs* a = (KArgs*)__builtin_amdgcn_kernarg_segment_ptr();
+  asm volatile("" : "+s"(a));
+  return a;
+}
+__device__ __forceinline__ int phase_tid() {
+  int t = threadIdx.x;
+  asm volatile("" : "+v"(t));
+  return t;
+}
+
+struct ResidentSrc {
+  const float* vl;
+  const float* wk;
+  float* covl;
+  bool has_cov;
+  __device__ __forceinline__ float2 v2(int k) const { return *reinterpret_cast<const float2*>(vl + k); }
+  __device__ __forceinline__ f32x2 w2(int k) const {
+    const float2 w = *reinterpret_cast<const float2*>(wk + k);
+    return f32x2{w.x, w.y};
+  }
+  __device__ __forceinline__ float cov_at(size_t, int p) const { return has_cov ? covl[p] : 0.f; }
+  __device__ __forceinline__ void cov_set(int i, float c) const { covl[i] = c; }
+};
+
+template <typename OnG, typename Early, typename Mark>
+struct StepHooks {
+  OnG on_g;
+  Early early_;
+  Mark mark_;
+  __device__ __forceinline__ int tid() const { return phase_tid(); }
+  __device__ __forceinline__ void early() const { early_(); }
+  __device__ __forceinline__ void mark(int i) const { mark_(i); }
+};
+template <typename OnG, typename Early, typename Mark>
+__device__ __forceinline__ StepHooks<OnG, Early, Mark> step_hooks(OnG g, Early e, Mark m) {
+  return StepHooks<OnG, Early, Mark>{g, e, m};
+}
+
+#ifdef TSAMD_DEC_STAMPS
+#define DEC_STAMP(i) (st[i] = (unsigned)wall_clock64())
+#else
+#define DEC_STAMP(i) ((void)0)
+#endif
+
+}
 
 __global__ __launch_bounds__(kNT) void dec_fwd_persistent_kernel(DecPersistentArgs p) {
   extern __shared__ __attribute__((aligned(16))) char smem[];
@@ -70,164 +126,233 @@
   float* wm = reinterpret_cast<float*>(smem + oMisc);
   float* wl = wm + kNW;
   float* redw = wl + kNW;
+  float* vl = reinterpret_cast<float*>(smem + oV);
+  float* wk = reinterpret_cast<float*>(smem + oWk);
+  float* covl = reinterpret_cast<float*>(smem + oCov);
 
   const int B = p.B, T = p.T, D = p.D;
   int team, j;
   if (!team_of(kNC, B / 16, team, j)) return;
-  const int tid = threadIdx.x, wid = tid >> 6, lane = tid & 63;
   const int r0 = team * 16, b = r0 + j;
-  const int l15 = lane & 15, kof = 8 * (lane >> 4);
-  gu64* gbuf = p.xbuf + (size_t)team * kTeamGranules;
-  gu64* chbuf = gbuf + 2 * kGg;
-  gu64* sbuf = chbuf + 2 * kGch;
-
+  const bool has_cov = p.COV != nullptr;
   int tile_last = D, row_last = D;
-  if (p.dlen) {
-    tile_last = 0;
-    for (int i = 0; i < 16; ++i) tile_last = max(tile_last, p.dlen[r0 + i]);
-    tile_last = min(tile_last, D);
-    row_last = p.dlen[b];
+  float cstate = 0.f;
+  {
+    const int tid = threadIdx.x, wid = tid >> 6, lane = tid & 63;
+    if (p.dlen) {
+      tile_last = 0;
+      for (int i = 0; i < 16; ++i) tile_last = max(tile_last, p.dlen[r0 + i]);
+      tile_last = min(tile_last, D);
+      row_last = p.dlen[b];
+    }
+    for (int i = tid; i < 64 * (kKc / 8); i += kNT) {
+      const int row = i / (kKc / 8), c8 = i % (kKc / 8);
+      const int grow = (row >> 4) * kH + 16 * j + (row & 15);
+      *reinterpret_cast<bf16x8*>(Wc + row * kWcS + c8 * 8) = ld8(p.KcT + (size_t)grow * kKc + c8 * 8);
+    }
+    for (int i = tid; i < 32 * (2 * kH / 8); i += kNT) {
+      const int row = i / (2 * kH / 8), c8 = i % (2 * kH / 8);
+      *reinterpret_cast<bf16x8*>(Ws + row * kWsS + c8 * 8) = ld8(p.WsT + (size_t)(32 * j + row) * (2 * kH) + c8 * 8);
+    }
+    if (tid < 16 * (kH / 8)) {
+      const int row = tid / (kH / 8), c8 = tid % (kH / 8);
+      *reinterpret_cast<bf16x8*>(ch + row * kChS + kH + c8 * 8) = ld8(p.Hb + (size_t)(r0 + row) * kH + c8 * 8);
+    }
+    if (tid < kA) {
+      vl[tid] = p.v[tid];
+      wk[tid] = (p.wc ? p.wc[tid] : 0.f) * K2LOG2E;
+    }
+    for (int i = tid; i < kRowMaxT; i += kNT) covl[i] = 0.f;
+    const int crow = (lane >> 4) * 4 + (wid & 3), cu = 16 * j + (lane & 15);
+    if (wid < 4) cstate = p.Cst[(size_t)(r0 + crow) * kH + cu];
   }
-
-  for (int i = tid; i < 64 * (kKc / 8); i += kNT) {
-    const int row = i / (kKc / 8), c8 = i % (kKc / 8);
-    const int grow = (row >> 4) * kH + 16 * j + (row & 15);
-    *reinterpret_cast<bf16x8*>(Wc + row * kWcS + c8 * 8) = ld8(p.KcT + (size_t)grow * kKc + c8 * 8);
-  }
-  for (int i = tid; i < 32 * (2 * kH / 8); i += kNT) {
-    const int row = i / (2 * kH / 8), c8 = i % (2 * kH / 8);
-    *reinterpret_cast<bf16x8*>(Ws + row * kWsS + c8 * 8) = ld8(p.WsT + (size_t)(32 * j + row) * (2 * kH) + c8 * 8);
-  }
-  if (tid < 16 * (kH / 8)) {
-    const int row = tid / (kH / 8), c8 = tid % (kH / 8);
-    *reinterpret_cast<bf16x8*>(ch + row * kChS + kH + c8 * 8) = ld8(p.Hb + (size_t)(r0 + row) * kH + c8 * 8);
-  }
-  const int crow = (lane >> 4) * 4 + (wid & 3), cu = 16 * j + l15;
-  const size_t cri = (size_t)(r0 + crow) * kH + cu;
-  float cstate = wid < 4 ? p.Cst[cri] : 0.f;
-  const size_t BH = (size_t)B * kH, BT = (size_t)B * T;
   bool dead = false;
+  const ResidentSrc src{vl, wk, covl, has_cov};
 
   for (int t = 0; t < tile_last; ++t) {
     const unsigned tag = (unsigned)t + 1u;
     const int par = t & 1;
-    const bf16 *Fp = p.F, *Gp = p.G;
-    const float *vp = p.v, *wcp = p.wc;
-    asm volatile("" : "+s"(Fp), "+s"(Gp), "+s"(vp), "+s"(wcp));
-    float xg[4] = {0.f, 0.f, 0.f, 0.f};
-    if (wid < 4) {
-      const float* xr = p.XG + ((size_t)t * B + r0 + crow) * (4 * kH);
-#pragma unroll
-      for (int g = 0; g < 4; ++g) xg[g] = xr[g * kH + cu];
-    }
-    if (t > 0) {
-      unsigned gv[1] = {0u};
-      sweep<1>(gbuf + (par ^ 1) * kGg, wid * 64, tag - 1u, gv, dead, p.err, 3u, lane);
-      *reinterpret_cast<unsigned*>(gt + wid * kGtS + 2 * lane) = gv[0];
-    }
-    __syncthreads();
+#ifdef TSAMD_DEC_STAMPS
+    unsigned st[kStamps] = {0u, 0u, 0u, 0u, 0u, 0u, 0u, 0u};
+#endif
+    float dc = 0.f, dh = 0.f, dgate[4] = {0.f, 0.f, 0.f, 0.f}, ds = 0.f;
     {
-      const int gate = wid & 3, ks = wid >> 2;
-      const int ib = t > 0 ? 0 : kE / 32, nst = kKc / 32 - ib;
-      const int i0 = ib + ks * nst / 4, i1 = ib + (ks + 1) * nst / 4;
-      const bf16* wrow = Wc + (gate * 16 + l15) * kWcS + kof;
-      const bf16* grow = gt + l15 * kGtS + kof;
-      const bf16* hrow = ch + l15 * kChS + kH - kE + kof;
-      f32x4 acc = f32x4{0, 0, 0, 0};
-      for (int i = i0; i < i1; ++i) {
-        const int k = 32 * i;
-        const bf16x8 a = k < kE ? ld8(grow + k) : ld8(hrow + k);
-        acc = mfma16(a, ld8(wrow + k), acc);
-      }
-#pragma unroll
-      for (int r = 0; r < 4; ++r) red[((ks * 4 + gate) * 4 + r) * 64 + lane] = acc[r];
-    }
-    __syncthreads();
-    if (wid < 4) {
-      float z[4];
-#pragma unroll
-      for (int g = 0; g < 4; ++g) {
-        float s = 0.f;
-#pragma unroll
-        for (int src = 0; src < 4; ++src) s += red[((src * 4 + g) * 4 + wid) * 64 + lane];
-        z[g] = s;
-      }
-      const float ig = fsigmoid(z[0] + xg[0]), jg = ftanh(z[1] + xg[1]);
-      const float fg = fsigmoid(z[2] + xg[2] + 1.0f), og = fsigmoid(z[3] + xg[3]);
-      const float c = fg * cstate + ig * jg;
-      const float h = og * ftanh(c);
-      cstate = c;
-      store_granule(chbuf + par * kGch + crow * kH + cu, tag, pack_bf2(c, h));
-      const size_t o = (size_t)(t + 1) * BH + cri;
-      p.Cst[o] = c;
-      p.Cb[o] = f2bf(c);
-      p.Hb[o] = f2bf(h);
-      float* a4 = p.ACT + ((size_t)t * B + r0 + crow) * (4 * kH);
-      a4[cu] = ig; a4[kH + cu] = jg; a4[2 * kH + cu] = fg; a4[3 * kH + cu] = og;
-    }
-    {
+      KArgs* a = phase_args();
+      const int tid = phase_tid(), wid = tid >> 6, lane = tid & 63;
+      const int l15 = lane & 15, kof = 8 * (lane >> 4);
+      const int crow = (lane >> 4) * 4 + (wid & 3), cu = 16 * j + l15;
+      gu64* gbuf = a->xbuf + (size_t)team * kTeamGranules;
+      if (t > 0) {
+        unsigned gv[1] = {0u};
+        sweep<1, kSleep>(gbuf + (par ^ 1) * kGg, wid * 64, tag - 1u, gv, dead, a->err, 3u, lane);
+        *reinterpret_cast<unsigned*>(gt + wid * kGtS + 2 * lane) = gv[0];
+      }
+      DEC_STAMP(0);
+      float xg[4] = {0.f, 0.f, 0.f, 0.f};
+      if (wid < 4) {
+        const float* xr = a->XG + ((size_t)t * B + r0 + crow) * (4 * kH);
+#pragma unroll
+        for (int g = 0; g < 4; ++g) xg[g] = xr[g * kH + cu];
+      }
+      __syncthreads();
+      {
+        const int gate = wid & 3, ks = wid >> 2;
+        const int ib = t > 0 ? 0 : kE / 32, nst = kKc / 32 - ib;
+        const int i0 = ib + ks * nst / 4, i1 = ib + (ks + 1) * nst / 4;
+        const bf16* wrow = Wc + (gate * 16 + l15) * kWcS + kof;
+        const bf16* grow = gt + l15 * kGtS + kof;
+        const bf16* hrow = ch + l15 * kChS + kH - kE + kof;
+        f32x4 acc = f32x4{0, 0, 0, 0};
+        for (int i = i0; i < i1; ++i) {
+          const int k = 32 * i;
+          const bf16x8 av = k < kE ? ld8(grow + k) : ld8(hrow + k);
+          acc = mfma16(av, ld8(wrow + k), acc);
+        }
+#pragma unroll
+        for (int r = 0; r < 4; ++r) red[((ks * 4 + gate) * 4 + r) * 64 + lane] = acc[r];
+      }
+      __syncthreads();
+      gu64* chbuf = gbuf + 2 * kGg;
+      if (wid < 4) {
+        float z[4];
+#pragma unroll
+        for (int g = 0; g < 4; ++g) {
+          float s = 0.f;
+#pragma unroll
+          for (int sl = 0; sl < 4; ++sl) s += red[((sl * 4 + g) * 4 + wid) * 64 + lane];
+          z[g] = s;
+        }
+        const float ig = fsigmoid(z[0] + xg[0]), jg = ftanh(z[1] + xg[1]);
+        const float fg = fsigmoid(z[2] + xg[2] + 1.0f), og = fsigmoid(z[3] + xg[3]);
+        const float c = fg * cstate + ig * jg;
+        const float h = og * ftanh(c);
+        cstate = c;
+        store_granule(chbuf + par * kGch + crow * kH + cu, tag, pack_bf2(c, h));
+        dc = c; dh = h;
+        dgate[0] = ig; dgate[1] = jg; dgate[2] = fg; dgate[3] = og;
+      }
+      DEC_STAMP(1);
       unsigned cv[4] = {0u, 0u, 0u, 0u};
-      sweep<4>(chbuf + par * kGch, wid * kH, tag, cv, dead, p.err, 3u, lane);
+      sweep<4, kSleep>(chbuf + par * kGch, wid * kH, tag, cv, dead, a->err, 3u, lane);
       unsigned short* crw = reinterpret_cast<unsigned short*>(ch + wid * kChS);
 #pragma unroll
       for (int q = 0; q < 4; ++q) {
         crw[q * 64 + lane] = (unsigned short)(cv[q] & 0xffffu);
         crw[kH + q * 64 + lane] = (unsigned short)(cv[q] >> 16);
       }
+      DEC_STAMP(2);
     }
     __syncthreads();
-    if (wid < 8) {
-      const int nt = wid & 1, ks = wid >> 1;
-      const bf16* arow = ch + l15 * kChS + kof;
-      const bf16* wrow = Ws + (nt * 16 + l15) * kWsS + kof;
-      f32x4 acc = f32x4{0, 0, 0, 0};
-#pragma unroll
-      for (int i = 4 * ks; i < 4 * ks + 4; ++i) acc = mfma16(ld8(arow + 32 * i), ld8(wrow + 32 * i), acc);
-#pragma unroll
-      for (int r = 0; r < 4; ++r) red[((ks * 2 + nt) * 4 + r) * 64 + lane] = acc[r];
-    }
-    __syncthreads();
-    if (wid < 8) {
-      const int w = wid & 3, nt = wid >> 2;
-      float o = 0.f;
-#pragma unroll
-      for (int src = 0; src < 4; ++src) o += red[((src * 2 + nt) * 4 + w) * 64 + lane];
-      const int row = (lane >> 4) * 4 + w, n = 32 * j + nt * 16 + l15;
-      const float sv = o + p.bs[n] + 0.f;
-      store_granule(sbuf + par * kGs + row * kA + n, tag, __float_as_uint(sv));
-      p.S[((size_t)t * B + r0 + row) * kA + n] = sv;
-    }
-    if (t < row_last && wid < 8) {
-      unsigned sv[1] = {0u};
-      sweep<1>(sbuf + par * kGs + j * kA, wid * 64, tag, sv, dead, p.err, 3u, lane);
-      srow[wid * 64 + lane] = __uint_as_float(sv[0]);
-    }
-    __syncthreads();
-    gu64* gdst = gbuf + par * kGg + j * (kE / 2);
-    attn_fwd_rowp_body<1, kNW>(
-        Fp, Gp, srow, vp, wcp, (p.COV && t > 0) ? p.COV + (size_t)t * BT : nullptr, p.lens,
-        p.ATT + (size_t)t * BT, p.COV ? p.COV + (size_t)(t + 1) * BT : nullptr,
-        p.covloss ? p.covloss + (size_t)t * B : nullptr, p.GV + (size_t)t * B * kE, p.GVb + (size_t)t * B * kE, T,
-        p.dlen, t, p.ATTb + (size_t)t * BT, b, es, part, wm, wl, redw, [&](int k, float g) {
-          const float gn = __shfl_xor(g, 1, 64);
-          if (!(k & 1)) store_granule(gdst + (k >> 1), tag, pack_bf2(g, gn));
-        });
+    {
+      KArgs* a = phase_args();
+      const int tid = phase_tid(), wid = tid >> 6, lane = tid & 63;
+      const int l15 = lane & 15, kof = 8 * (lane >> 4);
+      const int w = wid & 3, nt2 = (wid >> 2) & 1;
+      const int row = (lane >> 4) * 4 + w, n = 32 * j + nt2 * 16 + l15;
+      const float bsn = a->bs[n];
+      if (wid < 8) {
+        const int nt = wid & 1, ks = wid >> 1;
+        const bf16* arow = ch + l15 * kChS + kof;
+        const bf16* wrow = Ws + (nt * 16 + l15) * kWsS + kof;
+        f32x4 acc = f32x4{0, 0, 0, 0};
+#pragma unroll
+        for (int i = 4 * ks; i < 4 * ks + 4; ++i) acc = mfma16(ld8(arow + 32 * i), ld8(wrow + 32 * i), acc);
+#pragma unroll
+        for (int r = 0; r < 4; ++r) red[((ks * 2 + nt) * 4 + r) * 64 + lane] = acc[r];
+      }
+      __syncthreads();
+      gu64* sbuf = a->xbuf + (size_t)team * kTeamGranules + 2 * kGg + 2 * kGch;
+      if (wid < 8) {
+        float o = 0.f;
+#pragma unroll
+        for (int sl = 0; sl < 4; ++sl) o += red[((sl * 2 + nt2) * 4 + w) * 64 + lane];
+        const float sv = o + bsn + 0.f;
+        store_granule(sbuf + par * kGs + row * kA + n, tag, __float_as_uint(sv));
+        ds = sv;
+      }
+      DEC_STAMP(3);
+    }
+    {
+      KArgs* a = phase_args();
+      const bf16 *Fp = a->F, *Gp = a->G;
+      const int* lens = a->lens;
+      const int* dlen = a->dlen;
+      float *ATT = a->ATT, *COV = a->COV, *covloss = a->covloss, *GV = a->GV;
+      bf16 *ATTb = a->ATTb, *GVb = a->GVb;
+      gu64* gbuf = a->xbuf + (size_t)team * kTeamGranules;
+      {
+        const int tid = phase_tid(), wid = tid >> 6, lane = tid & 63;
+        if (t < row_last && wid < 8) {
+          unsigned sv[1] = {0u};
+          sweep<1, kSleep>(gbuf + 2 * kGg + 2 * kGch + par * kGs + j * kA, wid * 64, tag, sv, dead, a->err, 3u, lane);
+          srow[wid * 64 + lane] = __uint_as_float(sv[0]);
+        }
+      }
+      DEC_STAMP(4);
+      __syncthreads();
+      const size_t BT = (size_t)B * T;
+      gu64* gdst = gbuf + par * kGg + j * (kE / 2);
+      attn_fwd_rowp_core<1, kNW>(
+          Fp, Gp, srow, src, lens, ATT + (size_t)t * BT, has_cov ? COV + (size_t)(t + 1) * BT : nullptr,
+          has_cov ? covloss + (size_t)t * B : nullptr, GV + (size_t)t * B * kE, GVb + (size_t)t * B * kE, T, dlen, t,
+          ATTb + (size_t)t * BT, b, es, part, wm, wl, redw,
+          step_hooks(
+              [&](int k, float g) {
+                const float gn = __shfl_xor(g, 1, 64);
+                if (!(k & 1)) store_granule(gdst + (k >> 1), tag, pack_bf2(g, gn));
+              },
+              [&]() {
+                KArgs* a2 = phase_args();
+                const int tid = phase_tid(), wid = tid >> 6, lane = tid & 63;
+                const int l15 = lane & 15, w = wid & 3, rw = (lane >> 4) * 4 + w;
+                if (wid < 4) {
+                  const int cu = 16 * j + l15;
+                  const size_t o = ((size_t)(t + 1) * B + r0 + rw) * kH + cu;
+                  a2->Cst[o] = dc;
+                  a2->Cb[o] = f2bf(dc);
+                  a2->Hb[o] = f2bf(dh);
+                  float* a4 = a2->ACT + ((size_t)t * B + r0 + rw) * (4 * kH);
+                  a4[cu] = dgate[0]; a4[kH + cu] = dgate[1]; a4[2 * kH + cu] = dgate[2]; a4[3 * kH + cu] = dgate[3];
+                }
+                if (wid < 8) {
+                  const int n = 32 * j + ((wid >> 2) & 1) * 16 + l15;
+                  a2->S[((size_t)t * B + r0 + rw) * kA + n] = ds;
+                }
+              },
+              [&](int i) {
+                (void)i;
+#ifdef TSAMD_DEC_STAMPS
+                st[5 + i] = (unsigned)wall_clock64();
+#endif
+              }));
+    }
+    DEC_STAMP(7);
+#ifdef TSAMD_DEC_STAMPS
+    if (p.stamps && threadIdx.x == 0) {
+      unsigned* o = p.stamps + ((size_t)blockIdx.x * D + t) * kStamps;
+#pragma unroll
+      for (int i = 0; i < kStamps; ++i) o[i] = st[i];
+    }
+#endif
   }
+  __syncthreads();
   for (int t = tile_last; t < D; ++t) {
+    KArgs* a = phase_args();
+    const int tid = phase_tid(), wid = tid >> 6, lane = tid & 63;
     if (wid < 4) {
-      const size_t o = (size_t)(t + 1) * BH + cri;
-      p.Cst[o] = 0.f;
-      p.Cb[o] = f2bf(0.f);
-      p.Hb[o] = f2bf(0.f);
-      float* a4 = p.ACT + ((size_t)t * B + r0 + crow) * (4 * kH);
+      const int crow = (lane >> 4) * 4 + (wid & 3), cu = 16 * j + (lane & 15);
+      const size_t o = ((size_t)(t + 1) * B + r0 + crow) * kH + cu;
+      a->Cst[o] = 0.f;
+      a->Cb[o] = f2bf(0.f);
+      a->Hb[o] = f2bf(0.f);
+      float* a4 = a->ACT + ((size_t)t * B + r0 + crow) * (4 * kH);
       a4[cu] = 0.f; a4[kH + cu] = 0.f; a4[2 * kH + cu] = 0.f; a4[3 * kH + cu] = 0.f;
     }
-    __syncthreads();
-    attn_fwd_rowp_body<1, kNW>(
-        p.F, p.G, srow, p.v, p.wc, (p.COV && t > 0) ? p.COV + (size_t)t * BT : nullptr, p.lens,
-        p.ATT + (size_t)t * BT, p.COV ? p.COV + (size_t)(t + 1) * BT : nullptr,
-        p.covloss ? p.covloss + (size_t)t * B : nullptr, p.GV + (size_t)t * B * kE, p.GVb + (size_t)t * B * kE, T,
-        p.dlen, t, p.ATTb + (size_t)t * BT, b, es, part, wm, wl, redw, [](int, float) {});
+    const size_t BT = (size_t)B * T;
+    attn_fwd_rowp_dead<kNW>(src, a->ATT + (size_t)t * BT, has_cov ? a->COV + (size_t)(t + 1) * BT : nullptr,
+                            has_cov ? a->covloss + (size_t)t * B : nullptr, a->GV + (size_t)t * B * kE,
+                            a->GVb + (size_t)t * B * kE, T, a->ATTb + (size_t)t * BT, b,
+                            step_hooks([](int, float) {}, []() {}, [](int) {}));
   }
 }
 
@@ -238,6 +363,19 @@
 int dec_persistent_grid(int B) { return B >= 16 && B % 16 == 0 ? 8 * kNC * ((B / 16 + 7) / 8) : 0; }
 
 size_t dec_persistent_xbuf_elems(int B) { return (size_t)(B / 16) * kTeamGranules; }
+
+namespace {
+unsigned* g_stamps = nullptr;
+}
+int dec_persistent_stamps_into(unsigned* buf) {
+#ifdef TSAMD_DEC_STAMPS
+  g_stamps = buf;
+  return kStamps;
+#else
+  (void)buf;
+  return 0;
+#endif
+}
 
 int dec_persistent_capacity() {
   static std::mutex mu;
@@ -264,6 +402,6 @@
   const int grid = dec_persistent_grid(B);
   if (grid <= 0 || grid > dec_persistent_capacity()) return;
   DecPersistentArgs p{XG, KcT, WsT, bs, Cst, Cb, Hb, ACT, S, F, G, v, wc, COV, lens, ATT, ATTb, covloss, GV, GVb, dlen,
-                      (gu64*)xbuf, (gu32*)err, B, T, D};
+                      (gu64*)xbuf, (gu32*)err, g_stamps, B, T, D};
   hipLaunchKernelGGL(dec_fwd_persistent_kernel, dim3(grid), dim3(kNT), kLds, st, p);
 }
diff --git a/csrc/kernels/handoff.h b/csrc/kernels/handoff.h
--- a/csrc/kernels/handoff.h
+++ b/csrc/kernels/handoff.h
@@ -19,7 +19,7 @@
   __hip_atomic_store(g, ((unsigned long long)tag << 32) | v, RLX_AGENT);
 }
 
-template <int NPL>
+template <int NPL, int SLEEP = 24>
 __device__ __forceinline__ void sweep(const gu64* g, int first, unsigned tag, unsigned (&v)[NPL], bool& dead,
                                       gu32* err, unsigned code, int lane) {
   static_assert(NPL <= 32, "ready mask is 32 bits");
@@ -42,7 +42,7 @@
       dead = true;
       return;
     }
-    __builtin_amdgcn_s_sleep(24);
+    __builtin_amdgcn_s_sleep(SLEEP);
   }
 }
 
diff --git a/csrc/kernels/launchers.h b/csrc/kernels/launchers.h
--- a/csrc/kernels/launchers.h
+++ b/csrc/kernels/launchers.h
@@ -61,6 +61,7 @@
 int dec_persistent_grid(int B);
 int dec_persistent_capacity();
 size_t dec_persistent_xbuf_elems(int B);
+int dec_persistent_stamps_into(unsigned* buf);
 void launch_dec_fwd_persistent(const float* XG, const bf16* KcT, const bf16* WsT, const float* bs, float* Cst, bf16* Cb,
                                bf16* Hb, float* ACT, float* S, const bf16* F, const bf16* G, const float* v,
                                const float* wc, float* COV, const int* lens, float* ATT, bf16* ATTb, float* covloss,
diff --git a/textsummarization_on_flink_amd/_build.py b/textsummarization_on_flink_amd/_build.py
--- a/textsummarization_on_flink_amd/_build.py
+++ b/textsummarization_on_flink_amd/_build.py
@@ -57,16 +57,21 @@
     return out
 
 
+def kernel_flags(debug=False):
+    flags = ["-O3", "-std=c++17", "-fPIC", f"--offload-arch={ARCH}", "-ffp-contract=fast",
+             "-Wno-unused-result", "-munsafe-fp-atomics", f"-I{os.path.join(CSRC, 'kernels')}"]
+    if debug:
+        flags += ["-DTSAMD_DEBUG", "-fgpu-rdc"]
+    return flags
+
+
 def build_kernels(verbose=False, jobs=8, debug=False):
     bdir = BUILD + ("_debug" if debug else "")
     os.makedirs(bdir, exist_ok=True)
     kdir = os.path.join(CSRC, "kernels")
     hips = sorted(os.path.join(kdir, f) for f in os.listdir(kdir) if f.endswith(".hip"))
     hdrs = _headers(kdir)
-    common = ["-O3", "-std=c++17", "-fPIC", f"--offload-arch={ARCH}", "-ffp-contract=fast",
-              "-Wno-unused-result", "-munsafe-fp-atomics", f"-I{kdir}"]
-    if debug:
-        common += ["-DTSAMD_DEBUG", "-fgpu-rdc"]
+    common = kernel_flags(debug)
     objs, jobsl = [], []
     for src in hips:
         obj = os.path.join(bdir, os.path.basename(src) + ".o")
```

New measurement: 8.057 million tokens/s, median of 6. 1.07x the previous value.
